# liruihui/Dis-PU

Hardware: AMD Instinct MI355X
Metric: upsampled points/sec (256->1024, 4x) (higher is better)
Workload: dtype f32; 1 GPU; BASELINE configs[1]: 32 patches x 256 points per GPU, generator forward 256->1024 (4x), fp32; patches_per_gpu=32, global_patches=32, weights=xavier-uniform seed 1234, zero bias, parallelism=patch-sharded x1

## Files before the change

### dis-pu_amd/_lib.py

```python
import collections
import ctypes as C
import os

_HERE = os.path.dirname(os.path.abspath(__file__))
LIB_PATH = os.path.join(_HERE, "lib", "libdispu_hip.so")

ABI_VERSION = 5
ARITH_PLAIN = 0
ARITH_CONTRACT = 1
ARITH_PINNED_EXP = 2
MESH_BRUTE_FORCE = 8
MESH_TILE = 64
LINEAR_PLAN_INTS = 21
POISSON_MAX_N = 49152
POISSON_MAX_ROUNDS = 256
POISSON_CELLS_NONFINITE = 4
SORT_ROWS_MAX_K = 4096
RADIX_TILE = 2048
GRID_NONFINITE, GRID_AXIS_X, GRID_AXIS_Y, GRID_AXIS_Z, GRID_TOO_MANY_POINTS = 1, 2, 3, 4, 5
LATTICE_NONFINITE, LATTICE_RANGE = 1, 2
ORIENT_HOST_ROUNDS = 1
ORIENT_PROFILE_FLOATS = 8
CLUSTER_HEAD_INTS = 16

_vp, _i, _sz, _l =C.c_void_p, C.c_int, C.c_size_t, C.c_long

SIGNATURES = {
    "dispu_version": (_i, []),
    "dispu_error_string": (C.c_char_p, [_i]),
    "dispu_event_record": (_i, [_vp, _vp]),
    "dispu_stream_wait_event": (_i, [_vp, _vp]),
    "dispu_memset_async": (_i, [_vp, _i, _sz, _vp]),
    "dispu_fps_scratch_bytes": (_sz, [_i, _i, _i]),
    "dispu_fps": (_i, [_i, _i, _i, _vp, _vp, _vp, _i, _vp]),
    "dispu_fps_ws": (_i, [_i, _i, _i, _vp, _vp, _sz, _vp, _i, _vp]),
    "dispu_fps_segments_scratch_bytes": (_sz, [_i, _vp, _vp]),
    "dispu_fps_segments": (_i, [_i, _vp, _vp, _vp, _vp, _vp, _vp, _sz, _vp, _i, _vp]),
    "dispu_fps_cells_scratch_bytes": (_sz, [_i, _vp, _vp, _i]),
    "dispu_fps_cells": (_i, [_i, _vp, _vp, _vp, _vp, _vp, _vp, _sz, _vp, _vp, _i, _i, _vp]),
    "dispu_fps_cells_wanted": (_i, [_i, _i]),
    "dispu_pca_normals_scratch_bytes": (_sz, [_i, _vp, _i]),
    "dispu_pca_normals_segments": (_i, [_i, _vp, _vp, _i, _vp, _i, _vp, _vp, _vp, _vp, _vp, _vp, _sz, _vp]),
    "dispu_orient_consistent_scratch_bytes": (_sz, [_i, _vp, _i]),
    "dispu_orient_consistent_segments": (_i, [_i, _vp, _vp, _i, _vp, _vp, _vp, _i, _i, _vp, _vp, _vp, _vp, _vp, _vp, _sz, _vp, _vp]),
    "dispu_knn_mean_dist_scratch_bytes": (_sz, [_i, _vp, _i]),
    "dispu_knn_mean_dist_segments": (_i, [_i, _vp, _vp, _i, _vp, _vp, _vp, _vp, _sz, _vp]),
    "dispu_radius_count_scratch_bytes": (_sz, [_i, _vp]),
    "dispu_radius_count_segments": (_i, [_i, _vp, _vp, C.c_float, _i, _vp, _vp, _vp, _vp, _sz, _vp]),
    "dispu_outlier_threshold_segments": (_i, [_i, _vp, _vp, _vp, _vp, C.c_double, _vp, _vp]),
    "dispu_compact_scratch_bytes": (_sz, [_i, _vp]),
    "dispu_compact_segments": (_i, [_i, _vp, _vp, _vp, _i, _vp, _vp, _i, _vp, _vp, _vp, _vp, _vp, _sz, _vp]),
    "dispu_cluster_scratch_bytes": (_sz, [_i, _vp]),
    "dispu_cluster_segments": (_i, [_i, _vp, _vp, C.c_float, _i, _vp, _vp, _vp, _vp, _vp, _vp, _vp, _sz, _vp]),
    "dispu_cluster_select_segments": (_i, [_i, _vp, _vp, _vp, _vp, _vp, _vp, _i, _i, _vp, _vp]),
    "dispu_knn_cross_scratch_bytes": (_sz, [_i, _vp, _vp]),
    "dispu_knn_cross_segments": (_i, [_i, _vp, _vp, _vp, _vp, _i, _vp, _vp, _vp, _vp, _vp, _vp, _sz, _vp]),
    "dispu_transfer_attributes_segments": (_i, [_i, _vp, _vp, _vp, _vp, _i, _i, _vp, _vp, _i, _vp, _vp, _vp, _vp, _vp, _vp, _sz, _vp]),
    "dispu_mls_project_scratch_bytes": (_sz, [_i, _vp, _vp]),
    "dispu_mls_project_segments": (_i, [_i, _vp, _vp, _vp, _vp, _i, C.c_double, _i, _vp, _vp, _vp, _vp, _vp, _vp, _sz, _vp]),
    "dispu_icp_scratch_bytes": (_sz, [_i, _vp, _vp]),
    "dispu_icp_segments": (_i, [_i, _vp, _vp, _vp, _vp, _i, _i, C.c_float, C.c_double] + [_vp] * 13 + [_sz, _vp]),
    "dispu_rigid_apply_segments": (_i, [_i, _vp, _vp, _vp, _vp, _vp, _vp]),
    "dispu_signed_distance_scratch_bytes": (_sz, [_i, _vp, _vp]),
    "dispu_signed_distance_segments": (_i, [_i, _vp, _vp, _vp, _vp, _i, C.c_double, _vp, _vp, _vp, _vp, _vp, _vp, _sz, _vp]),
    "dispu_lattice_voxels_scratch_bytes": (_sz, [C.c_longlong]),
    "dispu_lattice_voxels": (_i, [C.c_longlong, _vp, C.c_float, _i, _vp, _vp, _vp, _vp, _sz, _vp]),
    "dispu_lattice_dilate_scratch_bytes": (_sz, [C.c_longlong, _i]),
    "dispu_lattice_dilate": (_i, [C.c_longlong, _vp, _i, _vp, _vp, _vp, _sz, _vp]),
    "dispu_lattice_corners_scratch_bytes": (_sz, [C.c_longlong]),
    "dispu_lattice_corners": (_i, [C.c_longlong, _vp, _vp, _vp, _vp, _vp, _sz, _vp]),
    "dispu_lattice_positions": (_i, [C.c_longlong, _vp, C.c_float, _vp, _vp]),
    "dispu_contour_count_scratch_bytes": (_sz, [C.c_longlong, C.c_longlong]),
    "dispu_contour_count": (_i, [C.c_longlong, C.c_longlong, _vp, _vp, _vp, _vp, _vp, _vp, _vp, _sz, _vp]),
    "dispu_contour_emit": (_i, [C.c_longlong, C.c_longlong, C.c_float, _vp, _vp, _vp, _vp, _vp, C.c_longlong, C.c_longlong, _vp, _vp, _vp]),
    "dispu_fps_segments_auto_scratch_bytes": (_sz, [_i, _vp, _vp]),
    "dispu_fps_segments_auto": (_i, [_i, _vp, _vp, _vp, _vp, _vp, _vp, _sz, _vp, _vp, _i, _vp]),
    "dispu_prob_sample": (_i, [_i, _i, _i, _vp, _vp, _vp, _vp, _vp]),
    "dispu_selection_sort": (_i, [_i, _i, _i, _i, _vp, _vp, _vp, _vp]),
    "dispu_gather_point": (_i, [_i, _i, _i, _vp, _vp, _vp, _vp]),
    "dispu_gather_point_grad": (_i, [_i, _i, _i, _vp, _vp, _vp, _vp]),
    "dispu_query_ball": (_i, [_i, _i, _i, _vp, _i, _vp, _vp, _vp, _vp, _i, _vp]),
    "dispu_group_point": (_i, [_i, _i, _i, _i, _i, _vp, _vp, _vp, _vp]),
    "dispu_group_point_grad": (_i, [_i, _i, _i, _i, _i, _vp, _vp, _vp, _vp]),
    "dispu_knn_point": (_i, [_i, _i, _i, _i, _i, _vp, _vp, _vp, _vp, _vp]),
    "dispu_knn_feat": (_i, [_i, _i, _i, _i, _i, _vp, _vp, _vp, _vp, _vp]),
    "dispu_knn_feat_strided": (_i, [_i, _i, _i, _i, _i, _vp, _i, _vp, _i, _vp, _vp, _vp]),
    "dispu_knn_xyz": (_i, [_i, _i, _i, _i, _vp, _vp, _vp, _vp, _i, _vp]),
    "dispu_knn_feat_scratch_bytes": (_sz, [_i, _i, _i, _i, _i]),
    "dispu_knn_feat_strided_ws": (_i, [_i, _i, _i, _i, _i, _vp, _i, _vp, _i, _vp, _vp, _vp, _sz, _vp]),
    "dispu_knn_xyz_scratch_bytes": (_sz, [_i, _i, _i, _i]),
    "dispu_knn_xyz_ws": (_i, [_i, _i, _i, _i, _vp, _vp, _vp, _vp, _vp, _sz, _i, _vp]),
    "dispu_three_nn": (_i, [_i, _i, _i, _vp, _vp, _vp, _vp, _i, _vp]),
    "dispu_three_interpolate": (_i, [_i, _i, _i, _i, _vp, _vp, _vp, _vp, _vp]),
    "dispu_three_interpolate_grad": (_i, [_i, _i, _i, _i, _vp, _vp, _vp, _vp, _vp]),
    "dispu_nn_distance": (_i, [_i, _i, _vp, _i, _vp, _vp, _vp, _vp, _vp, _i, _vp]),
    "dispu_nn_distance_grad": (_i, [_i, _i, _vp, _i, _vp, _vp, _vp, _vp, _vp, _vp, _vp, _vp]),
    "dispu_approx_match_scratch_bytes": (_sz, [_i, _i, _i]),
    "dispu_approx_match": (_i, [_i, _i, _i, _vp, _vp, _vp, _vp, _i, _vp]),
    "dispu_approx_match_ws": (_i, [_i, _i, _i, _vp, _vp, _vp, _vp, _sz, _i, _vp]),
    "dispu_approx_match_levels_ws": (_i, [_i, _i, _i, _vp, _vp, _vp, _sz, _i, _vp]),
    "dispu_emd_loss_grad_scratch_bytes": (_sz, [_i, _i, _i]),
    "dispu_emd_loss_grad": (_i, [_i, _i, _i, _vp, _vp, _vp, _vp, C.c_float, _vp, _vp, _vp, _sz, _i, _vp]),
    "dispu_match_cost_scratch_bytes": (_sz, [_i, _i, _i]),
    "dispu_match_cost": (_i, [_i, _i, _i, _vp, _vp, _vp, _vp, _i, _vp]),
    "dispu_match_cost_ws": (_i, [_i, _i, _i, _vp, _vp, _vp, _vp, _vp, _i, _vp]),
    "dispu_match_cost_grad_scratch_bytes": (_sz, [_i, _i, _i]),
    "dispu_match_cost_grad": (_i, [_i, _i, _i, _vp, _vp, _vp, _vp, _vp, _i, _vp]),
    "dispu_match_cost_grad_ws": (_i, [_i, _i, _i, _vp, _vp, _vp, _vp, _vp, _vp, _i, _vp]),
    "dispu_linear": (_i, [_i, _i, _i, _i, _vp, _l, _l, _vp, _l, _l, _i, _vp, _i, _vp, _l, _l, _vp, _l, _l, _vp, _l, _l, _vp]),
    "dispu_linear_bn": (_i, [_i, _i, _i, _i, _vp, _l, _l, _vp, _l, _l, _i, _vp, _vp, _vp, _i, _vp, _l, _l, _vp, _l, _l, _vp, _l, _l,
                             _vp]),
    "dispu_linear_tile": (_i, [_i, _i, _i]),
    "dispu_linear_tile2": (_i, [_i, _i, _i, _i, _i]),
    "dispu_debug_linear_tile": (None, [_i]),
    "dispu_linear_plan": (_i, [_i, _i, _i, _i, _vp, _l, _l, _vp, _l, _l, _i, _vp, _vp, _vp, _i, _vp, _l, _l, _vp, _l, _l, _vp, _l, _l, _vp, _l, _i,
                               _vp]),
    "dispu_linear_bf16_plan": (_i, [_i, _i, _i, _i]),
    "dispu_sa_fused": (_i, [_i, _i, _i, _i, _i, _vp, _vp, _vp, _vp, _i, _vp, _vp, _vp, _vp, _vp, _vp, _vp]),
    "dispu_edge_conv_fused": (_i, [_i, _i, _i, _i, _vp, _l, _vp, _i, _i, _vp, _vp, _vp, _vp, _vp, _i, _vp, _vp]),
    "dispu_group_center": (_i, [_l, _i, _i, _vp, _vp, _vp]),
    "dispu_pool_nsample": (_i, [_l, _i, _i, _i, _vp, _vp, _vp, _vp]),
    "dispu_idw_weights": (_i, [_l, _vp, _vp, _vp]),
    "dispu_l2_normalize_rows": (_i, [_l, _i, _vp, _vp, _vp]),
    "dispu_scale_add": (_i, [_l, _vp, C.c_float, _vp, _vp, _vp]),
    "dispu_edge_feature": (_i, [_l, _i, _i, _i, _vp, _l, _vp, _i, _i, _vp, _l, _vp]),
    "dispu_row_mean_max": (_i, [_i, _i, _vp, _vp, _vp, _vp]),
    "dispu_repulsion": (_i, [_l, _i, _i, _i, C.c_float, _vp, _vp, _vp, _vp]),
    "dispu_linear_small_k": (_i, [_l, _i, _i, _vp, _l, _vp, _vp, _i, _vp, _l, _vp]),
    "dispu_linear_small_n": (_i, [_l, _i, _i, _vp, _l, _vp, _vp, _i, _vp, _l, _vp, _l, _vp]),
    "dispu_edge_dense_conv": (_i, [_i, _i, _i, _vp, _l, _vp, _i, _i, _vp, _vp, _vp, _vp, _vp, _vp, _vp, _l, _vp]),
    "dispu_stem_block": (_i, [_i, _i, _i, _vp, _l, _i, _i, _vp, _vp, _vp, _vp, _vp, _vp, _vp, _l, _vp, _vp, _vp, _i, _vp, _l, _vp, _vp, _vp, _vp,
                              _l, _vp]),
    "dispu_edge_dense_conv_valu": (_i, [_i, _i, _i, _vp, _l, _vp, _i, _i, _vp, _vp, _vp, _vp, _vp, _vp, _vp, _l, _vp]),
    "dispu_dup_grid": (_i, [_i, _i, _i, _i, _vp, _l, _vp, _vp, _vp, _vp, _l, _vp]),
    "dispu_ps_prep": (_i, [_l, _i, _vp, _vp, _vp, _vp, _l, _vp, _l, _vp]),
    "dispu_ps_gather_sub_relu": (_i, [_l, _i, _i, _i, _vp, _vp, _l, _vp, _l, _vp, _l, _vp]),
    "dispu_ps_skip_max": (_i, [_l, _i, _i, _i, _vp, _vp, _vp, _l, _vp, _l, _vp]),
    "dispu_ps_weight_net": (_i, [_l, _i, _i, _i, _vp, _vp, _vp, _vp, _vp, _vp, _vp, _vp]),
    "dispu_ps_point_matmul": (_i, [_l, _i, _i, _i, _vp, _l, _vp, _vp, _l, _vp]),
    "dispu_ps_local": (_i, [_l, _i, _i, _i, _vp, _vp, _vp, _l, _vp, _vp, _vp, _vp, _vp, _vp, _vp, _vp, _vp]),
    "dispu_ps_local_bf16": (_i, [_l, _i, _i, _i, _vp, _vp, _vp, _l, _vp, _vp, _vp, _vp, _vp, _vp, _vp, _vp, _vp]),
    "dispu_knn_patch": (_i, [_i, _i, _i, _i, _vp, _vp, _vp, _vp]),
    "dispu_normalize_patches": (_i, [_i, _i, _vp, _vp, _vp, _vp, _vp]),
    "dispu_denormalize_patches": (_i, [_i, _i, _vp, _vp, _vp, _vp, _vp]),
    "dispu_knn_patch_segments": (_i, [_i, _vp, _vp, _vp, _vp, _i, _vp, _vp, _vp, _vp]),
    "dispu_normalize_segments": (_i, [_i, _vp, _vp, _vp, _vp, _vp, _vp, _vp]),
    "dispu_attention": (_i, [_i, _i, _i, _i, _vp, _l, _vp, _l, _vp, _l, C.c_float, _vp, _l, _vp]),
    "dispu_attention_fwd_lse": (_i, [_i, _i, _i, _i, _vp, _l, _vp, _l, _vp, _l, C.c_float, _vp, _l, _vp, _vp]),
    "dispu_attention_bwd": (_i, [_i, _i, _i, _i, _vp, _l, _vp, _l, _vp, _l, C.c_float, _vp, _l, _vp, _vp, _l, _vp, _l, _vp, _l, _vp, _l,
                                 _vp, _vp]),
    "dispu_attention_project": (_i, [_i, _i, _i, _i, _vp, _l, _vp, _l, _vp, _l, C.c_float, _vp, _vp, _i, _vp, _l, _vp]),
    "dispu_softmax_rows": (_i, [_l, _i, C.c_float, _vp, _l, _vp]),
    "dispu_linear_tn_bf16_stream_scratch_floats": (_l, [_i, _i, _i]),
    "dispu_linear_tn_bf16_stream": (_i, [_i, _i, _i, _vp, _l, _vp, _l, _i, _vp, _l, _i, _vp, _vp, _l, _vp]),
    "dispu_bf16_pack": (_i, [_i, _i, _vp, _l, _i, _vp, _vp]),
    "dispu_linear_bf16_stream": (_i, [_i, _i, _i, _vp, _l, _i, _vp, _l, _vp, _i, _vp, _l, _i, _i, _l, _vp]),
    "dispu_linear_bf16": (_i, [_i, _i, _i, _i, _vp, _l, _l, _vp, _l, _l, _i, _vp, _i, _vp, _l, _l, _vp, _l, _l, _vp, _l, _l, _vp]),
    "dispu_linear_tn_bf16_scratch_floats": (_l, [_i, _i, _i, _i]),
    "dispu_linear_tn_bf16": (_i, [_i, _i, _i, _i, _vp, _l, _l, _vp, _l, _l, _vp, _l, _l, _i, _vp, _vp, _l, _vp]),
    "dispu_bf16x3_split_weights": (_i, [_i, _i, _vp, _l, _vp, _vp]),
    "dispu_linear_bf16x3": (_i, [_i, _i, _i, _vp, _l, _vp, _vp, _i, _vp, _l, _vp, _l, _vp, _l, _vp]),
    "dispu_debug_x3_kernel": (None, [_i]),
    "dispu_linear_tn_scratch_floats": (_l, [_i, _i, _i, _i]),
    "dispu_linear_tn": (_i, [_i, _i, _i, _i, _vp, _l, _l, _vp, _l, _l, _vp, _l, _l, _i, _vp, _vp, _l, _vp]),
    "dispu_ps_local_grad": (_i, [_l, _i] + [_vp] * 3 + [_l] + [_vp] * 14),
    "dispu_linear_tn_plan": (_i, [_i, _i, _i, _i, _vp, _l, _l, _vp, _l, _l, _vp, _l, _l, _i, _vp, _vp, _l, _vp]),
    "dispu_linear_tn_bf16_plan": (_i, [_i, _i, _i, _i, _vp, _l, _l, _vp, _l, _l, _vp, _l, _l, _i, _vp, _vp, _l, _i, _vp]),
    "dispu_linear_tn_bf16_stream_plan": (_i, [_i, _i, _i, _vp, _l, _vp, _l, _i, _vp, _l, _i, _vp, _vp, _l, _vp]),
    "dispu_tn_defer": (_i, [_vp]),
    "dispu_tn_reduce_grouped": (_i, [_i, _vp, _vp, _vp]),
    "dispu_act_bias_grad_scratch_floats": (_l, [_l, _i]),
    "dispu_act_bias_grad": (_i, [_l, _i, _vp, _l, _vp, _l, _i, _vp, _l, _vp, _i, _vp, _l, _vp]),
    "dispu_max_k": (_i, [_l, _i, _i, _vp, _l, _vp, _l, _vp]),
    "dispu_max_k_grad": (_i, [_l, _i, _i, _vp, _l, _vp, _l, _vp, _l, _vp, _l, _i, _vp]),
    "dispu_max_k_grad_tail": (_i, [_l, _i, _i, _i, _vp, _l, _vp, _l, _vp, _l, _vp, _l, _vp]),
    "dispu_edge_feature_grad": (_i, [_l, _i, _i, _i, _vp, _l, _vp, _i, _i, _vp, _l, _vp]),
    "dispu_dup_sum_grad": (_i, [_i, _i, _i, _i, _vp, _l, _vp, _l, _vp]),
    "dispu_ps_group": (_i, [_l, _i, _i, _i, _vp, _vp, _vp, _l, _vp, _l, _vp]),
    "dispu_ps_group_grad": (_i, [_l, _i, _i, _i, _vp, _vp, _l, _vp, _vp, _l, _vp]),
    "dispu_ps_point_matmul_grad": (_i, [_l, _i, _i, _i, _vp, _l, _vp, _vp, _l, _vp, _l, _vp, _vp]),
    "dispu_softmax_rows_grad": (_i, [_l, _i, C.c_float, _vp, _l, _vp, _l, _vp]),
    "dispu_bn_scratch_bytes": (_l, [_l, _i]),
    "dispu_bn_train": (_i, [_l, _i, _vp, _l, _vp, _vp, C.c_float, C.c_float, _i, _vp, _l, _vp, _vp, _vp, _vp, _l, _vp]),
    "dispu_bn_train_grad": (_i, [_l, _i, _vp, _l, _vp, _l, _vp, _l, _vp, _vp, _i, _vp, _l, _vp, _vp, _vp, _vp, _l, _vp]),
    "dispu_sigmoid_offset": (_i, [_l, _vp, _vp, _vp, _vp]),
    "dispu_sigmoid_offset_grad": (_i, [_l, _vp, _vp, _vp, _vp, _vp]),
    "dispu_repulsion_grad": (_i, [_l, _i, _i, C.c_float, C.c_float, _vp, _vp, _vp, _vp]),
    "dispu_add3": (_i, [_l, _vp, _vp, _vp, _vp, _vp]),
    "dispu_linear_splitk_finish": (_i, [_l, _i, _i, _vp, _l, _vp, _i, _vp, _l, _vp]),
    "dispu_fill_rows": (_i, [_i, _i, _vp, C.c_float, _vp, _vp]),
    "dispu_mlp_chain": (_i, [_l, _i, _i, _i, _i, _vp, _l, _vp, _vp, _vp, _vp, _vp, _vp, _vp, _vp, _vp, _l, _i, _vp, _l, _vp, _l, _vp]),
    "dispu_linear_masked": (_i, [_i, _i, _i, _i, _vp, _l, _l, _vp, _l, _l, _i, _vp, _i, _vp, _l, _l, _vp, _l, _l, _vp, _l, _i, _vp]),
    "dispu_linear_bf16_masked": (_i, [_i, _i, _i, _i, _vp, _l, _l, _vp, _l, _l, _i, _vp, _i, _vp, _l, _l, _vp, _l, _l, _vp, _l, _i, _vp]),
    "dispu_mlp_chain_sum3": (_i, [_l, _i, _i, _i, _i, _vp, _vp, _vp, _l, _vp, _vp, _vp, _vp, _vp, _vp, _vp, _vp, _vp, _l, _i, _vp, _l, _vp, _l, _vp]),
    "dispu_mlp_chain_dup": (_i, [_i, _i, _i, _i, _i, _i, _i, _vp, _l, _vp, _vp, _vp, _vp, _vp, _vp, _vp, _vp, _vp, _vp, _vp, _vp, _l, _i, _vp, _l,
                                 _vp, _l, _vp]),
    "dispu_mlp_chain_stash": (_i, [_l, _i, _i, _i, _i, _vp, _l, _vp, _vp, _vp, _vp, _vp, _vp, _vp, _vp, _vp, _l, _vp, _l, _vp, _l, _vp, _l,
                                   _i, _vp, _l, _vp, _l, _vp]),
    "dispu_mlp_chain_grad": (_i, [_l, _i, _i, _i, _vp, _l, _vp, _vp, _vp, _vp, _vp, _l, _vp, _l, _vp, _l, _vp, _l, _vp, _l, _vp, _l, _vp, _l, _vp, _l,
                                  _vp, _vp, _vp, _l, _vp, _vp, _vp, _l, _vp]),
    "dispu_mask3": (_i, [_l, _i, _vp, _l, _vp, _l, _vp, _l, _vp, _l, _vp, _vp, _vp, _l, _vp]),
    "dispu_ps_wnet_scratch_bytes": (_l, [_l]),
    "dispu_ps_wnet_bn_stats": (_i, [_l, _i, _i, _i, _vp, _vp, _vp, _vp, _vp, _vp, C.c_float, C.c_float, _vp, _vp, _vp, _vp, _vp, _vp, _l, _vp]),
    "dispu_ps_wnet_grad": (_i, [_l, _i, _i, _i, _vp, _vp, _vp, _vp, _vp, _vp, _vp, _vp, _vp, _vp, _vp, _vp, _vp, _vp, _vp, _vp, _l, _vp]),
    "dispu_knn_invert": (_i, [_i, _i, _i, _vp, _vp, _vp, _vp]),
    "dispu_ps_conv0_gather_grad": (_i, [_l, _i, _i, _i, _vp, _vp, _vp, _vp, _l, _vp, _l, _vp, _l, _vp, _l, _vp, _l, _vp]),
    "dispu_ps_prep_grad": (_i, [_l, _i, _vp, _vp, _vp, _l, _vp, _l, _vp, _vp, _vp]),
    "dispu_ps_skip_max_grad": (_i, [_l, _i, _i, _i, _vp, _vp, _vp, _l, _vp, _l, _vp, _l, _vp, _vp, _l, _i, _vp]),
    "dispu_ps_point_matmul_grad_relu": (_i, [_l, _i, _i, _i, _vp, _l, _vp, _vp, _l, _vp, _l, _vp, _vp]),
    "dispu_edge_dense_conv_grad_scratch_floats": (_l, [_i, _i]),
    "dispu_edge_dense_conv_grad_partials": (_i, [_i, _i, _i, _vp, _l, _vp, _i, _i, _vp, _vp, _vp, _vp, _vp, _vp, _vp, _l, _vp, _l, _vp, _l, _vp]),
    "dispu_edge_dense_conv_grad_reduce": (_i, [_i, _i, _vp, _l, _vp, _vp, _vp, _vp, _vp, _vp, _vp]),
    "dispu_edge_dense_conv_grad": (_i, [_i, _i, _i, _vp, _l, _vp, _i, _i, _vp, _vp, _vp, _vp, _vp, _vp, _vp, _l, _vp, _l, _vp, _vp, _vp, _vp, _vp,
                                        _vp, _vp, _l, _vp]),
    "dispu_repulsion_loss_grad": (_i, [_l, _i, _i, C.c_float, C.c_float, _vp, _vp, _vp, _vp, _vp]),
    "dispu_transpose_batched": (_i, [_i, _vp, _vp, _vp, _vp]),
    "dispu_linear_bf16s": (_i, [_i, _i, _i, _i, _vp, _l, _l, _vp, _l, _l, _i, _vp, _i, _vp, _l, _l, _vp, _l, _l, _i, _vp]),
    "dispu_linear_tn_bf16s": (_i, [_i, _i, _i, _i, _vp, _l, _l, _vp, _l, _l, _vp, _l, _l, _i, _vp, _vp, _l, _i, _vp]),
    "dispu_ps_gather_sub_relu_bf16": (_i, [_l, _i, _i, _i, _vp, _vp, _l, _vp, _l, _vp, _l, _vp]),
    "dispu_ps_point_matmul_grad_relu_s": (_i, [_l, _i, _i, _i, _vp, _l, _vp, _vp, _l, _vp, _l, _vp, _i, _vp]),
    "dispu_ps_conv0_gather_grad_s": (_i, [_l, _i, _i, _i, _vp, _vp, _vp, _vp, _l, _i, _vp, _l, _vp, _l, _vp, _l, _vp, _l, _vp]),
    "dispu_chamfer_loss_grad": (_i, [_i, _i, _vp, _i, _vp, _vp, _vp, _vp, _vp, _vp, C.c_float, _vp, _vp, _vp]),
    "dispu_pu_loss_finalize": (_i, [_vp, _vp, _l, C.c_float, C.c_float, _vp, _vp]),
    "dispu_step_meters": (_i, [_i, _i, _i, _vp, _vp, _vp, _vp, _vp, _vp, _vp, _vp]),
    "dispu_uniform_loss_grad": (_i, [_i, _i, _i, _i, _vp, _vp, _vp, _vp, _vp, _vp, _vp, _vp, _i, _vp]),
    "dispu_pu_loss_finalize_u": (_i, [_vp, _vp, _l, C.c_float, C.c_float, _vp, _i, _l, C.c_float, _vp, _vp]),
    "dispu_pu_loss_finalize_e": (_i, [_vp, _vp, _l, C.c_float, C.c_float, _vp, _i, _l, C.c_float, _vp, _vp, _i, _i, C.c_float, _vp, _vp]),
    "dispu_augment": (_i, [_i, _i, _vp, _vp, _vp, _vp, _vp, _vp, _vp]),
    "dispu_sample_batch": (_i, [_i, _i, _i, _vp, _vp, _vp, _i, _i, C.c_ulonglong, _i, C.c_float, C.c_float, _i, _vp, _vp, _vp, _vp, _vp, _vp,
                                _vp, _vp, _vp, _vp]),
    "dispu_adam": (_i, [_l, _vp, _vp, _vp, _vp, C.c_float, C.c_float, C.c_float, C.c_float, C.c_float, _vp]),
    "dispu_point_to_mesh": (_i, [_i, _vp, _i, _vp, _vp, _vp, _vp, _vp, _vp, _i, _vp]),
    "dispu_disk_count": (_i, [_i, _i, _i, _vp, _vp, _vp, _vp, _vp]),
    "dispu_disk_fill": (_i, [_i, _i, _i, _vp, _vp, _vp, _vp, _vp, _vp]),
    "dispu_disk_uniformity_scratch_bytes": (_sz, [_i, _i]),
    "dispu_disk_uniformity": (_i, [_i, _i, _i, _vp, _vp, _vp, _vp, _vp, _i, _vp, _sz, _vp, _vp]),
    "dispu_row_mean_std": (_i, [_i, _i, _vp, _vp, _vp]),
    "dispu_geodesic_scratch_bytes": (_sz, [_i, _i]),
    "dispu_geodesic_hash_slots": (_i, [_i]),
    "dispu_geodesic_distances": (_i, [_i, _vp, _vp, _vp, _vp, _vp, _vp, _vp, _vp, _vp, _i, _vp, _vp, _vp, _vp, C.c_double, _i, _vp, _sz, _vp,
                                      _vp, _vp]),
    "dispu_geodesic_disk_count": (_i, [_i, _i, _vp, _vp, _vp, _vp, _vp]),
    "dispu_geodesic_disk_fill": (_i, [_i, _i, _vp, _vp, _vp, _vp, _vp, _vp, _vp]),
    "dispu_mesh_sample": (_i, [_i, _i, _vp, _vp, _vp, _i, C.c_ulonglong, _vp, _vp, _vp, _vp]),
    "dispu_poisson_disk_scratch_bytes": (_sz, [_i, _i]),
    "dispu_poisson_disk_keep": (_i, [_i, _i, _vp, _vp, _vp, _vp, _vp, _sz, _vp, _vp]),
    "dispu_poisson_disk_select": (_i, [_i, _i, _i, _i, _vp, _vp, _vp, _vp, _vp, _vp, _sz, _vp, _vp]),
    "dispu_sort_rows_i32": (_i, [_i, _i, _vp, _vp]),
    "dispu_poisson_cells_scratch_bytes": (_sz, [_i, C.c_longlong]),
    "dispu_poisson_cells_keep": (_i, [_i, _vp, _vp, _vp, _vp, _vp, _vp, _vp, _vp, _sz, _vp, _vp]),
    "dispu_poisson_cells_select": (_i, [_i, _vp, _vp, _vp, _vp, _i, _vp, _vp, _vp, _vp, _vp, _vp, _vp, _sz, _vp, _vp]),
    "dispu_radix_sort_scratch_bytes": (_sz, [C.c_longlong]),
    "dispu_radix_sort_pairs": (_i, [C.c_longlong, _i, _vp, _vp, _vp, _vp, _vp, _sz, _vp]),
    "dispu_grid_subsample_scratch_bytes": (_sz, [C.c_longlong, _i, _i]),
    "dispu_grid_subsample_plan": (_i, [C.c_longlong, _vp, C.c_float, _vp, _sz, _vp, _vp, _vp, _vp]),
    "dispu_grid_subsample_emit": (_i, [C.c_longlong, _i, _i, _i, _vp, _vp, _vp, _vp, _sz, _vp, _vp, _vp, _vp]),
}

class TnReduceDesc(C.Structure):
    _fields_ = [("part", _vp), ("out", _vp), ("dbias", _vp), ("ldo", _l), ("stride", _l), ("K", _i), ("N", _i), ("splits", _i),
                ("rows_p", _i), ("accumulate", _i), ("bias_accumulate", _i), ("assoc", _i), ("reserved", _i)]


_LIB = None


class DispuError(RuntimeError):
    pass


def lib():
    global _LIB
    if _LIB is None:
        import torch
        if not os.path.exists(LIB_PATH):
            raise DispuError(
                "libdispu_hip.so not found at %s -- build it with `python dis-pu_amd/build.py` "
                "(there is no CPU fallback for the dis-pu_amd ops)" % LIB_PATH)
        l = C.CDLL(LIB_PATH)
        for name, (res, args) in SIGNATURES.items():
            fn = getattr(l, name)
            fn.restype = res
            fn.argtypes = args
        if l.dispu_version() < ABI_VERSION:
            raise DispuError("libdispu_hip.so at %s has ABI version %d, this package needs >= %d -- rebuild it with "
                             "`python dis-pu_amd/build.py`" % (LIB_PATH, l.dispu_version(), ABI_VERSION))
        _LIB = l
    return _LIB


class Tape(object):
    def __init__(self):
        self.calls = []
        self.keep = []

    def replay(self):
        for fn, args, what in self.calls:
            rc = fn(*args)
            if rc:
                check(rc, what + " (tape replay)")

    def __len__(self):
        return len(self.calls)


_TAPE = None
_NO_TAPE = ("dispu_version", "dispu_error_string", "dispu_linear_tile", "dispu_linear_tile2", "dispu_linear_plan", "dispu_linear_bf16_plan",
            "dispu_linear_tn_plan", "dispu_linear_tn_bf16_plan", "dispu_linear_tn_bf16_stream_plan")


class _TapeLib(object):

    def __init__(self, real):
        self._real = real
        self._cache = {}

    def __getattr__(self, name):
        fn = self._cache.get(name)
        if fn is None:
            real = getattr(self._real, name)
            if name in _NO_TAPE or real.restype is not _i or "scratch" in name:
                fn = real
            else:
                argtypes = real.argtypes

                def fn(*args, _real=real, _types=argtypes, _name=name):
                    if _TAPE is None:
                        return _real(*args)
                    cargs = tuple(a if isinstance(a, C._SimpleCData) else t(a) for a, t in zip(args, _types))
                    rc = _real(*cargs)
                    _TAPE.calls.append((_real, cargs, _name))
                    return rc
            self._cache[name] = fn
        return fn


_TAPELIB = None


def tape_lib():
    global _TAPELIB
    if _TAPELIB is None:
        _TAPELIB = _TapeLib(lib())
    return _TAPELIB


def tape_begin():
    global _TAPE
    _TAPE = Tape()
    return _TAPE


def tape_end():
    global _TAPE
    t, _TAPE = _TAPE, None
    return t


def taping():
    return _TAPE


def check(code, what):
    if code != 0:
        msg = lib().dispu_error_string(code)
        raise DispuError("%s failed: hip error %d (%s)" % (what, code, msg.decode() if msg else "?"))


def linear_plan(batch, M, K, N, X, ldx, sx, W, ldw, sw, transb, bias, scale, shift, act, Y, ldy, sy, R1, ldr1, sr1, R2, ldr2, sr2, Mk, ldm,
                mcols):
    buf = (_i * LINEAR_PLAN_INTS)()
    check(lib().dispu_linear_plan(batch, M, K, N, X, ldx, sx, W, ldw, sw, transb, bias, scale, shift, act, Y, ldy, sy, R1, ldr1, sr1, R2, ldr2,
                                  sr2, Mk, ldm, mcols, buf), "dispu_linear_plan")
    out = []
    for i in range(buf[0]):
        kind, n0, n1, bm, bn, bk, tb, edge, epi, ng = buf[1 + 10 * i:11 + 10 * i]
        out.append(("tiled", n0, n1, bm, bn, bk, tb, edge, epi) if kind else ("skinny", n0, n1, ng, tb))
    return out


TnPlan = collections.namedtuple("TnPlan", "rc kind TK TNN edge splits rows direct reduce reduce_grid capped wpb grid_y")
TnBf16Plan = collections.namedtuple("TnBf16Plan", "rc kind tile splits rows reduce rows_p")
TnStreamPlan = collections.namedtuple("TnStreamPlan", "rc BN storage splits rows")
TN_KINDS = ("none", "narrow", "tiled", "clear")
TN_REDUCE = ("none", "scalar", "vec4")


def linear_tn_plan(batch, M, K, N, X, ldx, sx, Z, ldz, sz, out, ldo, so, accumulate, dbias, scratch, scratch_floats):
    buf = (_i * 12)()
    rc = lib().dispu_linear_tn_plan(batch, M, K, N, X, ldx, sx, Z, ldz, sz, out, ldo, so, accumulate, dbias, scratch, scratch_floats, buf)
    v = list(buf)
    return TnPlan(rc, TN_KINDS[v[0]], v[1], v[2], v[3], v[4], v[5], v[6], TN_REDUCE[v[7]], v[8], v[9], v[10], v[11])


def linear_tn_bf16_plan(batch, M, K, N, X, ldx, sx, Z, ldz, sz, out, ldo, so, accumulate, dbias, scratch, scratch_floats, storage=0):
    buf = (_i * 6)()
    rc = lib().dispu_linear_tn_bf16_plan(batch, M, K, N, X, ldx, sx, Z, ldz, sz, out, ldo, so, accumulate, dbias, scratch, scratch_floats,
                                         storage, buf)
    v = list(buf)
    return TnBf16Plan(rc, TN_KINDS[v[0]], v[1], v[2], v[3], v[4], v[5])


def linear_tn_bf16_stream_plan(M, K, N, X, ldx, Z, ldz, storage, out, ldo, accumulate, dbias, scratch, scratch_floats):
    buf = (_i * 4)()
    rc = lib().dispu_linear_tn_bf16_stream_plan(M, K, N, X, ldx, Z, ldz, storage, out, ldo, accumulate, dbias, scratch, scratch_floats, buf)
    return TnStreamPlan(rc, *list(buf))


def stream_ptr(device=None):
    import torch
    return C.c_void_p(torch.cuda.current_stream(device).cuda_stream)


def ptr(t):
    return C.c_void_p(t.data_ptr()) if t is not None else C.c_void_p(0)
```

### dis-pu_amd/csrc/linear.hip

```cpp
#include "common.h"
#include "internal.h"

#include <type_traits>

#include <cstdio>
#include <cstdlib>

namespace dispu {

typedef float f32x16 __attribute__((ext_vector_type(16)));

struct LinearArgs {
    int M, K, N;
    const float* X; long ldx; long sx;
    const float* W; long ldw; long sw;
    const float* bias;
    float* Y; long ldy; long sy;
    const float* R1; long ldr1; long sr1;
    const float* R2; long ldr2; long sr2;
    int act;
    const float* scale;
    const float* shift;
    const float* Mk; long ldm; int mcols;
};

template <int BM, int BN, int BK, bool TRANSB, bool EDGE>
struct LinearLds {
    static constexpr bool DMA = !EDGE && !TRANSB && BK == 16 && (BM == 64 || BM == 128) && (BN == 64 || BN == 128 || BN == 256);
    static constexpr int NST = DMA ? 4 : 2;
    static constexpr int LDA = DMA ? BM : BM + 1;
    static constexpr int LDB = TRANSB ? BN + 1 : (DMA && BN < 256) ? BN : BN + 4;
    static constexpr int STAGE = ((BK * (LDA + LDB) + 3) / 4) * 4;
    static constexpr size_t BYTES = (size_t)NST * STAGE * sizeof(float);
};

#ifdef LIN_CLOCK
__device__ unsigned long long lin_clock_ticks[4];
#endif
template <int BM, int BN, int WM, int WN, int BK, bool TRANSB, bool EDGE, int EPI_T>
__global__ __launch_bounds__(64 * (WM * WN + (LinearLds<BM, BN, BK, TRANSB, EDGE>::DMA ? 4 : WM * WN))) void linear_mfma_kernel(LinearArgs a) {
#ifdef LIN_CLOCK
    const unsigned long long lc0 = __builtin_readcyclecounter();
    unsigned long long lc_wait = 0;
#endif
    using L = LinearLds<BM, BN, BK, TRANSB, EDGE>;
    constexpr bool DMA = L::DMA;
    constexpr int NT = 64 * WM * WN;
    constexpr int LDA = L::LDA, LDB = L::LDB;
    constexpr int TM = BM / (32 * WM), TN = BN / (32 * WN);
    constexpr int A_F4 = BM * BK / 4 / NT;
    constexpr int B_F4 = BN * BK / 4 / NT;
    static_assert(A_F4 >= 1 && B_F4 >= 1 && TM >= 1 && TN >= 1, "tile too small for the workgroup");
    static_assert((BM * BK / 4) % NT == 0 && (BN * BK / 4) % NT == 0, "tile must split evenly over the threads");
    extern __shared__ __attribute__((aligned(16))) float lds[];

    const int lane = threadIdx.x & 63, wave = threadIdx.x >> 6;
    const int z = blockIdx.z;
    const int m0 = blockIdx.y * BM, n0 = blockIdx.x * BN;
    const int M = a.M, K = a.K, N = a.N;
    const int ntile = (K + BK - 1) / BK;

    if (wave >= WM * WN) {
        if constexpr (DMA) {
            const int lw = __builtin_amdgcn_readfirstlane(wave - WM * WN);
            const float* __restrict__ X = a.X + (size_t)z * a.sx;
            const float* __restrict__ W = a.W + (size_t)z * a.sw;
            constexpr int NA = 4 * BM / 64, NB = 16 * BN / 256, PER = (NA + NB) / 4;
            static_assert((NA + NB) % 4 == 0, "DMA instructions must split evenly over the four loader waves");
            constexpr int RPI = 256 / BN;
            const long ldw = a.ldw, ldx = a.ldx;
            const float* gsrc[PER];
            int ldst[PER];
#pragma unroll
            for (int u = 0; u < PER; ++u) {
                const int q = lw + 4 * u;
                if (q < NA) {
                    const int kg = q / (BM / 64), rb = q % (BM / 64);
                    gsrc[u] = X + (size_t)(m0 + rb * 64 + lane) * ldx + 4 * kg;
                    ldst[u] = (kg * BM + rb * 64) * 4;
                } else {
                    const int pb = q - NA, kr = pb * RPI + lane / (BN / 4);
                    gsrc[u] = W + (size_t)kr * ldw + n0 + 4 * (lane % (BN / 4));
                    ldst[u] = BK * LDA + (pb * RPI) * LDB;
                }
            }
            auto issue = [&](int t) {
                float* st = lds + (t & 3) * L::STAGE;
                const size_t ko = (size_t)t * BK;
#pragma unroll
                for (int u = 0; u < PER; ++u) {
                    const int q = lw + 4 * u;
                    const float* src = (q < NA) ? gsrc[u] + ko : gsrc[u] + ko * ldw;
                    __builtin_amdgcn_global_load_lds(src, (__attribute__((address_space(3))) void*)(st + ldst[u]), 16, 0, 0);
                }
            };
            auto wait_newer = [&](int newer) {
                if (newer >= 2) __builtin_amdgcn_s_waitcnt(0x0F70 | (((2 * PER) & 0xF)) | ((((2 * PER) >> 4) & 0x3) << 14));
                else if (newer == 1) __builtin_amdgcn_s_waitcnt(0x0F70 | ((PER & 0xF)) | (((PER >> 4) & 0x3) << 14));
                else __builtin_amdgcn_s_waitcnt(0x0F70);
            };
            issue(0);
            if (ntile > 1) issue(1);
            if (ntile > 2) issue(2);
            wait_newer(min(2, ntile - 1));
            asm volatile("s_barrier" ::: "memory");
            for (int t = 0; t < ntile; ++t) {
                if (t + 3 < ntile) issue(t + 3);
                wait_newer(max(0, min(2, ntile - 2 - t)));
                asm volatile("s_barrier" ::: "memory");
            }
            return;
        }
        const int tid = threadIdx.x - NT;
        const float* __restrict__ X = a.X + (size_t)z * a.sx;
        const float* __restrict__ W = a.W + (size_t)z * a.sw;
        const long ldx = a.ldx, ldw = a.ldw;
        float4 pa[A_F4], pb[B_F4];
        const bool x_vec = ((ldx & 3) == 0) && ((((uintptr_t)X) & 15) == 0);
        const bool w_vec = ((ldw & 3) == 0) && ((((uintptr_t)W) & 15) == 0);

        auto load_rowsk = [&](const float* __restrict__ P, long ld, bool vec, int row_base, int rows, int k0, int it) -> float4 {
            const int idx = tid + it * NT;
            const int r = idx / (BK / 4), kq = idx % (BK / 4);
            const int row = row_base + r, k = k0 + kq * 4;
            if constexpr (!EDGE) return *reinterpret_cast<const float4*>(P + (size_t)row * ld + k);
            float4 v = make_float4(0.f, 0.f, 0.f, 0.f);
            if (row < rows && k < K) {
                const float* p = P + (size_t)row * ld + k;
                if (vec && k + 3 < K) {
                    v = *reinterpret_cast<const float4*>(p);
                } else {
                    v.x = p[0];
                    if (k + 1 < K) v.y = p[1];
                    if (k + 2 < K) v.z = p[2];
                    if (k + 3 < K) v.w = p[3];
                }
            }
            return v;
        };
        auto store_rowsk = [&](float* S, int LD, float4 v, int it) {
            const int idx = tid + it * NT;
            const int r = idx / (BK / 4), kq = idx % (BK / 4);
            S[(kq * 4 + 0) * LD + r] = v.x;
            S[(kq * 4 + 1) * LD + r] = v.y;
            S[(kq * 4 + 2) * LD + r] = v.z;
            S[(kq * 4 + 3) * LD + r] = v.w;
        };
        auto load_b = [&](int k0, int it) -> float4 {
            const int idx = tid + it * NT;
            const int kr = idx / (BN / 4), nq = idx % (BN / 4);
            const int k = k0 + kr, n = n0 + nq * 4;
            if constexpr (!EDGE) return *reinterpret_cast<const float4*>(W + (size_t)k * ldw + n);
            float4 v = make_float4(0.f, 0.f, 0.f, 0.f);
            if (k < K && n < N) {
                const float* p = W + (size_t)k * ldw + n;
                if (w_vec && n + 3 < N) {
                    v = *reinterpret_cast<const float4*>(p);
                } else {
                    v.x = p[0];
                    if (n + 1 < N) v.y = p[1];
                    if (n + 2 < N) v.z = p[2];
                    if (n + 3 < N) v.w = p[3];
                }
            }
            return v;
        };
        auto store_b = [&](float* S, float4 v, int it) {
            const int idx = tid + it * NT;
            const int kr = idx / (BN / 4), nq = idx % (BN / 4);
            *reinterpret_cast<float4*>(&S[kr * LDB + nq * 4]) = v;
        };
        float4 pa1[A_F4], pb1[B_F4];
        auto load_tile = [&](int k0, float4 (&qa)[A_F4], float4 (&qb)[B_F4]) {
#pragma unroll
            for (int it = 0; it < A_F4; ++it) qa[it] = load_rowsk(X, ldx, x_vec, m0, M, k0, it);
#pragma unroll
            for (int it = 0; it < B_F4; ++it) qb[it] = TRANSB ? load_rowsk(W, ldw, w_vec, n0, N, k0, it) : load_b(k0, it);
        };
        auto store_tile = [&](int stage, const float4 (&qa)[A_F4], const float4 (&qb)[B_F4]) {
            float* As = lds + stage * L::STAGE;
            float* Bs = As + BK * LDA;
#pragma unroll
            for (int it = 0; it < A_F4; ++it) store_rowsk(As, LDA, qa[it], it);
#pragma unroll
            for (int it = 0; it < B_F4; ++it) {
                if constexpr (TRANSB) store_rowsk(Bs, LDB, qb[it], it);
                else store_b(Bs, qb[it], it);
            }
        };
        load_tile(0, pa, pb);
        store_tile(0, pa, pb);
        if (ntile > 1) load_tile(BK, pa1, pb1);
        if (ntile > 2) load_tile(2 * BK, pa, pb);
        __syncthreads();
        for (int t = 0; t < ntile; t += 2) {
            if (t + 1 < ntile) {
                store_tile(1, pa1, pb1);
                if (t + 3 < ntile) load_tile((t + 3) * BK, pa1, pb1);
            }
            __syncthreads();
            if (t + 1 < ntile) {
                if (t + 2 < ntile) {
                    store_tile(0, pa, pb);
                    if (t + 4 < ntile) load_tile((t + 4) * BK, pa, pb);
                }
                __syncthreads();
            }
        }
        return;
    }

    const int wm = wave / WN, wn = wave % WN;
    f32x16 acc[TM][TN];
#pragma unroll
    for (int i = 0; i < TM; ++i)
#pragma unroll
        for (int j = 0; j < TN; ++j)
#pragma unroll
            for (int r = 0; r < 16; ++r) acc[i][j][r] = 0.f;

    const int fi = lane & 31, fk = lane >> 5;
    constexpr bool CI = !EDGE && !TRANSB && (TN == 4 || TN == 2);
    auto rdB = [&](const float* Bs, int krow, float (&b)[TN]) {
        if constexpr (CI && TN == 4) {
            const float4 t4 = *reinterpret_cast<const float4*>(&Bs[krow * LDB + wn * (TN * 32) + 4 * fi]);
            b[0] = t4.x; b[1] = t4.y; b[2] = t4.z; b[3] = t4.w;
        } else if constexpr (CI && TN == 2) {
            const float2 t2 = *reinterpret_cast<const float2*>(&Bs[krow * LDB + wn * (TN * 32) + 2 * fi]);
            b[0] = t2.x; b[1] = t2.y;
        } else {
#pragma unroll
            for (int j = 0; j < TN; ++j) b[j] = Bs[krow * LDB + wn * (TN * 32) + j * 32 + fi];
        }
    };
    __syncthreads();
    if constexpr (DMA) {
        auto slab = [&](auto stage_c) {
            constexpr int SG = decltype(stage_c)::value;
            const float* st = lds + SG * L::STAGE;
            const float* Bs = st + BK * LDA;
            const float* Asf = st + fk;
            float a2[2][TM][2];
            float bf[2][TN];
#pragma unroll
            for (int i = 0; i < TM; ++i) {
                const float* pr = Asf + (wm * (TM * 32) + i * 32 + fi) * 4;
                a2[0][i][0] = pr[0]; a2[0][i][1] = pr[2];
            }
            rdB(Bs, fk, bf[0]);
#pragma unroll
            for (int s2 = 0; s2 < BK / 2; ++s2) {
                const int kg = s2 >> 1, u = s2 & 1, cur = s2 & 1, nxt = cur ^ 1;
                if (s2 + 1 < BK / 2) {
                    const int kk = 2 * (s2 + 1);
                    if (u == 1) {
#pragma unroll
                        for (int i = 0; i < TM; ++i) {
                            const float* pr = Asf + ((kg + 1) * BM + wm * (TM * 32) + i * 32 + fi) * 4;
                            a2[(kg + 1) & 1][i][0] = pr[0]; a2[(kg + 1) & 1][i][1] = pr[2];
                        }
                    }
                    rdB(Bs, kk + fk, bf[nxt]);
                }
#pragma unroll
                for (int i = 0; i < TM; ++i)
#pragma unroll
                    for (int j = 0; j < TN; ++j)
                        acc[i][j] = __builtin_amdgcn_mfma_f32_32x32x2f32(a2[kg & 1][i][u], bf[cur][j], acc[i][j], 0, 0, 0);
                constexpr int NB = CI ? 1 : TN / 2;
                if (u == 1) __builtin_amdgcn_sched_group_barrier(0x100, TM + NB, 0);
                else __builtin_amdgcn_sched_group_barrier(0x100, NB, 0);
                __builtin_amdgcn_sched_group_barrier(0x008, TM * TN, 0);
            }
#ifdef LIN_CLOCK
            const unsigned long long lb0 = __builtin_readcyclecounter();
            __syncthreads();
            lc_wait += __builtin_readcyclecounter() - lb0;
#else
            __syncthreads();
#endif
        };
        for (int t = 0; t < ntile; t += 4) {
            slab(std::integral_constant<int, 0>{});
            if (t + 1 < ntile) slab(std::integral_constant<int, 1>{});
            if (t + 2 < ntile) slab(std::integral_constant<int, 2>{});
            if (t + 3 < ntile) slab(std::integral_constant<int, 3>{});
        }
    } else
    for (int t = 0; t < ntile; ++t) {
        const float* As = lds + (t & 1) * L::STAGE;
        const float* Bs = As + BK * LDA;
        float af[2][TM], bf[2][TN];
#pragma unroll
        for (int i = 0; i < TM; ++i) af[0][i] = As[fk * LDA + wm * (TM * 32) + i * 32 + fi];
        rdB(Bs, fk, bf[0]);
#pragma unroll
        for (int s2 = 0; s2 < BK / 2; ++s2) {
            const int cur = s2 & 1, nxt = cur ^ 1;
            if (s2 + 1 < BK / 2) {
                const int kk = 2 * (s2 + 1);
#pragma unroll
                for (int i = 0; i < TM; ++i) af[nxt][i] = As[(kk + fk) * LDA + wm * (TM * 32) + i * 32 + fi];
                rdB(Bs, kk + fk, bf[nxt]);
            }
#pragma unroll
            for (int i = 0; i < TM; ++i)
#pragma unroll
                for (int j = 0; j < TN; ++j)
                    acc[i][j] = __builtin_amdgcn_mfma_f32_32x32x2f32(af[cur][i], bf[cur][j], acc[i][j], 0, 0, 0);
            __builtin_amdgcn_sched_group_barrier(0x100, TM + (CI ? 1 : TN), 0);
            __builtin_amdgcn_sched_group_barrier(0x008, TM * TN, 0);
        }
#ifdef LIN_CLOCK
        const unsigned long long lb0 = __builtin_readcyclecounter();
        __syncthreads();
        lc_wait += __builtin_readcyclecounter() - lb0;
#else
        __syncthreads();
#endif
    }

#ifdef LIN_CLOCK
    if (blockIdx.x == 0 && blockIdx.y == 5 && threadIdx.x == 0) { lin_clock_ticks[0] = __builtin_readcyclecounter() - lc0; lin_clock_ticks[1] = ntile; lin_clock_ticks[2] = lc_wait; }
#endif
    constexpr int EPI = (EPI_T == 6) ? 0 : EPI_T;
    constexpr bool E_SCALE = (EPI == 1 || EPI == 4), E_R1 = (EPI >= 2), E_R2 = (EPI >= 3);
    float* __restrict__ Y = a.Y + (size_t)z * a.sy;
    const float lo = (a.act == 1) ? 0.f : -__builtin_inff();
    const bool has_bias = a.bias != nullptr;
    const float* __restrict__ R1 = (E_R1 && a.R1) ? a.R1 + (size_t)z * a.sr1 : nullptr;
    const float* __restrict__ R2 = (E_R2 && a.R2) ? a.R2 + (size_t)z * a.sr2 : nullptr;
    const int wm_u = __builtin_amdgcn_readfirstlane(wm), wn_u = __builtin_amdgcn_readfirstlane(wn);
    const int rbase = m0 + wm_u * (TM * 32), cbase = n0 + wn_u * (TN * 32);
    const long ldy = a.ldy, ldr1 = a.ldr1, ldr2 = a.ldr2, ldm = a.ldm;
    const unsigned offy = (unsigned)(4 * fk * ldy + fi), off1 = (unsigned)(4 * fk * ldr1 + fi), off2 = (unsigned)(4 * fk * ldr2 + fi);
    const unsigned offm = (unsigned)(4 * fk * ldm + fi);
    if constexpr (CI) {
        typedef float vecT __attribute__((ext_vector_type(TN)));
        const int col0 = cbase + TN * fi;
        const unsigned voy = (unsigned)(4 * fk * ldy + TN * fi), vo1 = (unsigned)(4 * fk * ldr1 + TN * fi), vo2 = (unsigned)(4 * fk * ldr2 + TN * fi);
        const unsigned vom = (unsigned)(4 * fk * ldm + TN * fi);
        vecT bv, sc, sh;
#pragma unroll
        for (int j = 0; j < TN; ++j) { bv[j] = 0.f; sc[j] = 1.f; sh[j] = 0.f; }
        if (has_bias) bv = *reinterpret_cast<const vecT*>(a.bias + col0);
        if constexpr (E_SCALE) {
            if (a.scale) { sc = *reinterpret_cast<const vecT*>(a.scale + col0); sh = *reinterpret_cast<const vecT*>(a.shift + col0); }
        }
#pragma unroll
        for (int i = 0; i < TM; ++i) {
#pragma unroll
            for (int rb = 0; rb < 16; rb += 8) {
                vecT r1v[8], r2v[8], mkv[8];
                if constexpr (EPI == 5) {
#pragma unroll
                    for (int r = 0; r < 8; ++r) {
                        const int rowu = rbase + i * 32 + ((rb + r) & 3) + 8 * ((rb + r) >> 2);
#pragma unroll
                        for (int j = 0; j < TN; ++j) mkv[r][j] = 1.f;
                        if (a.Mk != nullptr) {
                            const vecT m = *reinterpret_cast<const vecT*>(a.Mk + (size_t)rowu * ldm + cbase + vom);
#pragma unroll
                            for (int j = 0; j < TN; ++j) mkv[r][j] = (col0 + j < a.mcols) ? m[j] : 1.f;
                        }
                    }
                }
                if constexpr (EPI >= 4) {
#pragma unroll
                    for (int r = 0; r < 8; ++r) {
                        const int rowu = rbase + i * 32 + ((rb + r) & 3) + 8 * ((rb + r) >> 2);
#pragma unroll
                        for (int j = 0; j < TN; ++j) { r1v[r][j] = 0.f; r2v[r][j] = 0.f; }
                        if (R1) r1v[r] = *reinterpret_cast<const vecT*>(R1 + (size_t)rowu * ldr1 + cbase + vo1);
                    }
#pragma unroll
                    for (int r = 0; r < 8; ++r) {
                        const int rowu = rbase + i * 32 + ((rb + r) & 3) + 8 * ((rb + r) >> 2);
                        if (R2) r2v[r] = *reinterpret_cast<const vecT*>(R2 + (size_t)rowu * ldr2 + cbase + vo2);
                    }
                }
#pragma unroll
                for (int r = 0; r < 8; ++r) {
                    const int rowu = rbase + i * 32 + ((rb + r) & 3) + 8 * ((rb + r) >> 2);
                    vecT v;
#pragma unroll
                    for (int j = 0; j < TN; ++j) {
                        float e = acc[i][j][rb + r];
                        if (has_bias) e = e + bv[j];
                        if constexpr (E_SCALE) {
                            if (a.scale) e = e * sc[j] + sh[j];
                        }
                        e = fmaxf(e, lo);
                        if constexpr (EPI >= 4) {
                            if (R1) e = e + r1v[r][j];
                            if (R2) e = e + r2v[r][j];
                        }
                        if constexpr (EPI == 5) e = (mkv[r][j] > 0.f) ? e : 0.f;
                        v[j] = e;
                    }
                    *reinterpret_cast<vecT*>(Y + (size_t)rowu * ldy + cbase + voy) = v;
                }
                if constexpr (EPI >= 4) __builtin_amdgcn_sched_barrier(0);
            }
        }
        return;
    }
#pragma unroll
    for (int j = 0; j < TN; ++j) {
        const int colu = cbase + j * 32;
        const int col = colu + fi;
        const bool col_ok = !EDGE || col < N;
        const int colc = col_ok ? col : 0;
        const float bv = has_bias ? a.bias[colc] : 0.f;
        float sc = 1.f, sh = 0.f;
        if constexpr (E_SCALE) {
            if (a.scale) { sc = a.scale[colc]; sh = a.shift[colc]; }
        }
#pragma unroll
        for (int i = 0; i < TM; ++i) {
            float r1v[16], r2v[16], mkv[16];
            if constexpr (EPI == 5) {
                const bool msk = a.Mk != nullptr && col < a.mcols && col_ok;
#pragma unroll
                for (int r = 0; r < 16; ++r) {
                    const int rowu = rbase + i * 32 + (r & 3) + 8 * (r >> 2);
                    const bool ok = msk && (!EDGE || rowu + 4 * fk < M);
                    mkv[r] = ok ? (a.Mk + (size_t)rowu * ldm + colu)[offm] : 1.f;
                }
            }
            if constexpr (EPI >= 4) {
#pragma unroll
                for (int r = 0; r < 16; ++r) {
                    const int rowu = rbase + i * 32 + (r & 3) + 8 * (r >> 2);
                    const bool ok = col_ok && (!EDGE || rowu + 4 * fk < M);
                    r1v[r] = (R1 && ok) ? (R1 + (size_t)rowu * ldr1 + colu)[off1] : 0.f;
                }
#pragma unroll
                for (int r = 0; r < 16; ++r) {
                    const int rowu = rbase + i * 32 + (r & 3) + 8 * (r >> 2);
                    const bool ok = col_ok && (!EDGE || rowu + 4 * fk < M);
                    r2v[r] = (R2 && ok) ? (R2 + (size_t)rowu * ldr2 + colu)[off2] : 0.f;
                }
            }
#pragma unroll
            for (int r = 0; r < 16; ++r) {
                const int rowu = rbase + i * 32 + (r & 3) + 8 * (r >> 2);
                if (col_ok && (!EDGE || rowu + 4 * fk < M)) {
                    float v = acc[i][j][r];
                    if (has_bias) v = v + bv;
                    if constexpr (E_SCALE) {
                        if (a.scale) v = v * sc + sh;
                    }
                    v = fmaxf(v, lo);
                    if constexpr (EPI >= 4) {
                        if (R1) v = v + r1v[r];
                        if (R2) v = v + r2v[r];
                    }
                    if constexpr (EPI == 5) v = (mkv[r] > 0.f) ? v : 0.f;
                    (Y + (size_t)rowu * ldy + colu)[offy] = v;
                }
            }
            if constexpr (EPI >= 4) __builtin_amdgcn_sched_barrier(0);
        }
    }
}

template <int BM, int BN, int WM, int WN, int BK, bool TRANSB, bool EDGE, int EPI>
static int launch_epi(const LinearArgs& a, dim3 grid, hipStream_t s) {
    constexpr size_t bytes = LinearLds<BM, BN, BK, TRANSB, EDGE>::BYTES;
    auto kern = linear_mfma_kernel<BM, BN, WM, WN, BK, TRANSB, EDGE, EPI>;
    if (bytes > 64 * 1024) {
        static DevOnce done;
        if (done.needed()) {
            hipError_t e = hipFuncSetAttribute(reinterpret_cast<const void*>(kern), hipFuncAttributeMaxDynamicSharedMemorySize, (int)bytes);
            if (e != hipSuccess) return (int)e;
            done.done();
        }
    }
    hipLaunchKernelGGL(kern, grid, dim3(64 * (WM * WN + (LinearLds<BM, BN, BK, TRANSB, EDGE>::DMA ? 4 : WM * WN))), bytes, s, a);
    return (int)hipGetLastError();
}

struct LinearLaunch {
    int skinny;
    int n0, n1;
    int bm, bn, bk;
    int transb;
    int edge;
    int epi;
    int ng;
};
struct LinearPlan {
    int n;
    LinearLaunch l[2];
};

}

using namespace dispu;

static int g_tile_override = 0;
DISPU_EXPORT void dispu_debug_linear_tile(int code) { g_tile_override = code; }

static int linear_tile_rule(int batch, int M, int N, bool dma) {
    if (g_tile_override > 0) return g_tile_override;
    const long mb128 = (long)((M + 127) / 128) * batch;
    if (N >= 256 && N % 256 == 0 && mb128 * (N / 256) >= 256) return 128257;
    if (N > 64 && N % 128 != 0 && N % 64 == 0 && mb128 >= 64) return 64064;
    const long mb64 = (long)((M + 63) / 64) * batch;
    if (N > 64) {
        if (mb128 * ((N + 127) / 128) >= 256) return 128128;
        const long wg = mb64 * ((N + 127) / 128);
        return (wg >= 512 || (dma && N % 128 == 0 && wg >= 256)) ? 64128 : 64064;
    }
    return mb128 >= 256 ? 128064 : 64064;
}

DISPU_EXPORT int dispu_linear_tile(int batch, int M, int N) { return linear_tile_rule(batch, M, N, true); }
DISPU_EXPORT int dispu_linear_tile2(int batch, int M, int K, int N, int transb) { return linear_tile_rule(batch, M, N, !transb && (K % 16) == 0); }

static LinearLaunch linear_decide_tiled(const LinearArgs& a, int batch, bool transb) {
    LinearLaunch l{};
    l.n0 = 0; l.n1 = a.N; l.transb = transb ? 1 : 0;
    constexpr int BK = 16;
    int bkr = 32;
    switch (linear_tile_rule(batch, a.M, a.N, !transb && (a.K % 16) == 0)) {
        case 128257: l.bm = 128; l.bn = 256; bkr = 16; break;
        case 128128: l.bm = 128; l.bn = 128; break;
        case 64128: l.bm = 64; l.bn = 128; break;
        case 128064: l.bm = 128; l.bn = 64; break;
        default: l.bm = 64; l.bn = 64; break;
    }
    const bool aligned = ((a.ldx & 3) == 0) && ((a.ldw & 3) == 0) && ((a.sx & 3) == 0) && ((a.sw & 3) == 0) &&
                         ((((uintptr_t)a.X) & 15) == 0) && ((((uintptr_t)a.W) & 15) == 0);
    const auto al16 = [](const void* p) { return (((uintptr_t)p) & 15) == 0; };
    const bool out_aligned = ((a.ldy & 3) == 0) && ((a.sy & 3) == 0) && al16(a.Y) && (!a.bias || al16(a.bias)) &&
                             (!a.scale || (al16(a.scale) && al16(a.shift))) &&
                             (!a.R1 || (((a.ldr1 & 3) == 0) && ((a.sr1 & 3) == 0) && al16(a.R1))) &&
                             (!a.R2 || (((a.ldr2 & 3) == 0) && ((a.sr2 & 3) == 0) && al16(a.R2))) &&
                             (!a.Mk || (((a.ldm & 3) == 0) && al16(a.Mk) && a.mcols >= a.N));
    const bool tiles_ok = aligned && out_aligned && (a.M % l.bm == 0) && (a.N % l.bn == 0);
    if (tiles_ok && !transb && (a.K % BK == 0)) { l.bk = BK; l.edge = 0; }
    else if (tiles_ok && transb && (a.K % bkr == 0)) { l.bk = bkr; l.edge = 0; }
    else { l.bk = bkr; l.edge = 1; }
    if (!a.scale && !a.R1 && !a.R2 && !a.Mk)
        l.epi = (l.bm == 128 && l.bn == 256 && l.bk == 16 && !transb && !l.edge && a.K >= 1024) ? 6 : 0;
    else if (a.scale && !a.R1 && !a.R2 && !a.Mk) l.epi = 1;
    else l.epi = a.Mk ? 5 : 4;
    return l;
}

static int linear_decide(int batch, int M, int K, int N, const float* X, long ldx, long sx, const float* W, long ldw, long sw, int transb,
                         const float* bias, const float* scale, const float* shift, int act, const float* Y, long ldy, long sy,
                         const float* R1, long ldr1, long sr1, const float* R2, long ldr2, long sr2, const float* Mk, long ldm, int mcols,
                         LinearPlan& plan) {
    plan = LinearPlan{};
    if (batch < 0 || M < 0 || K <= 0 || N <= 0 || !X || !W || !Y || act < 0 || act > 1 || ((scale == nullptr) != (shift == nullptr)))
        return (int)hipErrorInvalidValue;
    if (Mk && batch != 1) return (int)hipErrorInvalidValue;
    if (batch == 0 || M == 0) return 0;
    int nh = N;
    if (batch == 1 && !scale && !R2) {
        int ng = linear_skinny_rule(M, K, N, X, ldx, W, ldw, transb);
        if (ng == 0) {
            const int tail = N % 128, n0 = N - tail;
            if (n0 > 0 && tail > 0 && tail <= 32) {
                const float* Wt = transb ? W + (size_t)n0 * ldw : W + n0;
                const int ngt = linear_skinny_rule(M, K, tail, X, ldx, Wt, ldw, transb);
                if (ngt) {
                    LinearLaunch& t = plan.l[plan.n++];
                    t.skinny = 1; t.n0 = n0; t.n1 = N; t.transb = transb ? 1 : 0; t.ng = ngt;
                    nh = n0;
                    ng = linear_skinny_rule(M, K, nh, X, ldx, W, ldw, transb);
                }
            }
        }
        if (ng) {
            LinearLaunch& t = plan.l[plan.n++];
            t.skinny = 1; t.n0 = 0; t.n1 = nh; t.transb = transb ? 1 : 0; t.ng = ng;
            return 0;
        }
    }
    LinearArgs a{M, K, nh, X, ldx, sx, W, ldw, sw, bias, const_cast<float*>(Y), ldy, sy, R1, ldr1, sr1, R2, ldr2, sr2, act, scale, shift,
                 (Mk && mcols > 0) ? Mk : nullptr, ldm, mcols};
    plan.l[plan.n++] = linear_decide_tiled(a, batch, transb != 0);
    return 0;
}

template <int BM, int BN, int WM, int WN, int BK, bool TRANSB, bool EDGE>
static int launch_one(const LinearArgs& a, dim3 grid, int epi, hipStream_t s) {
    switch (epi) {
        case 0: return launch_epi<BM, BN, WM, WN, BK, TRANSB, EDGE, 0>(a, grid, s);
        case 1: return launch_epi<BM, BN, WM, WN, BK, TRANSB, EDGE, 1>(a, grid, s);
        case 4: return launch_epi<BM, BN, WM, WN, BK, TRANSB, EDGE, 4>(a, grid, s);
        case 5: return launch_epi<BM, BN, WM, WN, BK, TRANSB, EDGE, 5>(a, grid, s);
        case 6:
            if constexpr (BM == 128 && BN == 256 && BK == 16 && !TRANSB && !EDGE) return launch_epi<BM, BN, WM, WN, BK, TRANSB, EDGE, 6>(a, grid, s);
            break;
    }
    return (int)hipErrorInvalidValue;
}

template <int BM, int BN, int WM, int WN, int BK, int BKR = BK>
static int launch_linear(const LinearArgs& a, int batch, const LinearLaunch& l, hipStream_t s) {
    dim3 grid((a.N + BN - 1) / BN, (a.M + BM - 1) / BM, batch);
    if (!l.edge && !l.transb) return launch_one<BM, BN, WM, WN, BK, false, false>(a, grid, l.epi, s);
    if (!l.edge) return launch_one<BM, BN, WM, WN, BKR, true, false>(a, grid, l.epi, s);
    if (l.transb) return launch_one<BM, BN, WM, WN, BKR, true, true>(a, grid, l.epi, s);
    return launch_one<BM, BN, WM, WN, BKR, false, true>(a, grid, l.epi, s);
}

static int linear_impl(int batch, int M, int K, int N, const float* X, long ldx, long sx, const float* W, long ldw, long sw, int transb,
                       const float* bias, const float* scale, const float* shift, int act, float* Y, long ldy, long sy, const float* R1,
                       long ldr1, long sr1, const float* R2, long ldr2, long sr2, const float* Mk, long ldm, int mcols, void* stream);

DISPU_EXPORT int dispu_linear(int batch, int M, int K, int N, const float* X, long ldx, long sx, const float* W,
                              long ldw, long sw, int transb, const float* bias, int act, float* Y, long ldy, long sy,
                              const float* R1, long ldr1, long sr1, const float* R2, long ldr2, long sr2, void* stream) {
    return linear_impl(batch, M, K, N, X, ldx, sx, W, ldw, sw, transb, bias, nullptr, nullptr, act, Y, ldy, sy, R1, ldr1,
                       sr1, R2, ldr2, sr2, nullptr, 0, 0, stream);
}

DISPU_EXPORT int dispu_linear_masked(int batch, int M, int K, int N, const float* X, long ldx, long sx, const float* W,
                                     long ldw, long sw, int transb, const float* bias, int act, float* Y, long ldy, long sy,
                                     const float* R1, long ldr1, long sr1, const float* Mk, long ldm, int mcols, void* stream) {
    if (Mk && batch != 1) return (int)hipErrorInvalidValue;
    return linear_impl(batch, M, K, N, X, ldx, sx, W, ldw, sw, transb, bias, nullptr, nullptr, act, Y, ldy, sy, R1, ldr1,
                       sr1, nullptr, 0, 0, Mk, ldm, Mk ? mcols : 0, stream);
}

DISPU_EXPORT int dispu_linear_bn(int batch, int M, int K, int N, const float* X, long ldx, long sx, const float* W,
                                 long ldw, long sw, int transb, const float* bias, const float* scale, const float* shift,
                                 int act, float* Y, long ldy, long sy, const float* R1, long ldr1, long sr1,
                                 const float* R2, long ldr2, long sr2, void* stream) {
    return linear_impl(batch, M, K, N, X, ldx, sx, W, ldw, sw, transb, bias, scale, shift, act, Y, ldy, sy, R1, ldr1, sr1, R2, ldr2, sr2,
                       nullptr, 0, 0, stream);
}

DISPU_EXPORT int dispu_linear_plan(int batch, int M, int K, int N, const float* X, long ldx, long sx, const float* W, long ldw, long sw,
                                   int transb, const float* bias, const float* scale, const float* shift, int act, const float* Y, long ldy,
                                   long sy, const float* R1, long ldr1, long sr1, const float* R2, long ldr2, long sr2, const float* Mk,
                                   long ldm, int mcols, int* plan) {
    if (!plan) return (int)hipErrorInvalidValue;
    LinearPlan p;
    const int rc = linear_decide(batch, M, K, N, X, ldx, sx, W, ldw, sw, transb, bias, scale, shift, act, Y, ldy, sy, R1, ldr1, sr1, R2,
                                 ldr2, sr2, Mk, ldm, Mk ? mcols : 0, p);
    for (int i = 0; i < DISPU_LINEAR_PLAN_INTS; ++i) plan[i] = 0;
    if (rc) return rc;
    plan[0] = p.n;
    for (int i = 0; i < p.n; ++i) {
        const LinearLaunch& l = p.l[i];
        int* o = plan + 1 + 10 * i;
        o[0] = l.skinny ? 0 : 1; o[1] = l.n0; o[2] = l.n1; o[3] = l.bm; o[4] = l.bn; o[5] = l.bk; o[6] = l.transb; o[7] = l.edge;
        o[8] = l.epi; o[9] = l.ng;
    }
    return 0;
}

static int linear_impl(int batch, int M, int K, int N, const float* X, long ldx, long sx, const float* W, long ldw, long sw, int transb,
                       const float* bias, const float* scale, const float* shift, int act, float* Y, long ldy, long sy, const float* R1,
                       long ldr1, long sr1, const float* R2, long ldr2, long sr2, const float* Mk, long ldm, int mcols, void* stream) {
    LinearPlan plan;
    int rc = linear_decide(batch, M, K, N, X, ldx, sx, W, ldw, sw, transb, bias, scale, shift, act, Y, ldy, sy, R1, ldr1, sr1, R2, ldr2, sr2,
                           Mk, ldm, mcols, plan);
    if (rc) return rc;
    hipStream_t s = (hipStream_t)stream;
    for (int i = 0; i < plan.n; ++i) {
        const LinearLaunch& l = plan.l[i];
        const int n0 = l.n0, nn = l.n1 - l.n0;
        if (l.skinny) {
            const float* Wt = transb ? W + (size_t)n0 * ldw : W + n0;
            rc = linear_skinny_launch(l.ng, M, K, nn, X, ldx, Wt, ldw, transb, bias ? bias + n0 : nullptr, act, Y + n0, ldy,
                                      R1 ? R1 + n0 : nullptr, ldr1, Mk ? Mk + n0 : nullptr, ldm, mcols - n0, s);
        } else {
            LinearArgs a{M, K, nn, X, ldx, sx, W, ldw, sw, bias, Y, ldy, sy, R1, ldr1, sr1, R2, ldr2, sr2, act, scale, shift,
                         (Mk && mcols > 0) ? Mk : nullptr, ldm, mcols};
            switch (l.bm * 1000 + l.bn) {
                case 128256: rc = launch_linear<128, 256, 2, 2, 16>(a, batch, l, s); break;
                case 128128: rc = launch_linear<128, 128, 2, 2, 16, 32>(a, batch, l, s); break;
                case 64128: rc = launch_linear<64, 128, 2, 2, 16, 32>(a, batch, l, s); break;
                case 128064: rc = launch_linear<128, 64, 2, 2, 16, 32>(a, batch, l, s); break;
                default: rc = launch_linear<64, 64, 2, 2, 16, 32>(a, batch, l, s); break;
            }
        }
        if (rc) return rc;
    }
    return 0;
}
```

### dis-pu_amd/csrc/ps_local.hip

```cpp
#include "common.h"

#include <cstdlib>
#include <type_traits>

namespace dispu {

typedef float f32x16 __attribute__((ext_vector_type(16)));
typedef float f32x2 __attribute__((ext_vector_type(2)));
typedef float f32x4 __attribute__((ext_vector_type(4)));
typedef unsigned u32x4 __attribute__((ext_vector_type(4)));
typedef unsigned u32x2 __attribute__((ext_vector_type(2)));
typedef __bf16 bf16x4 __attribute__((ext_vector_type(4)));

constexpr int PL_BM = 128, PL_BN = 128, PL_BK = 32, PL_K = 128, PL_NT = 256;
constexpr int PL_LDA = PL_BM + 1, PL_LDB = PL_BN + 4;
constexpr int PL_STAGE = PL_BK * (PL_LDA + PL_LDB);
constexpr size_t PL_LDS_BYTES = (size_t)(2 * PL_STAGE + 8 * 256) * sizeof(float);

__global__ __launch_bounds__(PL_NT) void ps_local_kernel(long npoints, int n_per_cloud, const int* __restrict__ idx,
                                                          const float* __restrict__ xyz, const float* __restrict__ Gm, long ldg,
                                                          const float* __restrict__ Am, const float* __restrict__ W1,
                                                          const float* __restrict__ b1, const float* __restrict__ Ww,
                                                          const float* __restrict__ bw, const float* __restrict__ scale,
                                                          const float* __restrict__ shift, float* __restrict__ out) {
    extern __shared__ __attribute__((aligned(16))) float lds[];
    float* wv = lds + 2 * PL_STAGE;
    const int tid = threadIdx.x, lane = tid & 63, wave = tid >> 6;
    const int wm = wave >> 1, wn = wave & 1;
    const long p0 = (long)blockIdx.x * 8;

#pragma unroll
    for (int e = tid; e < 8 * 256; e += PL_NT) {
        const int t = e & 15, s = (e >> 4) & 15, pl = e >> 8;
        const long i = p0 + pl;
        float v = 0.f;
        if (i < npoints) {
            const long j = (i / n_per_cloud) * n_per_cloud + idx[i * 16 + s];
            float acc = 0.f;
#pragma unroll
            for (int c = 0; c < 3; ++c) acc = __builtin_fmaf(xyz[j * 3 + c] - xyz[i * 3 + c], Ww[c * 16 + t], acc);
            acc = acc + bw[t];
            acc = acc * scale[t] + shift[t];
            v = fmaxf(acc, 0.f);
        }
        wv[e] = v;
    }

    const int kq = tid & 7;
    long gi[4], gj[4];
#pragma unroll
    for (int it = 0; it < 4; ++it) {
        const int r = (tid >> 3) + 32 * it;
        long i = p0 + (r >> 4);
        if (i >= npoints) i = npoints - 1;
        gi[it] = i;
        gj[it] = (i / n_per_cloud) * n_per_cloud + idx[i * 16 + (r & 15)];
    }
    float4 pg[4], pa[4], pb[4];
    auto load_tile = [&](int k0) {
#pragma unroll
        for (int it = 0; it < 4; ++it) {
            pg[it] = *reinterpret_cast<const float4*>(Gm + gj[it] * ldg + k0 + kq * 4);
            pa[it] = *reinterpret_cast<const float4*>(Am + gi[it] * PL_K + k0 + kq * 4);
        }
#pragma unroll
        for (int it = 0; it < 4; ++it) {
            const int e = tid + it * PL_NT;
            const int kr = e / (PL_BN / 4), nq = e % (PL_BN / 4);
            pb[it] = *reinterpret_cast<const float4*>(W1 + (size_t)(k0 + kr) * PL_BN + nq * 4);
        }
    };
    auto store_tile = [&](int stage) {
        float* As = lds + stage * PL_STAGE;
        float* Bs = As + PL_BK * PL_LDA;
#pragma unroll
        for (int it = 0; it < 4; ++it) {
            const int r = (tid >> 3) + 32 * it;
            As[(kq * 4 + 0) * PL_LDA + r] = fmaxf(pg[it].x - pa[it].x, 0.f);
            As[(kq * 4 + 1) * PL_LDA + r] = fmaxf(pg[it].y - pa[it].y, 0.f);
            As[(kq * 4 + 2) * PL_LDA + r] = fmaxf(pg[it].z - pa[it].z, 0.f);
            As[(kq * 4 + 3) * PL_LDA + r] = fmaxf(pg[it].w - pa[it].w, 0.f);
        }
#pragma unroll
        for (int it = 0; it < 4; ++it) {
            const int e = tid + it * PL_NT;
            const int kr = e / (PL_BN / 4), nq = e % (PL_BN / 4);
            *reinterpret_cast<float4*>(&Bs[kr * PL_LDB + nq * 4]) = pb[it];
        }
    };

    f32x16 acc[2][2];
#pragma unroll
    for (int i = 0; i < 2; ++i)
#pragma unroll
        for (int j = 0; j < 2; ++j)
#pragma unroll
            for (int r = 0; r < 16; ++r) acc[i][j][r] = 0.f;

    constexpr int NTILE = PL_K / PL_BK;
    load_tile(0);
    store_tile(0);
    load_tile(PL_BK);
    __syncthreads();
    const int fi = lane & 31, fk = lane >> 5;
#pragma unroll
    for (int t = 0; t < NTILE; ++t) {
        const float* As = lds + (t & 1) * PL_STAGE;
        const float* Bs = As + PL_BK * PL_LDA;
        if (t + 1 < NTILE) {
            store_tile((t + 1) & 1);
            if (t + 2 < NTILE) load_tile((t + 2) * PL_BK);
        }
#pragma unroll
        for (int kk = 0; kk < PL_BK; kk += 2) {
            float af[2], bf[2];
#pragma unroll
            for (int i = 0; i < 2; ++i) af[i] = As[(kk + fk) * PL_LDA + wm * 64 + i * 32 + fi];
#pragma unroll
            for (int j = 0; j < 2; ++j) bf[j] = Bs[(kk + fk) * PL_LDB + wn * 64 + j * 32 + fi];
#pragma unroll
            for (int i = 0; i < 2; ++i)
#pragma unroll
                for (int j = 0; j < 2; ++j)
                    acc[i][j] = __builtin_amdgcn_mfma_f32_32x32x2f32(af[i], bf[j], acc[i][j], 0, 0, 0);
        }
        __syncthreads();
    }

#pragma unroll
    for (int j = 0; j < 2; ++j) {
        const int c = wn * 64 + j * 32 + fi;
        const float bias = b1[c];
#pragma unroll
        for (int i = 0; i < 2; ++i) {
#pragma unroll
            for (int q = 0; q < 2; ++q) {
                const int pl = wm * 4 + i * 2 + q;
                float own[8], oth[8];
#pragma unroll
                for (int u = 0; u < 8; ++u) {
                    own[u] = fmaxf(acc[i][j][q * 8 + u] + bias, 0.f);
                    oth[u] = __shfl_xor(own[u], 32, 64);
                }
                float o[8];
#pragma unroll
                for (int t = 0; t < 8; ++t) o[t] = 0.f;
                const float* wp = wv + pl * 256 + fk * 8;
#pragma unroll
                for (int s = 0; s < 16; ++s) {
                    const int u = (s & 3) + 4 * (s >> 3);
                    const bool hi = (s >> 2) & 1;
                    const float xv = (hi == (fk != 0)) ? own[u] : oth[u];
                    const float4 w0 = *reinterpret_cast<const float4*>(wp + s * 16);
                    const float4 w1 = *reinterpret_cast<const float4*>(wp + s * 16 + 4);
                    o[0] = __builtin_fmaf(xv, w0.x, o[0]); o[1] = __builtin_fmaf(xv, w0.y, o[1]);
                    o[2] = __builtin_fmaf(xv, w0.z, o[2]); o[3] = __builtin_fmaf(xv, w0.w, o[3]);
                    o[4] = __builtin_fmaf(xv, w1.x, o[4]); o[5] = __builtin_fmaf(xv, w1.y, o[5]);
                    o[6] = __builtin_fmaf(xv, w1.z, o[6]); o[7] = __builtin_fmaf(xv, w1.w, o[7]);
                }
                const long pi = p0 + pl;
                if (pi < npoints) {
                    float* dst = out + pi * 2048 + c * 16 + fk * 8;
                    *reinterpret_cast<float4*>(dst) = make_float4(o[0], o[1], o[2], o[3]);
                    *reinterpret_cast<float4*>(dst + 4) = make_float4(o[4], o[5], o[6], o[7]);
                }
            }
        }
    }
}


template <int CTRL>
__device__ __forceinline__ float pl_quad(float v) {
    return __int_as_float(__builtin_amdgcn_update_dpp(0, __float_as_int(v), CTRL, 0xF, 0xF, true));
}

__device__ __forceinline__ void pl_lds_barrier() { asm volatile("s_waitcnt lgkmcnt(0)\n\ts_barrier" ::: "memory"); }

constexpr int PW_LDAR = PL_BK + 4;
constexpr int PW_ASTG = PL_BM * PW_LDAR;
constexpr int PW_LDB = PL_BN + 16;
constexpr int PW_WRES = PL_K * PW_LDB;
constexpr int PW_FLOATS = PW_WRES + 2 * PW_ASTG + 2 * 2048 + 2 * 1024 + 512;
constexpr size_t PW_LDS_BYTES = (size_t)PW_FLOATS * sizeof(float);

template <bool UNI, bool OUT16 = false>
__global__ __launch_bounds__(512) void ps_local_ws_kernel(long npoints, int n_per_cloud, const int* __restrict__ idx,
                                                           const float* __restrict__ xyz, const float* __restrict__ Gm, int ldg,
                                                           const float* __restrict__ Am, const float* __restrict__ W1,
                                                           const float* __restrict__ b1, const float* __restrict__ Ww,
                                                           const float* __restrict__ bw, const float* __restrict__ scale,
                                                           const float* __restrict__ shift,
                                                           std::conditional_t<OUT16, unsigned short, float>* __restrict__ out) {
    extern __shared__ __attribute__((aligned(16))) float lds[];
    float* wres = lds;
    float* astg = wres + PW_WRES;
    float* wvbuf = astg + 2 * PW_ASTG;
    float* abuf = wvbuf + 2 * 2048;
    float* cxbuf = abuf + 2 * 1024;
    const int lane = threadIdx.x & 63, wave = threadIdx.x >> 6;
    const int np = (int)npoints;
    const int ng_all = (np + 7) / 8;
    const bool xcd_map = ((gridDim.x & 7u) == 0) && (ng_all % 8 == 0) && ((int)gridDim.x <= ng_all);
    const int gstep = xcd_map ? (int)(gridDim.x >> 3) : (int)gridDim.x;
    const int g_first = xcd_map ? (int)(blockIdx.x & 7u) * (ng_all / 8) + (int)(blockIdx.x >> 3) : (int)blockIdx.x;
    const int ng = xcd_map ? ((int)(blockIdx.x & 7u) + 1) * (ng_all / 8) : ng_all;
    if (g_first >= ng) return;
    constexpr int NTILE = PL_K / PL_BK;

    if (wave >= 4) {
        const int ht = threadIdx.x - 256;
        const int kq = ht & 7;
        const int rho = ht >> 3;
        const int rq = rho >> 4, rs = 4 * (rho & 3) + ((rho >> 2) & 3);
        auto clampi = [&](int i) { return (UNI || i < np) ? i : np - 1; };
        auto cloud_base = [&](int i) { return (int)((unsigned)i / (unsigned)n_per_cloud) * n_per_cloud; };
        auto cloud_base_g = [&](int g) { return __builtin_amdgcn_readfirstlane((int)((unsigned)(g * 8) / (unsigned)n_per_cloud) * n_per_cloud); };
        const __amdgpu_buffer_rsrc_t r_idx = __builtin_amdgcn_make_buffer_rsrc(const_cast<int*>(idx), 0, (int)((unsigned)np * 64u), 0x00020000);
        const __amdgpu_buffer_rsrc_t r_g = __builtin_amdgcn_make_buffer_rsrc(const_cast<float*>(Gm), 0, (int)((unsigned)np * (unsigned)ldg * 4u), 0x00020000);
        const __amdgpu_buffer_rsrc_t r_a = __builtin_amdgcn_make_buffer_rsrc(const_cast<float*>(Am), 0, (int)((unsigned)np * 512u), 0x00020000);
        const __amdgpu_buffer_rsrc_t r_x = __builtin_amdgcn_make_buffer_rsrc(const_cast<float*>(xyz), 0, (int)((unsigned)np * 12u), 0x00020000);
        auto bload4 = [](__amdgpu_buffer_rsrc_t rs, int voff, int soff) -> float4 {
            const u32x4 r = __builtin_amdgcn_raw_buffer_load_b128(rs, voff, soff, 0);
            return make_float4(__uint_as_float(r[0]), __uint_as_float(r[1]), __uint_as_float(r[2]), __uint_as_float(r[3]));
        };
        int goff[4], goff_n[4];
        int ioff[4];
#pragma unroll
        for (int it = 0; it < 4; ++it) ioff[it] = ((2 * it + rq) * 16 + rs) * 4;
        auto rows_of = [&](int g, int (&go)[4]) {
            if constexpr (UNI) {
                const int cb = cloud_base_g(g);
#pragma unroll
                for (int it = 0; it < 4; ++it)
                    go[it] = ((cb + (int)__builtin_amdgcn_raw_buffer_load_b32(r_idx, ioff[it], g * 512, 0)) * ldg + kq * 4) * 4;
            } else {
#pragma unroll
                for (int it = 0; it < 4; ++it) {
                    const int i = clampi(g * 8 + 2 * it + rq);
                    go[it] = (cloud_base(i) + idx[i * 16 + rs]) * ldg + kq * 4;
                }
            }
        };
        int ri[4];
        auto rows_load = [&](int g) {
#pragma unroll
            for (int it = 0; it < 4; ++it) {
                if constexpr (UNI) ri[it] = (int)__builtin_amdgcn_raw_buffer_load_b32(r_idx, ioff[it], g * 512, 0);
                else ri[it] = idx[clampi(g * 8 + 2 * it + rq) * 16 + rs];
            }
        };
        auto rows_finish = [&](int g, int (&go)[4]) {
            if constexpr (UNI) {
                const int cb = cloud_base_g(g);
#pragma unroll
                for (int it = 0; it < 4; ++it) go[it] = ((cb + ri[it]) * ldg + kq * 4) * 4;
            } else {
#pragma unroll
                for (int it = 0; it < 4; ++it) go[it] = (cloud_base(clampi(g * 8 + 2 * it + rq)) + ri[it]) * ldg + kq * 4;
            }
        };
        float4 pg0[4], pg1[4];
        auto load_g = [&](float4 (&pg)[4], int k0, const int (&go)[4]) {
#pragma unroll
            for (int it = 0; it < 4; ++it) {
                if constexpr (UNI) pg[it] = bload4(r_g, go[it], k0 * 4);
                else pg[it] = *reinterpret_cast<const float4*>(Gm + go[it] + k0);
            }
        };
        auto store_a = [&](const float4 (&pg)[4], int stage, int k0, const float* ab) {
            float* As = astg + stage * PW_ASTG;
            float4 avs[4];
#pragma unroll
            for (int it = 0; it < 4; ++it) avs[it] = *reinterpret_cast<const float4*>(ab + (2 * it + rq) * PL_K + k0 + kq * 4);
            __builtin_amdgcn_sched_barrier(0);
#pragma unroll
            for (int it = 0; it < 4; ++it) {
                const float4 av = avs[it];
                const int r = rho + 32 * it;
                const f32x2 dlo = f32x2{pg[it].x, pg[it].y} - f32x2{av.x, av.y};
                const f32x2 dhi = f32x2{pg[it].z, pg[it].w} - f32x2{av.z, av.w};
                *reinterpret_cast<float4*>(&As[r * PW_LDAR + kq * 4]) =
                    make_float4(fmaxf(dlo.x, 0.f), fmaxf(dlo.y, 0.f), fmaxf(dhi.x, 0.f), fmaxf(dhi.y, 0.f));
            }
        };
        float4 arow;
        auto load_arow = [&](int g) {
            if constexpr (UNI) {
                arow = bload4(r_a, ht * 16, g * (8 * PL_K * 4));
            } else {
                const int i = clampi(g * 8 + (ht >> 5));
                arow = *reinterpret_cast<const float4*>(Am + (size_t)i * PL_K + (ht & 31) * 4);
            }
        };
        auto store_arow = [&](float* ab) { *reinterpret_cast<float4*>(ab + (ht >> 5) * PL_K + (ht & 31) * 4) = arow; };
        const int wt = ht & 15, wsn = (ht >> 4) & 15;
        const float ww0 = Ww[wt], ww1 = Ww[16 + wt], ww2 = Ww[32 + wt], wbw = bw[wt], wsc = scale[wt], wsh = shift[wt];
        int pj = 0, pi_ = 0;
        float px[6];
        auto wn_a = [&](int g) {
            if (ht < 128) {
                if constexpr (UNI) {
                    pi_ = g * 8 + (ht >> 4);
                    pj = cloud_base_g(g) + (int)__builtin_amdgcn_raw_buffer_load_b32(r_idx, ht * 4, g * 512, 0);
                } else {
                    pi_ = clampi(g * 8 + (ht >> 4));
                    pj = cloud_base(pi_) + idx[pi_ * 16 + (ht & 15)];
                }
            }
        };
        auto wn_b = [&]() {
            if (ht < 128) {
                if constexpr (UNI) {
                    const int oj = pj * 12, oi = pi_ * 12;
#pragma unroll
                    for (int c = 0; c < 3; ++c) {
                        px[c] = __uint_as_float(__builtin_amdgcn_raw_buffer_load_b32(r_x, oj, c * 4, 0));
                        px[3 + c] = __uint_as_float(__builtin_amdgcn_raw_buffer_load_b32(r_x, oi, c * 4, 0));
                    }
                } else {
#pragma unroll
                    for (int c = 0; c < 3; ++c) { px[c] = xyz[pj * 3 + c]; px[3 + c] = xyz[pi_ * 3 + c]; }
                }
            }
        };
        auto wn_c = [&]() {
            if (ht < 128) {
#pragma unroll
                for (int c = 0; c < 3; ++c) cxbuf[ht * 4 + c] = px[c] - px[3 + c];
                cxbuf[ht * 4 + 3] = 0.f;
            }
        };
        auto wn_d = [&](int g, float* wv, int U0, int U1) {
#pragma unroll
            for (int u = U0; u < U1; ++u) {
                float v = 0.f;
                if (UNI || g * 8 + u < np) {
                    const float4 cx = *reinterpret_cast<const float4*>(cxbuf + (u * 16 + wsn) * 4);
                    float acc = 0.f;
                    acc = __builtin_fmaf(cx.x, ww0, acc);
                    acc = __builtin_fmaf(cx.y, ww1, acc);
                    acc = __builtin_fmaf(cx.z, ww2, acc);
                    acc = acc + wbw;
                    acc = acc * wsc + wsh;
                    v = fmaxf(acc, 0.f);
                }
                wv[ht + u * PL_NT] = v;
            }
        };

#pragma unroll
        for (int it = 0; it < 16; ++it) {
            const int e = ht + it * PL_NT;
            const int kr = e >> 5, nq = e & 31;
            *reinterpret_cast<float4*>(&wres[kr * PW_LDB + nq * 4]) = *reinterpret_cast<const float4*>(W1 + (size_t)kr * PL_BN + nq * 4);
        }
        int g = g_first;
        rows_of(g, goff);
        load_arow(g);
        store_arow(abuf);
        wn_a(g);
        wn_b();
        wn_c();
        load_g(pg0, 0, goff);
        load_g(pg1, PL_BK, goff);
        __syncthreads();
        wn_d(g, wvbuf, 0, 8);
        store_a(pg0, 0, 0, abuf);
        load_g(pg0, 2 * PL_BK, goff);
        __syncthreads();
        int n = 0;
#ifdef PL_STAMPS
        unsigned long long h_sa = 0, h_rest = 0, h_bar = 0;
#define PL_H(v) const unsigned long long v = __builtin_readcyclecounter()
#else
#define PL_H(v)
#endif
        for (; g < ng; g += gstep, ++n) {
            const int gn = g + gstep;
            const bool has_next = gn < ng;
            const float* ab = abuf + (n & 1) * 1024;
            float* ab_n = abuf + ((n + 1) & 1) * 1024;
            PL_H(a0);
            store_a(pg1, 1, PL_BK, ab);
            PL_H(a1);
            load_g(pg1, 3 * PL_BK, goff);
            if (n > 0) wn_d(g, wvbuf + (n & 1) * 2048, 3, 6);
            if (has_next) { rows_load(gn); load_arow(gn); wn_a(gn); }
            PL_H(a2);
            pl_lds_barrier();
            PL_H(b0);
            store_a(pg0, 0, 2 * PL_BK, ab);
            PL_H(b1);
            if (n > 0) wn_d(g, wvbuf + (n & 1) * 2048, 6, 8);
            if (has_next) { rows_finish(gn, goff_n); load_g(pg0, 0, goff_n); store_arow(ab_n); wn_b(); }
            PL_H(b2);
            pl_lds_barrier();
            PL_H(c0);
            store_a(pg1, 1, 3 * PL_BK, ab);
            PL_H(c1);
            if (has_next) { load_g(pg1, PL_BK, goff_n); wn_c(); }
            PL_H(c2);
            pl_lds_barrier();
            PL_H(d0);
            if (has_next) {
                store_a(pg0, 0, 0, ab_n);
            }
            PL_H(d1);
            if (has_next) {
                load_g(pg0, 2 * PL_BK, goff_n);
                wn_d(gn, wvbuf + ((n + 1) & 1) * 2048, 0, 3);
            }
            PL_H(d2);
            pl_lds_barrier();
#ifdef PL_STAMPS
            { PL_H(e0); h_sa += (a1 - a0) + (b1 - b0) + (c1 - c0) + (d1 - d0); h_rest += (a2 - a1) + (b2 - b1) + (c2 - c1) + (d2 - d1);
              h_bar += (b0 - a2) + (c0 - b2) + (d0 - c2) + (e0 - d2); }
#endif
#pragma unroll
            for (int it = 0; it < 4; ++it) goff[it] = goff_n[it];
        }
#ifdef PL_STAMPS
        if (blockIdx.x == 5 && (threadIdx.x & 63) == 0) {
            unsigned long long* st = reinterpret_cast<unsigned long long*>(out + (size_t)npoints * 2048) + 20 + (wave - 4) * 4;
            st[0] = h_sa; st[1] = h_rest; st[2] = h_bar; st[3] = n;
        }
#endif
        return;
    }

    const int wm = wave >> 1, wn = wave & 1;
    const int lc = lane & 15, la = lane >> 4;
    float bias[4];
#pragma unroll
    for (int cb = 0; cb < 4; ++cb) bias[cb] = b1[wn * 64 + cb * 16 + lc];
    __syncthreads();
    __syncthreads();
    int n = 0;
#ifdef PL_STAMPS
    unsigned long long c_mma = 0, c_bar = 0, c_con = 0, c_bt[4] = {0, 0, 0, 0};
#define PL_T(v) const unsigned long long v = __builtin_readcyclecounter()
#else
#define PL_T(v)
#endif
    f32x4 o[4][4];
#pragma unroll
    for (int pt = 0; pt < 4; ++pt)
#pragma unroll
        for (int cb = 0; cb < 4; ++cb) o[pt][cb] = f32x4{0.f, 0.f, 0.f, 0.f};
    const __amdgpu_buffer_rsrc_t out_rsrc = __builtin_amdgcn_make_buffer_rsrc(out, 0, (int)((unsigned)np * (OUT16 ? 4096u : 8192u)), 0x00020000);
    int g_prev = 0;
    auto flush_tile = [&](int gp, int pt, int cb, bool live) {
        const int pi = gp * 8 + 4 * wm + pt;
        const int ch = wn * 64 + cb * 16 + lc;
        const unsigned off = (live && pi < np) ? ((unsigned)pi * 2048u + (unsigned)(ch * 16 + 4 * la)) * (OUT16 ? 2u : 4u) : 0xFFFFFFF0u;
        if constexpr (OUT16) {
            const bf16x4 h = {(__bf16)o[pt][cb][0], (__bf16)o[pt][cb][1], (__bf16)o[pt][cb][2], (__bf16)o[pt][cb][3]};
            __builtin_amdgcn_raw_buffer_store_b64(__builtin_bit_cast(u32x2, h), out_rsrc, (int)off, 0, 0);
        } else {
            __builtin_amdgcn_raw_buffer_store_b128(__builtin_bit_cast(u32x4, o[pt][cb]), out_rsrc, (int)off, 0, 0);
        }
    };
    for (int g = g_first; g < ng; g += gstep, ++n) {
        const bool have_prev = n > 0;
        f32x4 acc[4][4];
#pragma unroll
        for (int pt = 0; pt < 4; ++pt)
#pragma unroll
            for (int cb = 0; cb < 4; ++cb) acc[pt][cb] = f32x4{0.f, 0.f, 0.f, 0.f};
#pragma unroll
        for (int t = 0; t < NTILE; ++t) {
            const float* As = astg + (t & 1) * PW_ASTG;
            const float* Bs = wres + (t * PL_BK) * PW_LDB;
            PL_T(s0);
            float af[2][4], bf[2][4];
            auto load_frags = [&](int k0, float (&a)[4], float (&b)[4]) {
#ifdef PL_X_NOA
#pragma unroll
                for (int pt = 0; pt < 4; ++pt) a[pt] = 1.0f + lc;
#else
#pragma unroll
                for (int pt = 0; pt < 4; ++pt) a[pt] = As[(wm * 64 + pt * 16 + lc) * PW_LDAR + k0 + la];
#endif
#ifdef PL_X_NOB
#pragma unroll
                for (int cb = 0; cb < 4; ++cb) b[cb] = 0.5f + la;
#else
#pragma unroll
                for (int cb = 0; cb < 4; ++cb) b[cb] = Bs[(k0 + la) * PW_LDB + wn * 64 + cb * 16 + lc];
#endif
            };
            load_frags(0, af[0], bf[0]);
#pragma unroll
            for (int ks = 0; ks < PL_BK / 4; ++ks) {
                const int cur = ks & 1;
                if (ks + 1 < PL_BK / 4) load_frags(4 * (ks + 1), af[cur ^ 1], bf[cur ^ 1]);
#pragma unroll
                for (int pt = 0; pt < 4; ++pt)
#pragma unroll
                    for (int cb = 0; cb < 4; ++cb)
                        acc[pt][cb] = __builtin_amdgcn_mfma_f32_16x16x4f32(af[cur][pt], bf[cur][cb], acc[pt][cb], 0, 0, 0);
#ifndef PL_NOFLUSH
                if ((ks & 1) == 0) {
                    const int u = t * 4 + (ks >> 1);
                    flush_tile(g_prev, u >> 2, u & 3, have_prev);
                }
#endif
            }
            PL_T(s1);
            pl_lds_barrier();
            PL_T(s2);
#ifdef PL_STAMPS
            c_mma += s1 - s0; c_bar += s2 - s1; c_bt[t] += s2 - s1;
#endif
        }
        PL_T(p0s);
        const float* wv = wvbuf + (n & 1) * 2048;
#pragma unroll
        for (int pt = 0; pt < 4; ++pt) {
            float bw[4];
#pragma unroll
            for (int b = 0; b < 4; ++b) bw[b] = wv[(4 * wm + pt) * 256 + (4 * b + la) * 16 + lc];
#pragma unroll
            for (int cb = 0; cb < 4; ++cb) o[pt][cb] = f32x4{0.f, 0.f, 0.f, 0.f};
#pragma unroll
            for (int b = 0; b < 4; ++b)
#pragma unroll
                for (int cb = 0; cb < 4; ++cb)
                    o[pt][cb] = __builtin_amdgcn_mfma_f32_16x16x4f32(bw[b], fmaxf(acc[pt][cb][b] + bias[cb], 0.f), o[pt][cb], 0, 0, 0);
        }
        g_prev = g;
#ifdef PL_STAMPS
        { PL_T(p2s); c_con += p2s - p0s; }
#endif
    }
#pragma unroll
    for (int u = 0; u < 16; ++u) flush_tile(g_prev, u >> 2, u & 3, n > 0);
#ifdef PL_STAMPS
    if (blockIdx.x == 5 && lane == 0) {
        unsigned long long* st = reinterpret_cast<unsigned long long*>(out + (size_t)npoints * 2048) + wave * 5;
        st[0] = c_mma; st[1] = c_bar; st[2] = 0; st[3] = c_con; st[4] = n;
        unsigned long long* sb = reinterpret_cast<unsigned long long*>(out + (size_t)npoints * 2048) + 40 + wave * 4;
        sb[0] = c_bt[0]; sb[1] = c_bt[1]; sb[2] = c_bt[2]; sb[3] = c_bt[3];
    }
#endif
}

}

using namespace dispu;

template <bool OUT16>
static int pw_launch(long npoints, int n_per_cloud, const int* idx, const float* xyz, const float* G, long ldg, const float* A, const float* W1,
                     const float* b1, const float* Ww, const float* bw, const float* scale, const float* shift,
                     std::conditional_t<OUT16, unsigned short, float>* out, hipStream_t stream) {
    const long max_pts = 262144;
    if (n_per_cloud > max_pts) return (int)hipErrorInvalidValue;
    const long per = npoints <= max_pts ? npoints : (max_pts / n_per_cloud) * (long)n_per_cloud;
    for (long p0 = 0; p0 < npoints; p0 += per) {
        const long np = (npoints - p0 < per) ? npoints - p0 : per;
        const long ngroups = (np + 7) / 8;
        const unsigned grid = (unsigned)(ngroups < 256 ? ngroups : 256);
        const bool uni = (n_per_cloud % 8) == 0 && (np % 8) == 0 && np * ldg * 4 < 0x7fffffffL;
        if (uni)
            hipLaunchKernelGGL((ps_local_ws_kernel<true, OUT16>), dim3(grid), dim3(512), PW_LDS_BYTES, stream, np, n_per_cloud, idx + p0 * 16,
                               xyz + p0 * 3, G + p0 * ldg, (int)ldg, A + p0 * PL_K, W1, b1, Ww, bw, scale, shift, out + p0 * 2048);
        else
            hipLaunchKernelGGL((ps_local_ws_kernel<false, OUT16>), dim3(grid), dim3(512), PW_LDS_BYTES, stream, np, n_per_cloud, idx + p0 * 16,
                               xyz + p0 * 3, G + p0 * ldg, (int)ldg, A + p0 * PL_K, W1, b1, Ww, bw, scale, shift, out + p0 * 2048);
    }
    return 0;
}

DISPU_EXPORT int dispu_ps_local(long npoints, int n_per_cloud, int k, int c, const int* idx, const float* xyz, const float* G,
                                long ldg, const float* A, const float* W1, const float* b1, const float* Ww, const float* bw,
                                const float* scale, const float* shift, float* out, void* stream) {
    if (npoints < 0 || n_per_cloud <= 0 || k != 16 || c != 128 || ldg < 128 || (ldg & 3) || npoints * ldg > 0x7fffffffL) return (int)hipErrorInvalidValue;
    if ((((uintptr_t)G) | ((uintptr_t)A) | ((uintptr_t)W1) | ((uintptr_t)out)) & 15) return (int)hipErrorInvalidValue;
    if (npoints == 0) return 0;
    const int mode = 1;
    static DevOnce attr;      
    if (attr.needed()) {
        hipError_t e = hipFuncSetAttribute(reinterpret_cast<const void*>(ps_local_kernel), hipFuncAttributeMaxDynamicSharedMemorySize,
                                           (int)PL_LDS_BYTES);
        if (e != hipSuccess) return (int)e;
        e = hipFuncSetAttribute(reinterpret_cast<const void*>(ps_local_ws_kernel<false>), hipFuncAttributeMaxDynamicSharedMemorySize,
                                (int)PW_LDS_BYTES);
        if (e != hipSuccess) return (int)e;
        e = hipFuncSetAttribute(reinterpret_cast<const void*>(ps_local_ws_kernel<true>), hipFuncAttributeMaxDynamicSharedMemorySize,
                                (int)PW_LDS_BYTES);
        if (e != hipSuccess) return (int)e;
        attr.done();
    }
    if (mode == 0) {
        hipLaunchKernelGGL(ps_local_kernel, dim3((unsigned)((npoints + 7) / 8)), dim3(PL_NT), PL_LDS_BYTES, (hipStream_t)stream, npoints,
                           n_per_cloud, idx, xyz, G, ldg, A, W1, b1, Ww, bw, scale, shift, out);
    } else {
        const int rc = pw_launch<false>(npoints, n_per_cloud, idx, xyz, G, ldg, A, W1, b1, Ww, bw, scale, shift, out, (hipStream_t)stream);
        if (rc) return rc;
    }
    return (int)hipGetLastError();
}

DISPU_EXPORT int dispu_ps_local_bf16(long npoints, int n_per_cloud, int k, int c, const int* idx, const float* xyz, const float* G,
                                     long ldg, const float* A, const float* W1, const float* b1, const float* Ww, const float* bw,
                                     const float* scale, const float* shift, void* out, void* stream) {
    if (npoints < 0 || n_per_cloud <= 0 || k != 16 || c != 128 || ldg < 128 || (ldg & 3) || npoints * ldg > 0x7fffffffL) return (int)hipErrorInvalidValue;
    if ((((uintptr_t)G) | ((uintptr_t)A) | ((uintptr_t)W1) | ((uintptr_t)out)) & 15) return (int)hipErrorInvalidValue;
    if (npoints == 0) return 0;
    static DevOnce attr;
    if (attr.needed()) {
        DISPU_TRY(hipFuncSetAttribute(reinterpret_cast<const void*>(ps_local_ws_kernel<false, true>), hipFuncAttributeMaxDynamicSharedMemorySize,
                                      (int)PW_LDS_BYTES));
        DISPU_TRY(hipFuncSetAttribute(reinterpret_cast<const void*>(ps_local_ws_kernel<true, true>), hipFuncAttributeMaxDynamicSharedMemorySize,
                                      (int)PW_LDS_BYTES));
        attr.done();
    }
    const int rc = pw_launch<true>(npoints, n_per_cloud, idx, xyz, G, ldg, A, W1, b1, Ww, bw, scale, shift, reinterpret_cast<unsigned short*>(out),
                                   (hipStream_t)stream);
    if (rc) return rc;
    return (int)hipGetLastError();
}
```

### dis-pu_amd/generator.py

```python
import collections
import contextlib
import math

import numpy as np
import torch

from . import _lib

K_NEIGH = 16
GROWTH = 24
DENSE_BLOCKS = 4
BN_EPS = 1e-3


def gen_grid(up_ratio):
    sq = int(math.sqrt(up_ratio)) + 1
    for i in range(sq, 0, -1):
        if up_ratio % i == 0:
            num_x, num_y = i, up_ratio // i
            break
    gx = np.linspace(-0.2, 0.2, num_x, dtype=np.float32)
    gy = np.linspace(-0.2, 0.2, num_y, dtype=np.float32)
    x, y = np.meshgrid(gx, gy)
    return np.stack([x, y], -1).reshape(-1, 2).astype(np.float32)


def _off(t, o):
    return _lib.C.c_void_p(t.data_ptr() + 4 * o)


Path = collections.namedtuple("Path", "stem heads in_chain attention local after add3 nl_late")


class _Opts(object):
    patch_num_point = 256
    up_ratio = 4


def linear_profile_name(plan, batch, M, K, N):
    tf = lambda v: "true" if v else "false"
    tiled = [l for l in plan if l[0] == "tiled"]
    if tiled:
        _, _, _, bm, bn, bk, tb, edge, epi = tiled[0]
        return "linear<%d, %d, 2, 2, %d, %s, %s, %d>[%dx%dx%d]" % (bm, bn, bk, tf(tb), tf(edge), epi, M * batch, K, N)
    if plan:
        return "linear_skinny<%d, %s>[%dx%dx%d]" % (plan[-1][3], tf(plan[-1][4]), M, K, N)
    return "linear"


class Generator(object):

    MAX_POINTS = 2048 * 256

    def __init__(self, opts=None, is_training=False, name="Generator", params=None, device=None, dtype="f32"):
        if dtype not in ("f32", "bf16"):
            raise ValueError("Generator dtype must be 'f32' or 'bf16', got %r" % (dtype,))
        if dtype == "bf16" and is_training:
            raise ValueError("Generator(dtype='bf16') is the inference mode; mixed-precision training is Trainer(dtype='bf16')")
        self.dtype = dtype
        self.opts = opts if opts is not None else _Opts()
        self.is_training = is_training
        self.name = name
        self.num_point = int(self.opts.patch_num_point)
        self.up_ratio = int(self.opts.up_ratio)
        if self.up_ratio != 4:
            raise NotImplementedError("the shipped generator graph is built for up_ratio 4 (DisPU/configs.py)")
        self.out_num_point = self.num_point * self.up_ratio
        self.device = torch.device(device if device is not None else "cuda:0")
        if self.device.type == "cuda" and self.device.index is None:
            self.device = torch.device("cuda", torch.cuda.current_device())
        self.P = {}
        self._ws = {}
        self.profile = None
        self.fused_local = True
        self.fused_attention = True
        self.fused_project = True
        self.split_bf16 = False
        self._planes = {}
        self._aft_bt = None
        self.branches = True
        self._aux = None
        self.fused_heads = True
        self.keep_intermediates = False
        self.chain_inputs = True
        self.return_views = False
        self.fine_out = None
        self._trainer = None
        if params is not None:
            self.load_params(params)

    def load_params(self, params):
        dev = self.device
        if self.is_training:
            from .train import Trainer, TrainOpts
            topts = TrainOpts()
            for k in dir(self.opts):
                if not k.startswith("_"):
                    setattr(topts, k, getattr(self.opts, k))
            self._trainer = Trainer(opts=topts, params=params, device=dev)
            self.P = self._trainer.P
            return
        self.P = {k: torch.from_numpy(np.ascontiguousarray(v, np.float32)).to(dev) for k, v in params.items()}
        self._planes = {}
        bn = "refine/PointShuffle/weight_net/wconv0/bn/"
        g, b = params[bn + "gamma"].astype(np.float64), params[bn + "beta"].astype(np.float64)
        mu, var = params[bn + "moving_mean"].astype(np.float64), params[bn + "moving_variance"].astype(np.float64)
        scale = g / np.sqrt(var + BN_EPS)
        self.bn_scale = torch.from_numpy(scale.astype(np.float32)).to(dev)
        self.bn_shift = torch.from_numpy((b - mu * scale).astype(np.float32)).to(dev)
        self.grid = torch.from_numpy(gen_grid(self.up_ratio)).to(dev)
        w1 = self.P["generator/upshuffle_0/conv1/weights"]
        self.w_up_feat = w1[:480].contiguous()
        self.w_up_grid = w1[480:482].contiguous()
        w0 = self.P["refine/PointShuffle/conv0/weights"]
        self.w_c0_feat = w0[6:134].contiguous()
        nlp = "refine/PointShuffle/PointShuffle/"
        self.w_up3 = torch.cat([self.P[nlp + "conv_kv/weights"], self.P[nlp + "conv_query/weights"], self.w_c0_feat], dim=1).contiguous()
        self.b_up3 = torch.cat([self.P[nlp + "conv_kv/biases"], self.P[nlp + "conv_query/biases"],
                                torch.zeros(128, dtype=torch.float32, device=dev)]).contiguous()
        wsk = self.P["refine/PointShuffle/skip/weights"]
        self.w_skip_pad = torch.cat([wsk, torch.zeros((10, wsk.shape[1]), dtype=torch.float32, device=dev)], dim=0).contiguous()
        if self.dtype == "bf16":
            w = self.P["refine/PointShuffle/after_conv/weights"]
            bt = torch.empty((256, 2048), dtype=torch.bfloat16, device=dev)
            _lib.check(_lib.lib().dispu_bf16_pack(2048, 256, _lib.ptr(w), 256, 1, _lib.ptr(bt), _lib.stream_ptr(dev)), "dispu_bf16_pack")
            self._aft_bt = bt

    def _w(self, scope):
        return self.P[scope + "/weights"], self.P[scope + "/biases"]

    def _workspace(self, B, N):
        key = (B, N)
        ws = self._ws.get(key)
        if ws is not None:
            return ws
        dev, f32, i32 = self.device, torch.float32, torch.int32
        M = N * self.up_ratio
        rn, rm, k = B * N, B * M, K_NEIGH

        def E(*shape, dtype=f32):
            return torch.empty(shape, dtype=dtype, device=dev)

        ws = dict(
            feat=E(rn, 480), prep=E(rn, 48), prep_b=E(rn, 48), kidx=E(rn, k + 1, dtype=i32), h256=E(rn, 256),
            up256=E(rm, 256), up128=E(rm, 128), c256=E(rm, 256), c64=E(rm, 64), coarse=E(B, M, 3),
            psidx=E(rm, k, dtype=i32), up3=E(rm, 320), att=E(rm, 64), nl=E(rm, 256),
            skipin=torch.zeros((rm, 144), dtype=f32, device=dev), skip=E(rm, 256), am=E(rm, 128),
            fp=E(rm, 2048, dtype=torch.bfloat16 if self.dtype == "bf16" else f32), aft=E(rm, 256), agg=E(rm, 256),
            f256=E(rm, 256), f64=E(rm, 64), fine=E(B, M, 3))
        ws["kv"], ws["q"], ws["gm"] = ws["up3"][:, 0:128], ws["up3"][:, 128:192], ws["up3"][:, 192:320]
        self._ws[key] = ws
        return ws

    def _extra(self, store, key, shape, dtype=torch.float32):
        t = store.get(key)
        if t is None or t.numel() < math.prod(shape):
            t = store[key] = torch.empty(shape, dtype=dtype, device=self.device)
        return t

    def _call(self, name, fn, *args):
        if self.profile is None:
            _lib.check(fn(*args), name)
            return
        e0, e1 = torch.cuda.Event(enable_timing=True), torch.cuda.Event(enable_timing=True)
        e0.record()
        _lib.check(fn(*args), name)
        e1.record()
        self.profile.append((name, e0, e1))

    def _linear(self, st, X, K, W, bias, act, Y, N, M=None, ldx=None, ldw=None, ldy=None, batch=1, sx=0, sw=0, sy=0,
                transb=0, R1=None, R2=None, xoff=0, woff=0, yoff=0):
        M = X.shape[0] if M is None else M
        ldx = X.stride(0) if ldx is None else ldx
        ldw = W.stride(0) if ldw is None else ldw
        ldy = Y.stride(0) if ldy is None else ldy
        x, w, b, y, r1, r2 = _off(X, xoff), _off(W, woff), _lib.ptr(bias), _off(Y, yoff), _lib.ptr(R1), _lib.ptr(R2)
        ldr1 = R1.stride(0) if R1 is not None else 0
        ldr2 = R2.stride(0) if R2 is not None else 0
        name = "linear"
        if self.profile is not None:
            plan = _lib.linear_plan(batch, M, K, N, x, ldx, sx, w, ldw, sw, transb, b, None, None, act, y, ldy, sy, r1, ldr1, 0, r2, ldr2, 0,
                                    None, 0, 0)
            name = linear_profile_name(plan, batch, M, K, N)
        self._call(name, _lib.lib().dispu_linear, batch, M, K, N, x, ldx, sx, w, ldw, sw, transb, b, act, y, ldy, sy, r1, ldr1, 0, r2, ldr2, 0, st)

    def __call__(self, inputs):
        return self.forward(inputs)

    @property
    def trainer(self):
        return self._trainer

    def path(self, B, N):
        bf16 = self.dtype == "bf16"
        if bf16 and (self.split_bf16 or not self.fused_local):
            raise ValueError("Generator(dtype='bf16') stores F' as bf16 in the fused local cell: it excludes split_bf16 and fused_local = False")
        M = N * self.up_ratio
        tiles = B * M % 128 == 0
        heads = bool(self.fused_heads and tiles)
        in_chain = bool(heads and self.chain_inputs)
        on_chip = self.fused_attention and M % 32 == 0
        if bf16:
            after = "bf16_stream" if tiles else "bf16s"
        elif self.split_bf16 and tiles:
            after = "x3"
        else:
            after = "plain" if in_chain else "residual"
        return Path(stem=N <= 256 and N % 2 == 0, heads=heads, in_chain=in_chain,
                    attention="project" if on_chip and self.fused_project else "flash" if on_chip else "gemm",
                    local="bf16" if bf16 else "fused" if self.fused_local else "pair", after=after,
                    add3=bf16 and not in_chain, nl_late=bool(self.branches and in_chain))

    def forward(self, inputs):
        if not self.P:
            raise RuntimeError("Generator has no parameters: call load_params() first")
        if self.is_training:
            coarse, fine = self._trainer.forward(inputs)
            return (coarse, fine) if self.return_views else (coarse.clone(), fine.clone())
        if not (isinstance(inputs, torch.Tensor) and inputs.is_cuda and inputs.dtype == torch.float32 and inputs.dim() == 3
                and inputs.shape[2] == 3):
            raise ValueError("Generator expects a float32 [B,N,3] tensor on a ROCm device")
        inputs = inputs.contiguous()
        B, N, _ = inputs.shape
        if N <= K_NEIGH:
            raise ValueError("Generator needs patches of at least %d points (the dense blocks take the k + 1 = %d nearest "
                             "neighbours of every point), got N = %d" % (K_NEIGH + 1, K_NEIGH + 1, N))
        chunk = max(1, self.MAX_POINTS // N)
        if B > chunk:
            if self.return_views:
                raise ValueError("return_views needs B <= %d at N = %d (one workspace)" % (chunk, N))
            outs = [self.forward(inputs[lo:lo + chunk]) for lo in range(0, B, chunk)]
            return torch.cat([o[0] for o in outs]), torch.cat([o[1] for o in outs])
        path = self.path(B, N)
        M = N * self.up_ratio
        fine = self.fine_out
        if fine is not None and not (isinstance(fine, torch.Tensor) and fine.device == inputs.device and fine.dtype == torch.float32
                                     and tuple(fine.shape) == (B, M, 3) and fine.is_contiguous()):
            raise ValueError("fine_out must be a contiguous float32 [%d, %d, 3] tensor on %s" % (B, M, inputs.device))
        ws = self._workspace(B, N)
        coarse, fine = ws["coarse"], ws["fine"] if fine is None else fine
        st = _lib.stream_ptr(inputs.device)
        self._features(ws, path, inputs, st)
        self._coarse_head(ws, path, B, N, st)
        ev_up3, ev_nl = self._non_local(ws, path, B, N, st)
        self._knn_skip(ws, B, M, st)
        self._join(ev_up3)
        self._local(ws, path, B, N, st)
        self._join(None if path.nl_late else ev_nl)
        self._after_conv(ws, path, B * M, st)
        self._join(ev_nl if path.nl_late else None)
        self._fine_head(ws, path, B * M, fine, st)
        return (coarse, fine) if self.return_views else (coarse.clone(), fine.clone())

    def _join(self, event):
        if event is not None:
            torch.cuda.current_stream(self.device).wait_event(event)

    def _chain(self, first, head):
        return [_lib.ptr(t) for scope in (first, head + "fc_layer0", head + "fc_layer1", head + "fc_layer2") for t in self._w(scope)]

    def _features(self, ws, path, inputs, st):
        L, ptr = _lib.lib(), _lib.ptr
        B, N, _ = inputs.shape
        rn, k1, feat = B * N, K_NEIGH + 1, ws["feat"]
        fe = "generator/feature_extraction_coarse/"
        wl0, bl0 = self._w(fe + "layer0")
        if not path.stem:
            self._call("layer0", L.dispu_linear_small_k, rn, 3, 24, ptr(inputs), 3, ptr(wl0), ptr(bl0), 0, _off(feat, 456), 480, st)
        col = 456
        for d in range(1, DENSE_BLOCKS + 1):
            pbuf, nxt = (ws["prep"], ws["prep_b"]) if d % 2 == 0 else (ws["prep_b"], ws["prep"])
            if d == 1:
                F, ldf, foff, C = feat, 480, 456, 24
            else:
                if not path.stem:
                    w, b = self._w(fe + "layer%d_prep" % d)
                    self._linear(st, feat, 480 - col, w, b, 1, pbuf, 48, xoff=col)
                F, ldf, foff, C = pbuf, 48, 0, 48
            convs = [ptr(t) for l in range(3) for t in self._w(fe + "layer%d/l%d" % (d, l))]
            width = 3 * GROWTH + C
            col -= width
            if path.stem:
                last = d == DENSE_BLOCKS
                wp, bp = (None, None) if last else self._w(fe + "layer%d_prep" % (d + 1))
                layer0 = (ptr(inputs), ptr(wl0), ptr(bl0), _off(feat, 456)) if d == 1 else (None, None, None, None)
                self._call("stem_block", L.dispu_stem_block, rn, N, C, _off(F, foff), ldf, k1, 1, *convs, _off(feat, col), 480,
                           ptr(ws["kidx"]) if self.keep_intermediates else None, ptr(wp), ptr(bp), 480 - col - width,
                           None if last else ptr(nxt), 48, *layer0, 480, st)
                continue
            nbf = L.dispu_knn_feat_scratch_bytes(B, N, N, C, k1)
            scratch = ptr(self._extra(ws, "knnf_scratch", (nbf,), torch.uint8)) if nbf else None
            self._call("knn_feat", L.dispu_knn_feat_strided_ws, B, N, N, C, k1, _off(F, foff), ldf, _off(F, foff), ldf, None, ptr(ws["kidx"]),
                       scratch, nbf, st)
            self._call("edge_dense_conv", L.dispu_edge_dense_conv, rn, N, C, _off(F, foff), ldf, ptr(ws["kidx"]), k1, 1, *convs,
                       _off(feat, col), 480, st)
        assert col == 0

    def _coarse_head(self, ws, path, B, N, st):
        L, ptr = _lib.lib(), _lib.ptr
        rm = B * N * self.up_ratio
        _, b1 = self._w("generator/upshuffle_0/conv1")
        conv2, cs = "generator/upshuffle_0/conv2", "generator/coarse_coordinate_regressor/"
        self._linear(st, ws["feat"], 480, self.w_up_feat, None, 0, ws["h256"], 256)
        if path.in_chain:
            self._call("mlp_chain[coarse]", L.dispu_mlp_chain_dup, B, N, self.up_ratio, 256, 128, 256, 64, ptr(ws["h256"]), 256, ptr(self.w_up_grid),
                       ptr(b1), ptr(self.grid), *self._chain(conv2, cs), ptr(ws["up128"]), 128, 0, None, 0, ptr(ws["coarse"]), 3, st)
            return
        self._call("dup_grid", L.dispu_dup_grid, B, N, 256, self.up_ratio, ptr(ws["h256"]), 256, ptr(self.w_up_grid), ptr(b1), ptr(self.grid),
                   ptr(ws["up256"]), 256, st)
        if path.heads:
            self._call("mlp_chain[coarse]", L.dispu_mlp_chain, rm, 256, 128, 256, 64, ptr(ws["up256"]), 256, *self._chain(conv2, cs),
                       ptr(ws["up128"]), 128, 0, None, 0, ptr(ws["coarse"]), 3, st)
        else:
            w, b = self._w(conv2)
            self._linear(st, ws["up256"], 256, w, b, 1, ws["up128"], 128)
            w, b = self._w(cs + "fc_layer0")
            self._linear(st, ws["up128"], 128, w, b, 1, ws["c256"], 256)
            w, b = self._w(cs + "fc_layer1")
            self._linear(st, ws["c256"], 256, w, b, 1, ws["c64"], 64)
            w, b = self._w(cs + "fc_layer2")
            self._call("coarse", L.dispu_linear_small_n, rm, 64, 3, ptr(ws["c64"]), 64, ptr(w), ptr(b), 0, None, 0, ptr(ws["coarse"]), 3, st)

    def _non_local(self, ws, path, B, N, st):
        L, ptr = _lib.lib(), _lib.ptr
        M, q, kv, sb = N * self.up_ratio, ws["q"], ws["kv"], st
        br, aux, ev_up3, ev_nl = self.branches, None, None, None
        if br:
            if self._aux is None:
                self._aux = (torch.cuda.Stream(device=self.device), torch.cuda.Event(), torch.cuda.Event(), torch.cuda.Event())
            aux, ev_fork, ev_up3, ev_nl = self._aux
            ev_fork.record(torch.cuda.current_stream(self.device))
            aux.wait_event(ev_fork)
            sb = _lib.C.c_void_p(aux.cuda_stream)
        with (torch.cuda.stream(aux) if br else contextlib.nullcontext()):
            self._linear(sb, ws["up128"], 128, self.w_up3, self.b_up3, 0, ws["up3"], 256)
            self._linear(sb, ws["up128"], 128, self.w_up3, self.b_up3[256:], 0, ws["up3"], 64, woff=256, yoff=256)
            if br:
                ev_up3.record(aux)
            w_bp, b_bp = self._w("refine/PointShuffle/PointShuffle/conv_back_project")
            if path.attention == "project":
                self._call("attention_project", L.dispu_attention_project, B, M, M, 64, ptr(q), 320, ptr(kv), 320, _off(kv, 64), 320, 0.125,
                           ptr(w_bp), ptr(b_bp), 256, ptr(ws["nl"]), 256, sb)
            elif path.attention == "flash":
                self._call("attention", L.dispu_attention, B, M, M, 64, ptr(q), 320, ptr(kv), 320, _off(kv, 64), 320, 0.125, ptr(ws["att"]), 64, sb)
            else:
                s = self._extra(self._ws, ("scores", B, N), (B, M, M))
                self._linear(sb, q, 64, kv, None, 0, s, M, M=M, ldx=320, ldw=320, ldy=M, batch=B, sx=M * 320, sw=M * 320, sy=M * M, transb=1)
                self._call("softmax", L.dispu_softmax_rows, B * M, M, 0.125, ptr(s), M, sb)
                self._linear(sb, s, M, kv, None, 0, ws["att"], 64, M=M, ldx=M, ldw=320, ldy=64, batch=B, sx=M * M, sw=M * 320, sy=M * 64, woff=64)
            if path.attention != "project":
                self._linear(sb, ws["att"], 64, w_bp, b_bp, 1, ws["nl"], 256)
            if br:
                ev_nl.record(aux)
        return ev_up3, ev_nl

    def _knn_skip(self, ws, B, M, st):
        L, ptr = _lib.lib(), _lib.ptr
        rm, k, coarse = B * M, K_NEIGH, ws["coarse"]
        nb = L.dispu_knn_xyz_scratch_bytes(B, M, M, k)
        scratch = ptr(self._extra(ws, "knn_scratch", (nb,), torch.uint8)) if nb else None
        self._call("knn_xyz", L.dispu_knn_xyz_ws, B, M, M, k, ptr(coarse), ptr(coarse), ptr(ws["psidx"]), None, scratch, nb, _lib.ARITH_PLAIN, st)
        self._call("skip_max", L.dispu_ps_skip_max, rm, M, k, 128, ptr(ws["psidx"]), ptr(coarse), ptr(ws["up128"]), 128, ptr(ws["skipin"]), 144, st)
        _, b = self._w("refine/PointShuffle/skip")
        self._linear(st, ws["skipin"], 144, self.w_skip_pad, b, 1, ws["skip"], 256)

    def _local(self, ws, path, B, N, st):
        L, ptr = _lib.lib(), _lib.ptr
        M, k, ps = N * self.up_ratio, K_NEIGH, "refine/PointShuffle/"
        rm, coarse, psidx, gm, am = B * M, ws["coarse"], ws["psidx"], ws["gm"], ws["am"]
        w0, b0 = self._w(ps + "conv0")
        self._call("ps_prep", L.dispu_ps_prep, rm, 128, ptr(coarse), ptr(w0), ptr(b0), ptr(gm), 320, ptr(am), 128, st)
        w1, b1 = self._w(ps + "conv1")
        wnet = [ptr(t) for t in self._w(ps + "weight_net/wconv0") + (self.bn_scale, self.bn_shift)]
        if path.local != "pair":
            name, fn = ("ps_local_bf16", L.dispu_ps_local_bf16) if path.local == "bf16" else ("ps_local", L.dispu_ps_local)
            self._call(name, fn, rm, M, k, 128, ptr(psidx), ptr(coarse), ptr(gm), 320, ptr(am), ptr(w1), ptr(b1), *wnet, ptr(ws["fp"]), st)
            return
        rows = rm * k
        flat = self._extra(self._ws, ("pair", B, N), (rows * 272,))
        x1, x2, wv = (t.view(rows, -1) for t in flat.split([rows * 128, rows * 128, rows * 16]))
        self._call("gather_sub_relu", L.dispu_ps_gather_sub_relu, rm, M, k, 128, ptr(psidx), ptr(gm), 320, ptr(am), 128, ptr(x1), 128, st)
        self._linear(st, x1, 128, w1, b1, 1, x2, 128)
        self._call("weight_net", L.dispu_ps_weight_net, rm, M, k, 16, ptr(psidx), ptr(coarse), *wnet, ptr(wv), st)
        self._call("point_matmul", L.dispu_ps_point_matmul, rm, k, 128, 16, ptr(x2), 128, ptr(wv), ptr(ws["fp"]), 2048, st)

    def _after_conv(self, ws, path, rm, st):
        L, ptr = _lib.lib(), _lib.ptr
        w, b = self._w("refine/PointShuffle/after_conv")
        fp, aft = ws["fp"], ws["aft"]
        if path.after == "bf16_stream":
            self._call("linear_bf16_stream[%dx2048x256]" % rm, L.dispu_linear_bf16_stream, rm, 2048, 256, ptr(fp), 2048, 1,
                       ptr(self._aft_bt), 2048, ptr(b), 1, ptr(aft), 256, 0, 1, 0, st)
        elif path.after == "bf16s":
            self._call("linear_bf16s[%dx2048x256]" % rm, L.dispu_linear_bf16s, 1, rm, 2048, 256, ptr(fp), 2048, 0, ptr(w), 256, 0, 0,
                       ptr(b), 1, ptr(aft), 256, 0, None, 0, 0, 1, st)
        elif path.after == "x3":
            pl = self._planes.get("after_conv")
            if pl is None:
                pl = torch.empty((3 * 2048 * 256,), dtype=torch.bfloat16, device=self.device)
                _lib.check(L.dispu_bf16x3_split_weights(2048, 256, ptr(w), 256, ptr(pl), st), "dispu_bf16x3_split_weights")
                self._planes["after_conv"] = pl
            skip, nl = (None, None) if path.in_chain else (ptr(ws["skip"]), ptr(ws["nl"]))
            self._call("linear_bf16x3[%dx2048x256]" % rm, L.dispu_linear_bf16x3, rm, 2048, 256, ptr(fp), 2048, ptr(pl), ptr(b), 1,
                       ptr(aft), 256, skip, 256, nl, 256, st)
        else:
            r1, r2 = (None, None) if path.after == "plain" else (ws["skip"], ws["nl"])
            self._linear(st, fp, 2048, w, b, 1, aft, 256, R1=r1, R2=r2)
        if path.add3:
            total = self._extra(ws, "sum", (rm, 256))
            self._call("add3", L.dispu_add3, rm * 256, ptr(aft), ptr(ws["skip"]), ptr(ws["nl"]), ptr(total), st)

    def _fine_head(self, ws, path, rm, fine, st):
        L, ptr = _lib.lib(), _lib.ptr
        agg, fs = "refine/PointShuffle/aggregation", "refine/fine_coordinate_regressor/"
        x, coarse = ws["sum"] if path.add3 else ws["aft"], ws["coarse"]
        if path.heads:
            tail = (ptr(ws["agg"]) if self.keep_intermediates else None, 256, 1, ptr(coarse), 3, ptr(fine), 3, st)
            if path.in_chain:
                self._call("mlp_chain[fine]", L.dispu_mlp_chain_sum3, rm, 256, 256, 256, 64, ptr(x), ptr(ws["skip"]), ptr(ws["nl"]), 256,
                           *self._chain(agg, fs), *tail)
            else:
                self._call("mlp_chain[fine]", L.dispu_mlp_chain, rm, 256, 256, 256, 64, ptr(x), 256, *self._chain(agg, fs), *tail)
            return
        w, b = self._w(agg)
        self._linear(st, x, 256, w, b, 1, ws["agg"], 256)
        w, b = self._w(fs + "fc_layer0")
        self._linear(st, ws["agg"], 256, w, b, 1, ws["f256"], 256)
        w, b = self._w(fs + "fc_layer1")
        self._linear(st, ws["f256"], 256, w, b, 1, ws["f64"], 64)
        w, b = self._w(fs + "fc_layer2")
        self._call("fine", L.dispu_linear_small_n, rm, 64, 3, ptr(ws["f64"]), 64, ptr(w), ptr(b), 1, ptr(coarse), 3, ptr(fine), 3, st)
```

### include/dispu_hip.h

```cpp
#ifndef DISPU_HIP_H
#define DISPU_HIP_H

#include <stddef.h>

#ifdef __cplusplus
extern "C" {
#endif

#define DISPU_ARITH_PLAIN 0
#define DISPU_ARITH_CONTRACT 1
#define DISPU_ARITH_PINNED_EXP 2
#define DISPU_KNN_LANE_PER_QUERY 4
#define DISPU_MESH_BRUTE_FORCE 8
#define DISPU_MESH_TILE 64

int dispu_version(void);
int dispu_event_record(void* event, void* stream);
int dispu_stream_wait_event(void* stream, void* event);
int dispu_memset_async(void* dst, int value, size_t bytes, void* stream);
const char* dispu_error_string(int code);


size_t dispu_fps_scratch_bytes(int b, int n, int m);
int dispu_fps(int b, int n, int m, const float* inp, float* temp, int* out, int arith, void* stream);
int dispu_fps_ws(int b, int n, int m, const float* inp, float* temp, size_t temp_bytes, int* out, int arith, void* stream);
size_t dispu_fps_segments_scratch_bytes(int C, const int* off_host, const int* moff_host);
int dispu_fps_segments(int C, const int* off, const int* moff, const int* off_host, const int* moff_host, const float* inp, void* temp,
                       size_t temp_bytes, int* out, int arith, void* stream);
size_t dispu_fps_cells_scratch_bytes(int C, const int* off_host, const int* moff_host, int cell);
int dispu_fps_cells(int C, const int* off, const int* moff, const int* off_host, const int* moff_host, const float* inp, void* scratch,
                    size_t scratch_bytes, int* out, int* status, int arith, int cell, void* stream);
int dispu_fps_cells_wanted(int n, int m);
size_t dispu_fps_segments_auto_scratch_bytes(int C, const int* off_host, const int* moff_host);
int dispu_fps_segments_auto(int C, const int* off, const int* moff, const int* off_host, const int* moff_host, const float* inp, void* temp,
                            size_t temp_bytes, int* out, int* status, int arith, void* stream);

int dispu_prob_sample(int b, int n, int m, const float* inp_p, const float* inp_r, float* temp, int* out, void* stream);

int dispu_gather_point(int b, int n, int m, const float* inp, const int* idx, float* out, void* stream);

int dispu_gather_point_grad(int b, int n, int m, const float* out_g, const int* idx, float* inp_g, void* stream);


int dispu_query_ball(int b, int n, int m, const float* radius, int nsample, const float* xyz1, const float* xyz2,
                     int* idx, int* pts_cnt, int arith, void* stream);

int dispu_group_point(int b, int n, int c, int m, int nsample, const float* points, const int* idx, float* out,
                      void* stream);

int dispu_group_point_grad(int b, int n, int c, int m, int nsample, const float* grad_out, const int* idx,
                           float* grad_points, void* stream);

int dispu_selection_sort(int b, int n, int m, int k, const float* dist, int* outi, float* out, void* stream);

int dispu_knn_point(int b, int n, int m, int c, int k, const float* xyz1, const float* xyz2, float* val, int* idx,
                    void* stream);

int dispu_knn_feat(int b, int n, int m, int c, int k, const float* points, const float* queries, float* dist,
                   int* idx, void* stream);

int dispu_knn_feat_strided(int b, int n, int m, int c, int k, const float* points, int ldp, const float* queries,
                           int ldq, float* dist, int* idx, void* stream);
size_t dispu_knn_feat_scratch_bytes(int b, int n, int m, int c, int k);
int dispu_knn_feat_strided_ws(int b, int n, int m, int c, int k, const float* points, int ldp, const float* queries, int ldq,
                              float* dist, int* idx, void* scratch, size_t scratch_bytes, void* stream);


int dispu_knn_xyz(int b, int n, int m, int k, const float* support, const float* query, int* idx, float* dist,
                  int arith, void* stream);
size_t dispu_knn_xyz_scratch_bytes(int b, int n, int m, int k);
int dispu_knn_xyz_ws(int b, int n, int m, int k, const float* support, const float* query, int* idx, float* dist, void* scratch,
                     size_t scratch_bytes, int arith, void* stream);


int dispu_three_nn(int b, int n, int m, const float* xyz1, const float* xyz2, float* dist, int* idx, int arith,
                   void* stream);
int dispu_three_interpolate(int b, int m, int c, int n, const float* points, const int* idx, const float* weight,
                            float* out, void* stream);
int dispu_three_interpolate_grad(int b, int n, int c, int m, const float* grad_out, const int* idx,
                                 const float* weight, float* grad_points, void* stream);


int dispu_nn_distance(int b, int n, const float* xyz1, int m, const float* xyz2, float* dist1, int* idx1, float* dist2,
                      int* idx2, int arith, void* stream);
int dispu_nn_distance_grad(int b, int n, const float* xyz1, int m, const float* xyz2, const float* grad_dist1,
                           const int* idx1, const float* grad_dist2, const int* idx2, float* grad_xyz1,
                           float* grad_xyz2, void* stream);


size_t dispu_approx_match_scratch_bytes(int b, int n, int m);
int dispu_approx_match(int b, int n, int m, const float* xyz1, const float* xyz2, float* match, float* temp, int arith,
                       void* stream);
int dispu_approx_match_ws(int b, int n, int m, const float* xyz1, const float* xyz2, float* match, float* temp,
                          size_t temp_bytes, int arith, void* stream);
int dispu_approx_match_levels_ws(int b, int n, int m, const float* xyz1, const float* xyz2, float* temp, size_t temp_bytes, int arith,
                                 void* stream);
size_t dispu_emd_loss_grad_scratch_bytes(int b, int n, int m);
int dispu_emd_loss_grad(int b, int n, int m, const float* xyz1, const float* xyz2, float* temp, const float* radius, float coef,
                        float* cost, float* dpred, float* scratch, size_t scratch_bytes, int arith, void* stream);
int dispu_match_cost(int b, int n, int m, const float* xyz1, const float* xyz2, const float* match, float* cost, int arith,
                     void* stream);
size_t dispu_match_cost_scratch_bytes(int b, int n, int m);
int dispu_match_cost_ws(int b, int n, int m, const float* xyz1, const float* xyz2, const float* match, float* cost,
                        float* scratch, int arith, void* stream);
int dispu_match_cost_grad(int b, int n, int m, const float* xyz1, const float* xyz2, const float* match, float* grad1,
                          float* grad2, int arith, void* stream);
size_t dispu_match_cost_grad_scratch_bytes(int b, int n, int m);
int dispu_match_cost_grad_ws(int b, int n, int m, const float* xyz1, const float* xyz2, const float* match, float* grad1,
                             float* grad2, float* scratch, int arith, void* stream);


int dispu_linear(int batch, int M, int K, int N, const float* X, long ldx, long sx, const float* W, long ldw, long sw,
                 int transb, const float* bias, int act, float* Y, long ldy, long sy, const float* R1, long ldr1,
                 long sr1, const float* R2, long ldr2, long sr2, void* stream);
int dispu_linear_bn(int batch, int M, int K, int N, const float* X, long ldx, long sx, const float* W, long ldw, long sw,
                    int transb, const float* bias, const float* scale, const float* shift, int act, float* Y, long ldy,
                    long sy, const float* R1, long ldr1, long sr1, const float* R2, long ldr2, long sr2, void* stream);
int dispu_linear_tile(int batch, int M, int N);
int dispu_linear_tile2(int batch, int M, int K, int N, int transb);
void dispu_debug_linear_tile(int code);
#define DISPU_LINEAR_PLAN_INTS 21
int dispu_linear_plan(int batch, int M, int K, int N, const float* X, long ldx, long sx, const float* W, long ldw, long sw,
                      int transb, const float* bias, const float* scale, const float* shift, int act, const float* Y, long ldy,
                      long sy, const float* R1, long ldr1, long sr1, const float* R2, long ldr2, long sr2, const float* Mk,
                      long ldm, int mcols, int* plan);
int dispu_linear_small_k(long rows, int K, int N, const float* X, long ldx, const float* W, const float* bias, int act,
                         float* Y, long ldy, void* stream);
int dispu_linear_small_n(long rows, int K, int N, const float* X, long ldx, const float* W, const float* bias, int mode,
                         const float* R, long ldr, float* Y, long ldy, void* stream);
int dispu_edge_dense_conv(int npoints, int n_per_cloud, int C, const float* F, long ldf, const int* idx, int ldi, int ioff,
                          const float* W0, const float* b0, const float* W1, const float* b1, const float* W2,
                          const float* b2, float* Y, long ldy, void* stream);
int dispu_stem_block(int npoints, int n_per_cloud, int C, const float* F, long ldf, int ksel, int ioff, const float* W0, const float* b0,
                     const float* W1, const float* b1, const float* W2, const float* b2, float* Y, long ldy, int* idx_out, const float* Wp,
                     const float* bp, int k_old, float* P, long ldp, const float* xyz, const float* Wl, const float* bl, float* Lout,
                     long ldl, void* stream);
int dispu_edge_dense_conv_valu(int npoints, int n_per_cloud, int C, const float* F, long ldf, const int* idx, int ldi,
                               int ioff, const float* W0, const float* b0, const float* W1, const float* b1,
                               const float* W2, const float* b2, float* Y, long ldy, void* stream);
int dispu_dup_grid(int nclouds, int n, int co, int up, const float* H, long ldh, const float* Wg, const float* bias,
                   const float* grid, float* Y, long ldy, void* stream);
int dispu_ps_prep(long rows, int co, const float* xyz, const float* W0, const float* bias, float* G, long ldg, float* A,
                  long lda, void* stream);
int dispu_ps_gather_sub_relu(long rows, int n_per_cloud, int k, int c, const int* idx, const float* G, long ldg,
                             const float* A, long lda, float* X1, long ldx1, void* stream);
int dispu_ps_skip_max(long rows, int n_per_cloud, int k, int cf, const int* idx, const float* xyz, const float* feat,
                      long ldf, float* out, long ldo, void* stream);
int dispu_ps_weight_net(long rows, int n_per_cloud, int k, int t_n, const int* idx, const float* xyz, const float* Ww,
                        const float* bw, const float* scale, const float* shift, float* wv, void* stream);
int dispu_ps_point_matmul(long rows, int k, int c, int t_n, const float* X2, long ldx2, const float* wv, float* out,
                          long ldo, void* stream);
int dispu_ps_local(long npoints, int n_per_cloud, int k, int c, const int* idx, const float* xyz, const float* G, long ldg,
                   const float* A, const float* W1, const float* b1, const float* Ww, const float* bw, const float* scale,
                   const float* shift, float* out, void* stream);
int dispu_ps_local_bf16(long npoints, int n_per_cloud, int k, int c, const int* idx, const float* xyz, const float* G, long ldg,
                        const float* A, const float* W1, const float* b1, const float* Ww, const float* bw, const float* scale,
                        const float* shift, void* out, void* stream);
int dispu_attention(int b, int m, int nk, int d, const float* Q, long ldq, const float* K, long ldk, const float* V,
                    long ldv, float scale, float* O, long ldo, void* stream);
int dispu_attention_project(int b, int m, int nk, int d, const float* Q, long ldq, const float* K, long ldk, const float* V,
                            long ldv, float scale, const float* W, const float* bias, int n_out, float* Y, long ldy,
                            void* stream);
int dispu_attention_fwd_lse(int b, int m, int nk, int d, const float* Q, long ldq, const float* K, long ldk, const float* V,
                            long ldv, float scale, float* O, long ldo, float* lse2, void* stream);
int dispu_attention_bwd(int b, int m, int nk, int d, const float* Q, long ldq, const float* K, long ldk, const float* V, long ldv,
                        float scale, const float* O, long ldo, const float* lse2, const float* dO, long lddo, float* dQ, long lddq,
                        float* dK, long lddk, float* dV, long lddv, float* dvec, void* stream);
int dispu_softmax_rows(long rows, int n, float mul, float* S, long lds, void* stream);

int dispu_mlp_chain(long rows, int K0, int N1, int N2, int N3, const float* X, long ldx, const float* W1, const float* b1,
                    const float* W2, const float* b2, const float* W3, const float* b3, const float* W4, const float* b4,
                    float* Y1, long ldy1, int mode, const float* R, long ldr, float* out, long ldo, void* stream);
int dispu_mlp_chain_sum3(long rows, int K0, int N1, int N2, int N3, const float* X, const float* X2, const float* X3, long ldx,
                         const float* W1, const float* b1, const float* W2, const float* b2, const float* W3, const float* b3,
                         const float* W4, const float* b4, float* Y1, long ldy1, int mode, const float* R, long ldr, float* out, long ldo,
                         void* stream);
int dispu_mlp_chain_dup(int nclouds, int n, int up, int K0, int N1, int N2, int N3, const float* H, long ldh, const float* Wg,
                        const float* bg, const float* grid, const float* W1, const float* b1, const float* W2, const float* b2,
                        const float* W3, const float* b3, const float* W4, const float* b4, float* Y1, long ldy1, int mode, const float* R,
                        long ldr, float* out, long ldo, void* stream);

int dispu_group_center(long rows, int ns, int c, float* grouped, const float* center, void* stream);
int dispu_sa_fused(int b, int n, int m, int ns, int c, const float* xyz, const float* new_xyz, const float* points, const int* idx,
                   int nl, const float* const* W, const float* const* bias, const float* const* scale, const float* const* shift,
                   const int* cout, float* out, void* stream);
int dispu_edge_conv_fused(int b, int n, int k, int c, const float* feat, long ldf, const int* idx, int ldi, int nl,
                          const float* const* W, const float* const* bias, const float* const* scale, const float* const* shift,
                          const int* cout, int act_last, float* out, void* stream);
int dispu_pool_nsample(long rows, int ns, int c, int mode, const float* X, const float* gxyz, float* out, void* stream);
int dispu_l2_normalize_rows(long rows, int c, const float* X, float* out, void* stream);
int dispu_scale_add(long n, const float* x, float alpha, const float* y, float* out, void* stream);
int dispu_idw_weights(long rows, const float* dist, float* weight, void* stream);
int dispu_edge_feature(long rows, int n_per_cloud, int k, int c, const float* F, long ldf, const int* idx, int ldi, int ioff,
                       float* out, long ldo, void* stream);
int dispu_row_mean_max(int b, int n, const float* x, float* mean, float* mx, void* stream);
int dispu_repulsion(long rows, int n_per_cloud, int ns, int use_l1, float h, const float* pred, const int* idx, float* out,
                    void* stream);

int dispu_linear_bf16(int batch, int M, int K, int N, const float* X, long ldx, long sx, const float* W, long ldw, long sw,
                      int transb, const float* bias, int act, float* Y, long ldy, long sy, const float* R1, long ldr1, long sr1,
                      const float* R2, long ldr2, long sr2, void* stream);
long dispu_linear_tn_bf16_scratch_floats(int batch, int M, int K, int N);
int dispu_linear_tn_bf16(int batch, int M, int K, int N, const float* X, long ldx, long sx, const float* Z, long ldz, long sz,
                         float* out, long ldo, long so, int accumulate, float* dbias, float* scratch, long scratch_floats,
                         void* stream);
int dispu_bf16x3_split_weights(int K, int N, const float* W, long ldw, void* planes, void* stream);
int dispu_linear_bf16x3(int M, int K, int N, const float* X, long ldx, const void* planes, const float* bias, int act, float* Y,
                        long ldy, const float* R1, long ldr1, const float* R2, long ldr2, void* stream);
void dispu_debug_x3_kernel(int which);
long dispu_linear_tn_scratch_floats(int batch, int M, int K, int N);
int dispu_linear_tn(int batch, int M, int K, int N, const float* X, long ldx, long sx, const float* Z, long ldz, long sz,
                    float* out, long ldo, long so, int accumulate, float* dbias, float* scratch, long scratch_floats,
                    void* stream);
#define DISPU_LINEAR_TN_PLAN_INTS 12
int dispu_linear_tn_plan(int batch, int M, int K, int N, const float* X, long ldx, long sx, const float* Z, long ldz, long sz,
                         const float* out, long ldo, long so, int accumulate, const float* dbias, const float* scratch,
                         long scratch_floats, int* plan);
#define DISPU_LINEAR_TN_BF16_PLAN_INTS 6
int dispu_linear_tn_bf16_plan(int batch, int M, int K, int N, const void* X, long ldx, long sx, const void* Z, long ldz, long sz,
                              const float* out, long ldo, long so, int accumulate, const float* dbias, const float* scratch,
                              long scratch_floats, int storage, int* plan);
#define DISPU_LINEAR_TN_BF16_STREAM_PLAN_INTS 4
int dispu_linear_tn_bf16_stream_plan(int M, int K, int N, const void* X, long ldx, const void* Z, long ldz, int storage, const float* out,
                                     long ldo, int accumulate, const float* dbias, const float* scratch, long scratch_floats, int* plan);
typedef struct dispu_tn_reduce_desc {
    const float* part; float* out; float* dbias;
    long ldo, stride;
    int K, N, splits, rows_p;
    int accumulate, bias_accumulate, assoc, reserved;
} dispu_tn_reduce_desc;
int dispu_tn_defer(dispu_tn_reduce_desc* desc);
int dispu_tn_reduce_grouped(int count, const dispu_tn_reduce_desc* table_host, const dispu_tn_reduce_desc* table_device, void* stream);
long dispu_act_bias_grad_scratch_floats(long rows, int n);
int dispu_act_bias_grad(long rows, int n, const float* dY, long lddy, const float* Y, long ldy, int act, float* dZ, long lddz,
                        float* dbias, int accumulate, float* scratch, long scratch_floats, void* stream);
int dispu_max_k(long rows, int ns, int c, const float* X, long ldx, float* out, long ldo, void* stream);
int dispu_max_k_grad(long rows, int ns, int c, const float* X, long ldx, const float* Y, long ldy, const float* dY, long lddy,
                     float* dX, long lddx, int accumulate, void* stream);
int dispu_max_k_grad_tail(long rows, int ns, int c, int tail, const float* X, long ldx, const float* Y, long ldy, const float* dY,
                          long lddy, float* dX, long lddx, void* stream);
int dispu_edge_feature_grad(long rows, int n_per_cloud, int k, int c, const float* dE, long lde, const int* idx, int ldi,
                            int ioff, float* dF, long lddf, void* stream);
int dispu_dup_sum_grad(int nclouds, int n, int co, int up, const float* dZ, long lddz, float* dH, long lddh, void* stream);
int dispu_ps_group(long rows, int n_per_cloud, int k, int cf, const int* idx, const float* xyz, const float* feat, long ldf,
                   float* gf, long ldg, void* stream);
int dispu_ps_group_grad(long rows, int n_per_cloud, int k, int cf, const int* idx, const float* dgf, long ldg, float* dxyz,
                        float* dfeat, long lddf, void* stream);
int dispu_ps_point_matmul_grad(long rows, int k, int c, int t_n, const float* X2, long ldx2, const float* wv, const float* dout,
                               long ldo, float* dX2, long lddx2, float* dwv, void* stream);
int dispu_softmax_rows_grad(long rows, int n, float mul, const float* P, long ldp, float* dP, long lddp, void* stream);
long dispu_bn_scratch_bytes(long rows, int c);
int dispu_bn_train(long rows, int c, const float* X, long ldx, const float* gamma, const float* beta, float eps, float decay,
                   int act, float* Y, long ldy, float* stats, float* moving_mean, float* moving_var, void* scratch,
                   long scratch_bytes, void* stream);
int dispu_bn_train_grad(long rows, int c, const float* X, long ldx, const float* Y, long ldy, const float* dY, long lddy,
                        const float* stats, const float* gamma, int act, float* dX, long lddx, float* dgamma, float* dbeta,
                        float* sums, void* scratch, long scratch_bytes, void* stream);
int dispu_sigmoid_offset(long total, const float* z, const float* base, float* out, void* stream);
int dispu_sigmoid_offset_grad(long total, const float* z, const float* dout, float* dz, float* dbase, void* stream);
int dispu_repulsion_grad(long rows, int n_per_cloud, int ns, float h, float scale, const float* pred, const int* idx,
                         float* dpred, void* stream);
int dispu_add3(long total, const float* a, const float* b, const float* c, float* out, void* stream);
int dispu_linear_splitk_finish(long rows, int n, int nparts, const float* part, long part_stride, const float* bias, int act, float* Y,
                               long ldy, void* stream);
int dispu_fill_rows(int b, int n, const float* val, float mul, float* out, void* stream);
int dispu_adam(long total, float* p, const float* g, float* m, float* v, float lr_t, float beta1, float beta2, float eps,
               float gscale, void* stream);

int dispu_linear_masked(int batch, int M, int K, int N, const float* X, long ldx, long sx, const float* W, long ldw, long sw,
                        int transb, const float* bias, int act, float* Y, long ldy, long sy, const float* R1, long ldr1, long sr1,
                        const float* Mk, long ldm, int mcols, void* stream);
int dispu_linear_bf16_masked(int batch, int M, int K, int N, const float* X, long ldx, long sx, const float* W, long ldw, long sw,
                             int transb, const float* bias, int act, float* Y, long ldy, long sy, const float* R1, long ldr1, long sr1,
                             const float* Mk, long ldm, int mcols, void* stream);
int dispu_linear_bf16_plan(int batch, int M, int N, int splits);
int dispu_bf16_pack(int rows, int cols, const float* W, long ldw, int transpose, void* out, void* stream);
long dispu_linear_tn_bf16_stream_scratch_floats(int M, int K, int N);
int dispu_linear_tn_bf16_stream(int M, int K, int N, const void* X, long ldx, const void* Z, long ldz, int storage, float* out, long ldo,
                                int accumulate, float* dbias, float* scratch, long scratch_floats, void* stream);
int dispu_linear_bf16_stream(int M, int K, int N, const void* X, long ldx, int x_bf16, const void* Bt, long ldb, const float* bias, int act,
                             void* Y, long ldy, int y_bf16, int splits, long y_split, void* stream);
int dispu_mlp_chain_stash(long rows, int K0, int N1, int N2, int N3, const float* X, long ldx, const float* W1, const float* b1,
                          const float* W2, const float* b2, const float* W3, const float* b3, const float* W4, const float* b4,
                          float* Y1, long ldy1, float* Y2, long ldy2, float* Y3, long ldy3, float* Z, long ldz, int mode,
                          const float* R, long ldr, float* out, long ldo, void* stream);
int dispu_mlp_chain_grad(long rows, int K0, int N1, int N2, const float* dZ, long lddz, const float* W4, const float* Wt3,
                         const float* Wt2, const float* Wt1, const float* Y3, long ldy3, const float* Y2, long ldy2,
                         const float* Y1, long ldy1, const float* R, long ldr, const float* R2, long ldr2, float* D3, long ldd3,
                         float* D2, long ldd2, float* D1, long ldd1, const float* Ma, const float* Mb, const float* Mc, long ldm, float* Da, float* Db,
                         float* Dc, long ldd0, void* stream);
int dispu_ps_local_grad(long npoints, int n_per_cloud, const int* idx, const float* xyz, const float* Gm, long ldg, const float* Am,
                        const float* W1, const float* b1, const float* W1t, const float* Ww, const float* bw, const float* scale,
                        const float* shift, const float* dF, float* dz1, float* dwv, float* dG, float* dAneg, void* stream);
int dispu_mask3(long rows, int n, const float* dY, long lddy, const float* Y1, long ld1, const float* Y2, long ld2, const float* Y3,
                long ld3, float* o1, float* o2, float* o3, long ldo, void* stream);
long dispu_ps_wnet_scratch_bytes(long rows);
int dispu_ps_wnet_bn_stats(long rows, int n_per_cloud, int k, int t_n, const int* idx, const float* xyz, const float* Ww, const float* bw,
                           const float* gamma, const float* beta, float eps, float decay, float* stats, float* scale, float* shift,
                           float* moving_mean, float* moving_var, void* scratch, long scratch_bytes, void* stream);
int dispu_ps_wnet_grad(long rows, int n_per_cloud, int k, int t_n, const int* idx, const float* xyz, const float* Ww, const float* bw,
                       const float* stats, const float* scale, const float* shift, const float* gamma, const float* dwv, float* dWw,
                       float* dbw, float* dgamma, float* dbeta, float* dxyz, float* sums, void* scratch, long scratch_bytes, void* stream);
int dispu_knn_invert(int b, int n, int k, const int* idx, int* off, int* inv, void* stream);
int dispu_ps_conv0_gather_grad(long rows, int n_per_cloud, int k, int c, const int* idx, const int* off, const int* inv, const float* dh0,
                               long ldz, const float* Gm, long ldgm, const float* Am, long ldam, float* dG, long ldg, float* dAneg, long lda,
                               void* stream);
int dispu_ps_prep_grad(long rows, int co, const float* xyz, const float* W0, const float* dG, long ldg, const float* dAneg, long lda,
                       float* dxyz, float* dW0, void* stream);
int dispu_ps_skip_max_grad(long rows, int n_per_cloud, int k, int cf, const int* idx, const float* xyz, const float* feat, long ldf,
                           const float* gmax, long ldm, const float* dgmax, long ldd, float* dxyz, float* dfeat, long lddf,
                           int feat_is_relu, void* stream);
long dispu_edge_dense_conv_grad_scratch_floats(int npoints, int C);
int dispu_edge_dense_conv_grad(int npoints, int n_per_cloud, int C, const float* F, long ldf, const int* idx, int ldi, int ioff,
                               const float* W0, const float* b0, const float* W1, const float* b1, const float* W2, const float* b2,
                               const float* dOut, long lddo, float* dF, long lddf, float* dW0, float* db0, float* dW1, float* db1,
                               float* dW2, float* db2, float* scratch, long scratch_floats, void* stream);
int dispu_edge_dense_conv_grad_partials(int npoints, int n_per_cloud, int C, const float* F, long ldf, const int* idx, int ldi, int ioff,
                                        const float* W0, const float* b0, const float* W1, const float* b1, const float* W2,
                                        const float* b2, const float* dOut, long lddo, float* dF, long lddf, float* scratch,
                                        long scratch_floats, void* stream);
int dispu_edge_dense_conv_grad_reduce(int npoints, int C, const float* scratch, long scratch_floats, float* dW0, float* db0, float* dW1,
                                      float* db1, float* dW2, float* db2, void* stream);
int dispu_chamfer_loss_grad(int b, int n_gt, const float* gt, int n_pred, const float* pred, const float* d_gt, const int* i_gt,
                            const float* d_pred, const int* i_pred, const float* radius, float coef, float* value, float* dpred,
                            void* stream);
int dispu_pu_loss_finalize(const float* cd, const float* rep, long nrep, float wf, float rep_w, float* out, void* stream);
int dispu_step_meters(int b, int n_gt, int n_pred, const float* d_gt_c, const float* d_pred_c, const float* d_gt_f,
                      const float* d_pred_f, const float* radius, const float* loss_out, float* row, void* stream);
int dispu_repulsion_loss_grad(long rows, int n_per_cloud, int ns, float h, float scale, const float* pred, const int* idx, float* out,
                              float* dpred, void* stream);
int dispu_uniform_loss_grad(int b, int n, int npoint, int nlevels, const int* ns, const float* levels, const float* pcd,
                            const int* seeds, float* partial, float* dpcd, int* idx_out, int* cnt_out, int arith, void* stream);
int dispu_pu_loss_finalize_u(const float* cd, const float* rep, long nrep, float wf, float rep_w, const float* upart, int nlevels,
                             long nu, float uniform_w, float* out, void* stream);
int dispu_pu_loss_finalize_e(const float* cd, const float* rep, long nrep, float wf, float rep_w, const float* upart, int nlevels,
                             long nu, float uniform_w, const float* emd_cost, const float* radius, int b, int m, float emd_w,
                             float* out, void* stream);
int dispu_transpose_batched(int count, const int* desc, const float* src, float* dst, void* stream);
int dispu_linear_bf16s(int batch, int M, int K, int N, const void* X, long ldx, long sx, const float* W, long ldw, long sw, int transb,
                       const float* bias, int act, void* Y, long ldy, long sy, const float* R1, long ldr1, long sr1, int storage,
                       void* stream);
int dispu_linear_tn_bf16s(int batch, int M, int K, int N, const void* X, long ldx, long sx, const void* Z, long ldz, long sz, float* out,
                          long ldo, long so, int accumulate, float* dbias, float* scratch, long scratch_floats, int storage, void* stream);
int dispu_ps_gather_sub_relu_bf16(long rows, int n_per_cloud, int k, int c, const int* idx, const float* G, long ldg, const float* A,
                                  long lda, void* X1, long ldx1, void* stream);
int dispu_ps_point_matmul_grad_relu_s(long rows, int k, int c, int t_n, const void* X2, long ldx2, const float* wv, const void* dout,
                                      long ldo, void* dX2, long lddx2, float* dwv, int bf16_storage, void* stream);
int dispu_ps_conv0_gather_grad_s(long rows, int n_per_cloud, int k, int c, const int* idx, const int* off, const int* inv, const void* dh0,
                                 long ldz, int dh0_bf16, const float* Gm, long ldgm, const float* Am, long ldam, float* dG, long ldg,
                                 float* dAneg, long lda, void* stream);
int dispu_ps_point_matmul_grad_relu(long rows, int k, int c, int t_n, const float* X2, long ldx2, const float* wv, const float* dout,
                                    long ldo, float* dX2, long lddx2, float* dwv, void* stream);

int dispu_augment(int b, int n, const float* in, const float* noise, const float* rot, const float* scale,
                  const float* shift, float* out, void* stream);

#define DISPU_SAMPLER_MAX_ROUNDS 4096
#define DISPU_SAMPLER_MAX_G 8192
int dispu_sample_batch(int L, int G, int P, const float* gt_data, const float* input_data, const int* perm, int start, int B,
                       unsigned long long seed, int epoch, float jitter_sigma, float jitter_clip, int augment, float* input, float* gt,
                       float* radius, int* status, int* idx_out, float* rot_out, float* scale_out, float* noise_out,
                       unsigned int* raw_out, void* stream);

int dispu_knn_patch(int b, int n, int m, int k, const float* cloud, const float* queries, int* idx, void* stream);
int dispu_normalize_patches(int b, int n, const float* in, float* out, float* centroid, float* furthest, void* stream);
int dispu_denormalize_patches(int b, int m, const float* in, const float* centroid, const float* furthest, float* out,
                              void* stream);
int dispu_knn_patch_segments(int C, const int* off, const int* qoff, const int* off_host, const int* qoff_host, int k, const float* cloud,
                             const float* queries, int* idx, void* stream);
int dispu_normalize_segments(int C, const int* off, const int* off_host, const float* in, float* out, float* centroid, float* furthest,
                             void* stream);

int dispu_point_to_mesh(int n, const float* points, int F, const float* tris, const int* face_ids, const float* tile_box, float* dist,
                        float* proj, int* face, int flags, void* stream);
int dispu_disk_count(int S, int n, int R, const float* seeds, const float* points, const float* radii, long long* offsets,
                     void* stream);
int dispu_disk_fill(int S, int n, int R, const float* seeds, const float* points, const float* radii, const long long* offsets,
                    int* members, void* stream);
size_t dispu_disk_uniformity_scratch_bytes(int S, int R);
int dispu_disk_uniformity(int S, int R, int n, const float* points, const long long* offsets, const int* members, const double* radii,
                          const double* pct, int N, void* scratch, size_t scratch_bytes, double* out, void* stream);
size_t dispu_geodesic_scratch_bytes(int S, int window_cap);
int dispu_geodesic_hash_slots(int window_cap);
int dispu_geodesic_distances(int S, const int* seed_face, const double* seed_bary, const double* verts, const int* faces, const int* twin,
                             const double* edge_geo, const int* pseudo, const long long* fan_off, const int* fan, int n, const float* points,
                             const int* point_face, const long long* cand_off, const int* cand, double max_dist, int window_cap,
                             void* scratch, size_t scratch_bytes, double* dist, int* status, void* stream);
int dispu_geodesic_disk_count(int S, int R, const long long* cand_off, const double* dist, const float* radii, long long* offsets,
                              void* stream);
int dispu_geodesic_disk_fill(int S, int R, const long long* cand_off, const int* cand, const double* dist, const float* radii,
                             const long long* offsets, int* members, void* stream);
int dispu_row_mean_std(int b, int n, const float* x, double* out, void* stream);

int dispu_mesh_sample(int V, int F, const float* verts, const int* faces, const double* cum, int count, unsigned long long seed,
                      float* points, int* face, double* bary, void* stream);
#define DISPU_POISSON_MAX_N 49152
#define DISPU_POISSON_MAX_ROUNDS 256
size_t dispu_poisson_disk_scratch_bytes(int b, int n);
int dispu_poisson_disk_keep(int b, int n, const float* points, const float* radius, unsigned char* keep, int* count, void* scratch,
                            size_t scratch_bytes, int* status, void* stream);
int dispu_poisson_disk_select(int b, int n, int m, int steps, const float* points, const float* r_hi, int* idx, float* r_out,
                              int* count_out, void* scratch, size_t scratch_bytes, int* status, void* stream);
int dispu_sort_rows_i32(int b, int k, int* idx, void* stream);
#define DISPU_POISSON_CELLS_NONFINITE 4
size_t dispu_poisson_cells_scratch_bytes(int C, long long total_n);
int dispu_poisson_cells_keep(int C, const int* off, const int* off_host, const float* points, const float* radius, unsigned char* keep,
                             int* count, int* rounds, void* scratch, size_t scratch_bytes, int* status, void* stream);
int dispu_poisson_cells_select(int C, const int* off, const int* moff, const int* off_host, const int* moff_host, int steps,
                               const float* points, const float* r_hi, int* idx, float* r_out, int* count_out, int* rounds,
                               void* scratch, size_t scratch_bytes, int* status, void* stream);

#define DISPU_RADIX_TILE 2048
size_t dispu_radix_sort_scratch_bytes(long long n);
int dispu_radix_sort_pairs(long long n, int bits, const unsigned long long* keys_in, const unsigned int* vals_in,
                           unsigned long long* keys_out, unsigned int* vals_out, void* scratch, size_t scratch_bytes, void* stream);
#define DISPU_GRID_NONFINITE 1
#define DISPU_GRID_AXIS_X 2
#define DISPU_GRID_AXIS_Y 3
#define DISPU_GRID_AXIS_Z 4
#define DISPU_GRID_TOO_MANY_POINTS 5
size_t dispu_grid_subsample_scratch_bytes(long long n, int fdim, int ldim);
int dispu_grid_subsample_plan(long long n, const float* points, float dl, void* scratch, size_t scratch_bytes, int* m_out, int* status_out,
                              double* grid_out, void* stream);
int dispu_grid_subsample_emit(long long n, int m, int fdim, int ldim, const float* points, const float* features, const int* classes,
                              void* scratch, size_t scratch_bytes, float* out_points, float* out_features, int* out_classes, void* stream);

size_t dispu_pca_normals_scratch_bytes(int C, const int* off_host, int k);
int dispu_pca_normals_segments(int C, const int* off, const int* off_host, int k, const float* cloud, int orient_mode, const float* orient,
                               float* normal, float* variation, int* idx_out, int* status, void* scratch, size_t scratch_bytes,
                               void* stream);

size_t dispu_knn_mean_dist_scratch_bytes(int C, const int* off_host, int k);
int dispu_knn_mean_dist_segments(int C, const int* off, const int* off_host, int k, const float* cloud, float* mean_dist, int* status,
                                 void* scratch, size_t scratch_bytes, void* stream);
size_t dispu_radius_count_scratch_bytes(int C, const int* off_host);
int dispu_radius_count_segments(int C, const int* off, const int* off_host, float radius, int cap, const float* cloud, int* count,
                                int* status, void* scratch, size_t scratch_bytes, void* stream);
int dispu_outlier_threshold_segments(int C, const int* off, const int* off_host, const float* mean_dist, const int* status, double ratio,
                                     double* stats, void* stream);
size_t dispu_compact_scratch_bytes(int C, const int* off_host);
int dispu_compact_segments(int C, const int* off, const int* off_host, const float* cloud, int rule, const void* src, const double* stats,
                           int min_neighbors, const int* status, float* out_points, int* out_index, int* new_off, void* scratch,
                           size_t scratch_bytes, void* stream);

#define DISPU_CLUSTER_HEAD_INTS 16
size_t dispu_cluster_scratch_bytes(int C, const int* off_host);
int dispu_cluster_segments(int C, const int* off, const int* off_host, float eps, int min_points, const float* cloud, int* labels,
                           unsigned char* core_or_null, int* sizes_or_null, int* nclusters, int* status, void* scratch,
                           size_t scratch_bytes, void* stream);
int dispu_cluster_select_segments(int C, const int* off, const int* off_host, const int* labels, const int* sizes, const int* nclusters,
                                  const int* status, int keep, int min_size, int* flags, void* stream);

size_t dispu_knn_cross_scratch_bytes(int C, const int* qoff_host, const int* roff_host);
int dispu_knn_cross_segments(int C, const int* qoff, const int* qoff_host, const int* roff, const int* roff_host, int k,
                             const float* queries, const float* refs, int* idx_out, float* d2_out, int* status, void* scratch,
                             size_t scratch_bytes, void* stream);
int dispu_transfer_attributes_segments(int C, const int* qoff, const int* qoff_host, const int* roff, const int* roff_host, int k, int mode,
                                       const float* queries, const float* refs, int F, const float* feat, float* out_feat,
                                       const int* labels, int* out_labels, int* status, void* scratch, size_t scratch_bytes, void* stream);

#define DISPU_ORIENT_HOST_ROUNDS 1
#define DISPU_ORIENT_PROFILE_FLOATS 8
size_t dispu_orient_consistent_scratch_bytes(int C, const int* off_host, int k);
int dispu_orient_consistent_segments(int C, const int* off, const int* off_host, int k, const float* points, const float* normal_in,
                                     const int* neighbors, int vote, int flags, float* normal_out, unsigned char* flip, int* component,
                                     int* n_components, int* status, void* scratch, size_t scratch_bytes, float* profile_host,
                                     void* stream);

size_t dispu_mls_project_scratch_bytes(int C, const int* qoff_host, const int* roff_host);
int dispu_mls_project_segments(int C, const int* qoff, const int* qoff_host, const int* roff, const int* roff_host, int k, double support,
                               int iterations, const float* queries, const float* refs, float* out, int* idx_out, int* status,
                               void* scratch, size_t scratch_bytes, void* stream);

size_t dispu_signed_distance_scratch_bytes(int C, const int* qoff_host, const int* roff_host);
int dispu_signed_distance_segments(int C, const int* qoff, const int* qoff_host, const int* roff, const int* roff_host, int k, double support,
                                   const float* queries, const float* refs, const float* normals, float* out, int* status, void* scratch,
                                   size_t scratch_bytes, void* stream);

size_t dispu_icp_scratch_bytes(int C, const int* qoff_host, const int* roff_host);
int dispu_icp_segments(int C, const int* qoff, const int* qoff_host, const int* roff, const int* roff_host, int mode, int iterations,
                       float max_d2, double tolerance, const float* source, const float* target, const float* target_normals,
                       const double* init, double* transform, float* aligned, int* corr, int* inliers, double* rmse, int* iters,
                       int* flag, int* status, void* scratch, size_t scratch_bytes, void* stream);
int dispu_rigid_apply_segments(int C, const int* off, const int* off_host, const float* points, const double* transform, float* out,
                               void* stream);

#define DISPU_LATTICE_NONFINITE 1
#define DISPU_LATTICE_RANGE 2
size_t dispu_lattice_voxels_scratch_bytes(long long n);
int dispu_lattice_voxels(long long n, const float* points, float voxel, int band, unsigned long long* occ_out, int* count_host,
                         int* status_host, void* scratch, size_t scratch_bytes, void* stream);
size_t dispu_lattice_dilate_scratch_bytes(long long nocc, int band);
int dispu_lattice_dilate(long long nocc, const unsigned long long* occ, int band, unsigned long long* act_out, long long* count_host,
                         void* scratch, size_t scratch_bytes, void* stream);
size_t dispu_lattice_corners_scratch_bytes(long long nvox);
int dispu_lattice_corners(long long nvox, const unsigned long long* act, unsigned long long* lat_out, int* corner_out,
                          long long* count_host, void* scratch, size_t scratch_bytes, void* stream);
int dispu_lattice_positions(long long nlat, const unsigned long long* lat, float voxel, float* pos_out, void* stream);
size_t dispu_contour_count_scratch_bytes(long long nvox, long long nlat);
int dispu_contour_count(long long nvox, long long nlat, const int* corner, const float* values, unsigned* slot_number, unsigned* tri_start,
                        long long* nverts_host, long long* nfaces_host, void* scratch, size_t scratch_bytes, void* stream);
int dispu_contour_emit(long long nvox, long long nlat, float voxel, const unsigned long long* lat, const int* corner, const float* values,
                       const unsigned* slot_number, const unsigned* tri_start, long long nverts, long long nfaces, float* verts_out,
                       int* faces_out, void* stream);

#ifdef __cplusplus
}
#endif
#endif
```

Measured before the change: 36.05 million points/s.

## Fuse PointShuffle ps_prep into up3 linear epilogue and xyz-forming local kernel

```diff
diff --git a/dis-pu_amd/_lib.py b/dis-pu_amd/_lib.py
--- a/dis-pu_amd/_lib.py
+++ b/dis-pu_amd/_lib.py
@@ -115,6 +115,8 @@
     "dispu_debug_linear_tile": (None, [_i]),
     "dispu_linear_plan": (_i, [_i, _i, _i, _i, _vp, _l, _l, _vp, _l, _l, _i, _vp, _vp, _vp, _i, _vp, _l, _l, _vp, _l, _l, _vp, _l, _l, _vp, _l, _i,
                                _vp]),
+    "dispu_linear_xyz3": (_i, [_i, _i, _i, _vp, _l, _vp, _l, _vp, _vp, _l, _vp, _vp, _l, _i, _i, _vp]),
+    "dispu_linear_xyz3_plan": (_i, [_i, _i, _i, _vp, _l, _vp, _l, _vp, _vp, _l, _vp, _vp, _l, _i, _i, _vp]),
     "dispu_linear_bf16_plan": (_i, [_i, _i, _i, _i]),
     "dispu_sa_fused": (_i, [_i, _i, _i, _i, _i, _vp, _vp, _vp, _vp, _i, _vp, _vp, _vp, _vp, _vp, _vp, _vp]),
     "dispu_edge_conv_fused": (_i, [_i, _i, _i, _i, _vp, _l, _vp, _i, _i, _vp, _vp, _vp, _vp, _vp, _i, _vp, _vp]),
@@ -140,6 +142,8 @@
     "dispu_ps_point_matmul": (_i, [_l, _i, _i, _i, _vp, _l, _vp, _vp, _l, _vp]),
     "dispu_ps_local": (_i, [_l, _i, _i, _i, _vp, _vp, _vp, _l, _vp, _vp, _vp, _vp, _vp, _vp, _vp, _vp, _vp]),
     "dispu_ps_local_bf16": (_i, [_l, _i, _i, _i, _vp, _vp, _vp, _l, _vp, _vp, _vp, _vp, _vp, _vp, _vp, _vp, _vp]),
+    "dispu_ps_local_xyz": (_i, [_l, _i, _i, _i, _vp, _vp, _vp, _l, _vp, _vp, _vp, _vp, _vp, _vp, _vp, _vp, _vp]),
+    "dispu_ps_local_xyz_bf16": (_i, [_l, _i, _i, _i, _vp, _vp, _vp, _l, _vp, _vp, _vp, _vp, _vp, _vp, _vp, _vp, _vp]),
     "dispu_knn_patch": (_i, [_i, _i, _i, _i, _vp, _vp, _vp, _vp]),
     "dispu_normalize_patches": (_i, [_i, _i, _vp, _vp, _vp, _vp, _vp]),
     "dispu_denormalize_patches": (_i, [_i, _i, _vp, _vp, _vp, _vp, _vp]),
@@ -305,7 +309,8 @@
 
 
 _TAPE = None
-_NO_TAPE = ("dispu_version", "dispu_error_string", "dispu_linear_tile", "dispu_linear_tile2", "dispu_linear_plan", "dispu_linear_bf16_plan",
+_NO_TAPE = ("dispu_version", "dispu_error_string", "dispu_linear_tile", "dispu_linear_tile2", "dispu_linear_plan", "dispu_linear_xyz3_plan",
+            "dispu_linear_bf16_plan",
             "dispu_linear_tn_plan", "dispu_linear_tn_bf16_plan", "dispu_linear_tn_bf16_stream_plan")
 
 
@@ -372,6 +377,16 @@
     buf = (_i * LINEAR_PLAN_INTS)()
     check(lib().dispu_linear_plan(batch, M, K, N, X, ldx, sx, W, ldw, sw, transb, bias, scale, shift, act, Y, ldy, sy, R1, ldr1, sr1, R2, ldr2,
                                   sr2, Mk, ldm, mcols, buf), "dispu_linear_plan")
+    return _plan_launches(buf)
+
+
+def linear_xyz3_plan(M, K, N, X, ldx, W, ldw, bias, Y, ldy, xyz, W3, ldw3, c_lo, c_hi):
+    buf = (_i * LINEAR_PLAN_INTS)()
+    check(lib().dispu_linear_xyz3_plan(M, K, N, X, ldx, W, ldw, bias, Y, ldy, xyz, W3, ldw3, c_lo, c_hi, buf), "dispu_linear_xyz3_plan")
+    return _plan_launches(buf)
+
+
+def _plan_launches(buf):
     out = []
     for i in range(buf[0]):
         kind, n0, n1, bm, bn, bk, tb, edge, epi, ng = buf[1 + 10 * i:11 + 10 * i]
diff --git a/dis-pu_amd/csrc/linear.hip b/dis-pu_amd/csrc/linear.hip
--- a/dis-pu_amd/csrc/linear.hip
+++ b/dis-pu_amd/csrc/linear.hip
@@ -22,6 +22,10 @@
     const float* scale;
     const float* shift;
     const float* Mk; long ldm; int mcols;
+    const float* P3 = nullptr;
+    const float* W3 = nullptr;
+    long ldw3 = 0;
+    int c_lo = 0, c_hi = 0;
 };
 
 template <int BM, int BN, int BK, bool TRANSB, bool EDGE>
@@ -220,6 +224,14 @@
             for (int r = 0; r < 16; ++r) acc[i][j][r] = 0.f;
 
     const int fi = lane & 31, fk = lane >> 5;
+    constexpr bool E_XYZ = (EPI_T == 7);
+    float p3[3] = {0.f, 0.f, 0.f};
+    if constexpr (E_XYZ) {
+        int prow = m0 + wm * (TM * 32) + lane % (TM * 32);
+        if (EDGE && prow >= M) prow = M - 1;
+        const float* pp = a.P3 + (size_t)prow * 3;
+        p3[0] = pp[0]; p3[1] = pp[1]; p3[2] = pp[2];
+    }
     constexpr bool CI = !EDGE && !TRANSB && (TN == 4 || TN == 2);
     auto rdB = [&](const float* Bs, int krow, float (&b)[TN]) {
         if constexpr (CI && TN == 4) {
@@ -323,7 +335,7 @@
 #ifdef LIN_CLOCK
     if (blockIdx.x == 0 && blockIdx.y == 5 && threadIdx.x == 0) { lin_clock_ticks[0] = __builtin_readcyclecounter() - lc0; lin_clock_ticks[1] = ntile; lin_clock_ticks[2] = lc_wait; }
 #endif
-    constexpr int EPI = (EPI_T == 6) ? 0 : EPI_T;
+    constexpr int EPI = (EPI_T == 6 || EPI_T == 7) ? 0 : EPI_T;
     constexpr bool E_SCALE = (EPI == 1 || EPI == 4), E_R1 = (EPI >= 2), E_R2 = (EPI >= 3);
     float* __restrict__ Y = a.Y + (size_t)z * a.sy;
     const float lo = (a.act == 1) ? 0.f : -__builtin_inff();
@@ -335,6 +347,12 @@
     const long ldy = a.ldy, ldr1 = a.ldr1, ldr2 = a.ldr2, ldm = a.ldm;
     const unsigned offy = (unsigned)(4 * fk * ldy + fi), off1 = (unsigned)(4 * fk * ldr1 + fi), off2 = (unsigned)(4 * fk * ldr2 + fi);
     const unsigned offm = (unsigned)(4 * fk * ldm + fi);
+    const float* pts = lds + wave * 256;
+    if constexpr (E_XYZ) {
+        *reinterpret_cast<float4*>(lds + wave * 256 + (lane % (TM * 32)) * 4) = make_float4(p3[0], p3[1], p3[2], 0.f);
+        __builtin_amdgcn_fence(__ATOMIC_RELEASE, "wavefront");
+        __builtin_amdgcn_wave_barrier();
+    }
     if constexpr (CI) {
         typedef float vecT __attribute__((ext_vector_type(TN)));
         const int col0 = cbase + TN * fi;
@@ -346,6 +364,27 @@
         if (has_bias) bv = *reinterpret_cast<const vecT*>(a.bias + col0);
         if constexpr (E_SCALE) {
             if (a.scale) { sc = *reinterpret_cast<const vecT*>(a.scale + col0); sh = *reinterpret_cast<const vecT*>(a.shift + col0); }
+        }
+        if constexpr (E_XYZ) {
+            if (col0 >= a.c_lo && col0 < a.c_hi) {
+                const vecT w0 = *reinterpret_cast<const vecT*>(a.W3 + col0), w1 = *reinterpret_cast<const vecT*>(a.W3 + a.ldw3 + col0),
+                           w2 = *reinterpret_cast<const vecT*>(a.W3 + 2 * a.ldw3 + col0);
+#pragma unroll
+                for (int i = 0; i < TM; ++i) {
+#pragma unroll
+                    for (int r = 0; r < 16; ++r) {
+                        const int rw = i * 32 + (r & 3) + 8 * (r >> 2);
+                        const float4 pt = *reinterpret_cast<const float4*>(pts + (rw + 4 * fk) * 4);
+#pragma unroll
+                        for (int j = 0; j < TN; ++j) {
+                            float g = pt.x * w0[j];
+                            g = __builtin_fmaf(pt.y, w1[j], g);
+                            g = __builtin_fmaf(pt.z, w2[j], g);
+                            acc[i][j][r] = acc[i][j][r] + g;
+                        }
+                    }
+                }
+            }
         }
 #pragma unroll
         for (int i = 0; i < TM; ++i) {
@@ -416,6 +455,27 @@
         if constexpr (E_SCALE) {
             if (a.scale) { sc = a.scale[colc]; sh = a.shift[colc]; }
         }
+        if constexpr (E_XYZ) {
+            if (colu >= a.c_lo && colu < a.c_hi) {
+                const float w0 = a.W3[colc], w1 = a.W3[a.ldw3 + colc], w2 = a.W3[2 * a.ldw3 + colc];
+#pragma unroll
+                for (int i = 0; i < TM; ++i) {
+#pragma unroll
+                    for (int r = 0; r < 16; ++r) {
+                        const int rw = i * 32 + (r & 3) + 8 * (r >> 2);
+                        const int rowu = rbase + rw;
+                        const float4 pt = *reinterpret_cast<const float4*>(pts + (rw + 4 * fk) * 4);
+                        if (col_ok && (!EDGE || rowu + 4 * fk < M)) {
+                            float g = pt.x * w0;
+                            g = __builtin_fmaf(pt.y, w1, g);
+                            g = __builtin_fmaf(pt.z, w2, g);
+                            (Y + (size_t)rowu * ldy + colu)[offy] = (acc[i][j][r] + g) + bv;
+                        }
+                    }
+                }
+                continue;
+            }
+        }
 #pragma unroll
         for (int i = 0; i < TM; ++i) {
             float r1v[16], r2v[16], mkv[16];
@@ -538,13 +598,15 @@
                              (!a.scale || (al16(a.scale) && al16(a.shift))) &&
                              (!a.R1 || (((a.ldr1 & 3) == 0) && ((a.sr1 & 3) == 0) && al16(a.R1))) &&
                              (!a.R2 || (((a.ldr2 & 3) == 0) && ((a.sr2 & 3) == 0) && al16(a.R2))) &&
-                             (!a.Mk || (((a.ldm & 3) == 0) && al16(a.Mk) && a.mcols >= a.N));
+                             (!a.Mk || (((a.ldm & 3) == 0) && al16(a.Mk) && a.mcols >= a.N)) &&
+                             (!a.W3 || (((a.ldw3 & 3) == 0) && al16(a.W3)));
     const bool tiles_ok = aligned && out_aligned && (a.M % l.bm == 0) && (a.N % l.bn == 0);
     if (tiles_ok && !transb && (a.K % BK == 0)) { l.bk = BK; l.edge = 0; }
     else if (tiles_ok && transb && (a.K % bkr == 0)) { l.bk = bkr; l.edge = 0; }
     else { l.bk = bkr; l.edge = 1; }
-    if (!a.scale && !a.R1 && !a.R2 && !a.Mk)
-        l.epi = (l.bm == 128 && l.bn == 256 && l.bk == 16 && !transb && !l.edge && a.K >= 1024) ? 6 : 0;
+    if (a.W3) l.epi = 7;
+    else if (!a.scale && !a.R1 && !a.R2 && !a.Mk)
+        l.epi =(l.bm == 128 && l.bn == 256 && l.bk == 16 && !transb && !l.edge && a.K >= 1024) ? 6 : 0;
     else if (a.scale && !a.R1 && !a.R2 && !a.Mk) l.epi = 1;
     else l.epi = a.Mk ? 5 : 4;
     return l;
@@ -597,6 +659,9 @@
         case 6:
             if constexpr (BM == 128 && BN == 256 && BK == 16 && !TRANSB && !EDGE) return launch_epi<BM, BN, WM, WN, BK, TRANSB, EDGE, 6>(a, grid, s);
             break;
+        case 7:
+            if constexpr (!TRANSB) return launch_epi<BM, BN, WM, WN, BK, TRANSB, EDGE, 7>(a, grid, s);
+            break;
     }
     return (int)hipErrorInvalidValue;
 }
@@ -608,6 +673,28 @@
     if (!l.edge) return launch_one<BM, BN, WM, WN, BKR, true, false>(a, grid, l.epi, s);
     if (l.transb) return launch_one<BM, BN, WM, WN, BKR, true, true>(a, grid, l.epi, s);
     return launch_one<BM, BN, WM, WN, BKR, false, true>(a, grid, l.epi, s);
+}
+
+static int launch_tiled(const LinearArgs& a, int batch, const LinearLaunch& l, hipStream_t s) {
+    switch (l.bm * 1000 + l.bn) {
+        case 128256: return launch_linear<128, 256, 2, 2, 16>(a, batch, l, s);
+        case 128128: return launch_linear<128, 128, 2, 2, 16, 32>(a, batch, l, s);
+        case 64128: return launch_linear<64, 128, 2, 2, 16, 32>(a, batch, l, s);
+        case 128064: return launch_linear<128, 64, 2, 2, 16, 32>(a, batch, l, s);
+        default: return launch_linear<64, 64, 2, 2, 16, 32>(a, batch, l, s);
+    }
+}
+
+static void plan_write(int rc, const LinearPlan& p, int* plan) {
+    for (int i = 0; i < DISPU_LINEAR_PLAN_INTS; ++i) plan[i] = 0;
+    if (rc) return;
+    plan[0] = p.n;
+    for (int i = 0; i < p.n; ++i) {
+        const LinearLaunch& l = p.l[i];
+        int* o = plan + 1 + 10 * i;
+        o[0] = l.skinny ? 0 : 1; o[1] = l.n0; o[2] = l.n1; o[3] = l.bm; o[4] = l.bn; o[5] = l.bk; o[6] = l.transb; o[7] = l.edge;
+        o[8] = l.epi; o[9] = l.ng;
+    }
 }
 
 static int linear_impl(int batch, int M, int K, int N, const float* X, long ldx, long sx, const float* W, long ldw, long sw, int transb,
@@ -645,16 +732,8 @@
     LinearPlan p;
     const int rc = linear_decide(batch, M, K, N, X, ldx, sx, W, ldw, sw, transb, bias, scale, shift, act, Y, ldy, sy, R1, ldr1, sr1, R2,
                                  ldr2, sr2, Mk, ldm, Mk ? mcols : 0, p);
-    for (int i = 0; i < DISPU_LINEAR_PLAN_INTS; ++i) plan[i] = 0;
-    if (rc) return rc;
-    plan[0] = p.n;
-    for (int i = 0; i < p.n; ++i) {
-        const LinearLaunch& l = p.l[i];
-        int* o = plan + 1 + 10 * i;
-        o[0] = l.skinny ? 0 : 1; o[1] = l.n0; o[2] = l.n1; o[3] = l.bm; o[4] = l.bn; o[5] = l.bk; o[6] = l.transb; o[7] = l.edge;
-        o[8] = l.epi; o[9] = l.ng;
-    }
-    return 0;
+    plan_write(rc, p, plan);
+    return rc;
 }
 
 static int linear_impl(int batch, int M, int K, int N, const float* X, long ldx, long sx, const float* W, long ldw, long sw, int transb,
@@ -675,15 +754,40 @@
         } else {
             LinearArgs a{M, K, nn, X, ldx, sx, W, ldw, sw, bias, Y, ldy, sy, R1, ldr1, sr1, R2, ldr2, sr2, act, scale, shift,
                          (Mk && mcols > 0) ? Mk : nullptr, ldm, mcols};
-            switch (l.bm * 1000 + l.bn) {
-                case 128256: rc = launch_linear<128, 256, 2, 2, 16>(a, batch, l, s); break;
-                case 128128: rc = launch_linear<128, 128, 2, 2, 16, 32>(a, batch, l, s); break;
-                case 64128: rc = launch_linear<64, 128, 2, 2, 16, 32>(a, batch, l, s); break;
-                case 128064: rc = launch_linear<128, 64, 2, 2, 16, 32>(a, batch, l, s); break;
-                default: rc = launch_linear<64, 64, 2, 2, 16, 32>(a, batch, l, s); break;
-            }
+            rc = launch_tiled(a, batch, l, s);
         }
         if (rc) return rc;
     }
     return 0;
 }
+
+static int linear_xyz3_decide(int M, int K, int N, const float* X, long ldx, const float* W, long ldw, const float* bias, const float* Y,
+                              long ldy, const float* xyz, const float* W3, long ldw3, int c_lo, int c_hi, LinearArgs& a, LinearPlan& plan) {
+    plan = LinearPlan{};
+    if (M < 0 || K <= 0 || N <= 0 || !X || !W || !bias || !Y || !xyz || !W3 || ldw3 < N) return (int)hipErrorInvalidValue;
+    if (c_lo < 0 || c_hi < c_lo || c_hi > N || (c_lo % 64) != 0 || (c_hi % 64) != 0) return (int)hipErrorInvalidValue;
+    a = LinearArgs{M, K, N, X, ldx, 0, W, ldw, 0, bias, const_cast<float*>(Y), ldy, 0, nullptr, 0, 0, nullptr, 0, 0, 0, nullptr, nullptr,
+                   nullptr, 0, 0, xyz, W3, ldw3, c_lo, c_hi};
+    if (M == 0) return 0;
+    plan.l[plan.n++] = linear_decide_tiled(a, 1, false);
+    return 0;
+}
+
+DISPU_EXPORT int dispu_linear_xyz3(int M, int K, int N, const float* X, long ldx, const float* W, long ldw, const float* bias, float* Y,
+                                   long ldy, const float* xyz, const float* W3, long ldw3, int c_lo, int c_hi, void* stream) {
+    LinearArgs a;
+    LinearPlan plan;
+    const int rc = linear_xyz3_decide(M, K, N, X, ldx, W, ldw, bias, Y, ldy, xyz, W3, ldw3, c_lo, c_hi, a, plan);
+    if (rc || plan.n == 0) return rc;
+    return launch_tiled(a, 1, plan.l[0], (hipStream_t)stream);
+}
+
+DISPU_EXPORT int dispu_linear_xyz3_plan(int M, int K, int N, const float* X, long ldx, const float* W, long ldw, const float* bias,
+                                        const float* Y, long ldy, const float* xyz, const float* W3, long ldw3, int c_lo, int c_hi, int* plan) {
+    if (!plan) return (int)hipErrorInvalidValue;
+    LinearArgs a;
+    LinearPlan p;
+    const int rc = linear_xyz3_decide(M, K, N, X, ldx, W, ldw, bias, Y, ldy, xyz, W3, ldw3, c_lo, c_hi, a, p);
+    plan_write(rc, p, plan);
+    return rc;
+}
diff --git a/dis-pu_amd/csrc/ps_local.hip b/dis-pu_amd/csrc/ps_local.hip
--- a/dis-pu_amd/csrc/ps_local.hip
+++ b/dis-pu_amd/csrc/ps_local.hip
@@ -10,6 +10,7 @@
 typedef float f32x4 __attribute__((ext_vector_type(4)));
 typedef unsigned u32x4 __attribute__((ext_vector_type(4)));
 typedef unsigned u32x2 __attribute__((ext_vector_type(2)));
+typedef unsigned u32x3 __attribute__((ext_vector_type(3)));
 typedef __bf16 bf16x4 __attribute__((ext_vector_type(4)));
 
 constexpr int PL_BM = 128, PL_BN = 128, PL_BK = 32, PL_K = 128, PL_NT = 256;
@@ -184,7 +185,7 @@
 constexpr int PW_FLOATS = PW_WRES + 2 * PW_ASTG + 2 * 2048 + 2 * 1024 + 512;
 constexpr size_t PW_LDS_BYTES = (size_t)PW_FLOATS * sizeof(float);
 
-template <bool UNI, bool OUT16 = false>
+template <bool UNI, bool OUT16 = false, bool FORM = false>
 __global__ __launch_bounds__(512) void ps_local_ws_kernel(long npoints, int n_per_cloud, const int* __restrict__ idx,
                                                            const float* __restrict__ xyz, const float* __restrict__ Gm, int ldg,
                                                            const float* __restrict__ Am, const float* __restrict__ W1,
@@ -285,15 +286,39 @@
             }
         };
         float4 arow;
+        float4 wc0 = make_float4(0.f, 0.f, 0.f, 0.f), wc1 = wc0, wc2 = wc0;
+        if constexpr (FORM) {
+            wc0 = *reinterpret_cast<const float4*>(Am + 0 * PL_K + (ht & 31) * 4);
+            wc1 = *reinterpret_cast<const float4*>(Am + 1 * PL_K + (ht & 31) * 4);
+            wc2 = *reinterpret_cast<const float4*>(Am + 2 * PL_K + (ht & 31) * 4);
+        }
         auto load_arow = [&](int g) {
-            if constexpr (UNI) {
+            if constexpr (FORM) {
+                if constexpr (UNI) {
+                    const u32x3 r = __builtin_amdgcn_raw_buffer_load_b96(r_x, (ht >> 5) * 12, g * 96, 0);
+                    arow = make_float4(__uint_as_float(r[0]), __uint_as_float(r[1]), __uint_as_float(r[2]), 0.f);
+                } else {
+                    const float* p = xyz + (size_t)clampi(g * 8 + (ht >> 5)) * 3;
+                    arow = make_float4(p[0], p[1], p[2], 0.f);
+                }
+            } else if constexpr (UNI) {
                 arow = bload4(r_a, ht * 16, g * (8 * PL_K * 4));
             } else {
                 const int i = clampi(g * 8 + (ht >> 5));
                 arow = *reinterpret_cast<const float4*>(Am + (size_t)i * PL_K + (ht & 31) * 4);
             }
         };
-        auto store_arow = [&](float* ab) { *reinterpret_cast<float4*>(ab + (ht >> 5) * PL_K + (ht & 31) * 4) = arow; };
+        auto store_arow = [&](float* ab) {
+            float4 v = arow;
+            if constexpr (FORM) {
+                const f32x2 xx = {arow.x, arow.x}, yy = {arow.y, arow.y}, zz = {arow.z, arow.z};
+                f32x2 lo = xx * f32x2{wc0.x, wc0.y}, hi = xx * f32x2{wc0.z, wc0.w};
+                lo = __builtin_elementwise_fma(yy, f32x2{wc1.x, wc1.y}, lo); hi = __builtin_elementwise_fma(yy, f32x2{wc1.z, wc1.w}, hi);
+                lo = __builtin_elementwise_fma(zz, f32x2{wc2.x, wc2.y}, lo); hi = __builtin_elementwise_fma(zz, f32x2{wc2.z, wc2.w}, hi);
+                v = make_float4(lo.x, lo.y, hi.x, hi.y);
+            }
+            *reinterpret_cast<float4*>(ab + (ht >> 5) * PL_K + (ht & 31) * 4) = v;
+        };
         const int wt = ht & 15, wsn = (ht >> 4) & 15;
         const float ww0 = Ww[wt], ww1 = Ww[16 + wt], ww2 = Ww[32 + wt], wbw = bw[wt], wsc = scale[wt], wsh = shift[wt];
         int pj = 0, pi_ = 0;
@@ -550,7 +575,7 @@
 
 using namespace dispu;
 
-template <bool OUT16>
+template <bool OUT16, bool FORM = false>
 static int pw_launch(long npoints, int n_per_cloud, const int* idx, const float* xyz, const float* G, long ldg, const float* A, const float* W1,
                      const float* b1, const float* Ww, const float* bw, const float* scale, const float* shift,
                      std::conditional_t<OUT16, unsigned short, float>* out, hipStream_t stream) {
@@ -562,12 +587,13 @@
         const long ngroups = (np + 7) / 8;
         const unsigned grid = (unsigned)(ngroups < 256 ? ngroups : 256);
         const bool uni = (n_per_cloud % 8) == 0 && (np % 8) == 0 && np * ldg * 4 < 0x7fffffffL;
+        const float* Ap = FORM ? A : A + p0 * PL_K;
         if (uni)
-            hipLaunchKernelGGL((ps_local_ws_kernel<true, OUT16>), dim3(grid), dim3(512), PW_LDS_BYTES, stream, np, n_per_cloud, idx + p0 * 16,
-                               xyz + p0 * 3, G + p0 * ldg, (int)ldg, A + p0 * PL_K, W1, b1, Ww, bw, scale, shift, out + p0 * 2048);
+            hipLaunchKernelGGL((ps_local_ws_kernel<true, OUT16, FORM>), dim3(grid), dim3(512), PW_LDS_BYTES, stream, np, n_per_cloud, idx + p0 * 16,
+                               xyz + p0 * 3, G + p0 * ldg, (int)ldg, Ap, W1, b1, Ww, bw, scale, shift, out + p0 * 2048);
         else
-            hipLaunchKernelGGL((ps_local_ws_kernel<false, OUT16>), dim3(grid), dim3(512), PW_LDS_BYTES, stream, np, n_per_cloud, idx + p0 * 16,
-                               xyz + p0 * 3, G + p0 * ldg, (int)ldg, A + p0 * PL_K, W1, b1, Ww, bw, scale, shift, out + p0 * 2048);
+            hipLaunchKernelGGL((ps_local_ws_kernel<false, OUT16, FORM>), dim3(grid), dim3(512), PW_LDS_BYTES, stream, np, n_per_cloud, idx + p0 * 16,
+                               xyz + p0 * 3, G + p0 * ldg, (int)ldg, Ap, W1, b1, Ww, bw, scale, shift, out + p0 * 2048);
     }
     return 0;
 }
@@ -621,3 +647,36 @@
     if (rc) return rc;
     return (int)hipGetLastError();
 }
+
+template <bool OUT16>
+static int ps_local_xyz(long npoints, int n_per_cloud, int k, int c, const int* idx, const float* xyz, const float* G, long ldg, const float* W0,
+                        const float* W1, const float* b1, const float* Ww, const float* bw, const float* scale, const float* shift,
+                        std::conditional_t<OUT16, unsigned short, float>* out, void* stream) {
+    if (npoints < 0 || n_per_cloud <= 0 || k != 16 || c != 128 || ldg < 128 || (ldg & 3) || npoints * ldg > 0x7fffffffL) return (int)hipErrorInvalidValue;
+    if (!W0 || ((((uintptr_t)G) | ((uintptr_t)W0) | ((uintptr_t)W1) | ((uintptr_t)out)) & 15)) return (int)hipErrorInvalidValue;
+    if (npoints == 0) return 0;
+    static DevOnce attr;
+    if (attr.needed()) {
+        DISPU_TRY(hipFuncSetAttribute(reinterpret_cast<const void*>(ps_local_ws_kernel<false, OUT16, true>),
+                                      hipFuncAttributeMaxDynamicSharedMemorySize, (int)PW_LDS_BYTES));
+        DISPU_TRY(hipFuncSetAttribute(reinterpret_cast<const void*>(ps_local_ws_kernel<true, OUT16, true>),
+                                      hipFuncAttributeMaxDynamicSharedMemorySize, (int)PW_LDS_BYTES));
+        attr.done();
+    }
+    const int rc = pw_launch<OUT16, true>(npoints, n_per_cloud, idx, xyz, G, ldg, W0, W1, b1, Ww, bw, scale, shift, out, (hipStream_t)stream);
+    if (rc) return rc;
+    return (int)hipGetLastError();
+}
+
+DISPU_EXPORT int dispu_ps_local_xyz(long npoints, int n_per_cloud, int k, int c, const int* idx, const float* xyz, const float* G, long ldg,
+                                    const float* W0, const float* W1, const float* b1, const float* Ww, const float* bw, const float* scale,
+                                    const float* shift, float* out, void* stream) {
+    return ps_local_xyz<false>(npoints, n_per_cloud, k, c, idx, xyz, G, ldg, W0, W1, b1, Ww, bw, scale, shift, out, stream);
+}
+
+DISPU_EXPORT int dispu_ps_local_xyz_bf16(long npoints, int n_per_cloud, int k, int c, const int* idx, const float* xyz, const float* G,
+                                         long ldg, const float* W0, const float* W1, const float* b1, const float* Ww, const float* bw,
+                                         const float* scale, const float* shift, void* out, void* stream) {
+    return ps_local_xyz<true>(npoints, n_per_cloud, k, c, idx, xyz, G, ldg, W0, W1, b1, Ww, bw, scale, shift,
+                              reinterpret_cast<unsigned short*>(out), stream);
+}
diff --git a/dis-pu_amd/generator.py b/dis-pu_amd/generator.py
--- a/dis-pu_amd/generator.py
+++ b/dis-pu_amd/generator.py
@@ -117,7 +117,10 @@
         nlp = "refine/PointShuffle/PointShuffle/"
         self.w_up3 = torch.cat([self.P[nlp + "conv_kv/weights"], self.P[nlp + "conv_query/weights"], self.w_c0_feat], dim=1).contiguous()
         self.b_up3 = torch.cat([self.P[nlp + "conv_kv/biases"], self.P[nlp + "conv_query/biases"],
-                                torch.zeros(128, dtype=torch.float32, device=dev)]).contiguous()
+                                self.P["refine/PointShuffle/conv0/biases"]]).contiguous()
+        self.b_up3_pair = self.b_up3.clone()
+        self.b_up3_pair[192:] = 0.0
+        self.w_xyz3 = torch.cat([torch.zeros((3, 192), dtype=torch.float32, device=dev), w0[0:3] + w0[3:6]], dim=1).contiguous()
         wsk = self.P["refine/PointShuffle/skip/weights"]
         self.w_skip_pad = torch.cat([wsk, torch.zeros((10, wsk.shape[1]), dtype=torch.float32, device=dev)], dim=0).contiguous()
         if self.dtype == "bf16":
@@ -145,7 +148,7 @@
             feat=E(rn, 480), prep=E(rn, 48), prep_b=E(rn, 48), kidx=E(rn, k + 1, dtype=i32), h256=E(rn, 256),
             up256=E(rm, 256), up128=E(rm, 128), c256=E(rm, 256), c64=E(rm, 64), coarse=E(B, M, 3),
             psidx=E(rm, k, dtype=i32), up3=E(rm, 320), att=E(rm, 64), nl=E(rm, 256),
-            skipin=torch.zeros((rm, 144), dtype=f32, device=dev), skip=E(rm, 256), am=E(rm, 128),
+            skipin=torch.zeros((rm, 144), dtype=f32, device=dev), skip=E(rm, 256),
             fp=E(rm, 2048, dtype=torch.bfloat16 if self.dtype == "bf16" else f32), aft=E(rm, 256), agg=E(rm, 256),
             f256=E(rm, 256), f64=E(rm, 64), fine=E(B, M, 3))
         ws["kv"], ws["q"], ws["gm"] = ws["up3"][:, 0:128], ws["up3"][:, 128:192], ws["up3"][:, 192:320]
@@ -183,6 +186,15 @@
                                     None, 0, 0)
             name = linear_profile_name(plan, batch, M, K, N)
         self._call(name, _lib.lib().dispu_linear, batch, M, K, N, x, ldx, sx, w, ldw, sw, transb, b, act, y, ldy, sy, r1, ldr1, 0, r2, ldr2, 0, st)
+
+    def _linear_xyz3(self, st, ws, col, N, c_lo, c_hi):
+        up128, coarse, rm = ws["up128"], ws["coarse"], ws["up128"].shape[0]
+        args = (rm, 128, N, _lib.ptr(up128), 128, _off(self.w_up3, col), 320, _off(self.b_up3, col), _off(ws["up3"], col), 320,
+                _lib.ptr(coarse), _off(self.w_xyz3, col), 320, c_lo, c_hi)
+        name = "linear"
+        if self.profile is not None:
+            name = linear_profile_name(_lib.linear_xyz3_plan(*args), 1, rm, 128, N)
+        self._call(name, _lib.lib().dispu_linear_xyz3, *args, st)
 
     def __call__(self, inputs):
         return self.forward(inputs)
@@ -333,8 +345,12 @@
             aux.wait_event(ev_fork)
             sb = _lib.C.c_void_p(aux.cuda_stream)
         with (torch.cuda.stream(aux) if br else contextlib.nullcontext()):
-            self._linear(sb, ws["up128"], 128, self.w_up3, self.b_up3, 0, ws["up3"], 256)
-            self._linear(sb, ws["up128"], 128, self.w_up3, self.b_up3[256:], 0, ws["up3"], 64, woff=256, yoff=256)
+            if path.local == "pair":
+                self._linear(sb, ws["up128"], 128, self.w_up3, self.b_up3_pair, 0, ws["up3"], 256)
+                self._linear(sb, ws["up128"], 128, self.w_up3, self.b_up3_pair[256:], 0, ws["up3"], 64, woff=256, yoff=256)
+            else:
+                self._linear_xyz3(sb, ws, 0, 256, 192, 256)
+                self._linear_xyz3(sb, ws, 256, 64, 0, 64)
             if br:
                 ev_up3.record(aux)
             w_bp, b_bp = self._w("refine/PointShuffle/PointShuffle/conv_back_project")
@@ -367,15 +383,16 @@
     def _local(self, ws, path, B, N, st):
         L, ptr = _lib.lib(), _lib.ptr
         M, k, ps = N * self.up_ratio, K_NEIGH, "refine/PointShuffle/"
-        rm, coarse, psidx, gm, am = B * M, ws["coarse"], ws["psidx"], ws["gm"], ws["am"]
+        rm, coarse, psidx, gm = B * M, ws["coarse"], ws["psidx"], ws["gm"]
         w0, b0 = self._w(ps + "conv0")
-        self._call("ps_prep", L.dispu_ps_prep, rm, 128, ptr(coarse), ptr(w0), ptr(b0), ptr(gm), 320, ptr(am), 128, st)
         w1, b1 = self._w(ps + "conv1")
         wnet = [ptr(t) for t in self._w(ps + "weight_net/wconv0") + (self.bn_scale, self.bn_shift)]
         if path.local != "pair":
-            name, fn = ("ps_local_bf16", L.dispu_ps_local_bf16) if path.local == "bf16" else ("ps_local", L.dispu_ps_local)
-            self._call(name, fn, rm, M, k, 128, ptr(psidx), ptr(coarse), ptr(gm), 320, ptr(am), ptr(w1), ptr(b1), *wnet, ptr(ws["fp"]), st)
+            name, fn = ("ps_local_bf16", L.dispu_ps_local_xyz_bf16) if path.local == "bf16" else ("ps_local", L.dispu_ps_local_xyz)
+            self._call(name, fn, rm, M, k, 128, ptr(psidx), ptr(coarse), ptr(gm), 320, ptr(w0), ptr(w1), ptr(b1), *wnet, ptr(ws["fp"]), st)
             return
+        am = self._extra(ws, "am", (rm, 128))
+        self._call("ps_prep", L.dispu_ps_prep, rm, 128, ptr(coarse), ptr(w0), ptr(b0), ptr(gm), 320, ptr(am), 128, st)
         rows = rm * k
         flat = self._extra(self._ws, ("pair", B, N), (rows * 272,))
         x1, x2, wv = (t.view(rows, -1) for t in flat.split([rows * 128, rows * 128, rows * 16]))
diff --git a/include/dispu_hip.h b/include/dispu_hip.h
--- a/include/dispu_hip.h
+++ b/include/dispu_hip.h
@@ -124,6 +124,10 @@
                       int transb, const float* bias, const float* scale, const float* shift, int act, const float* Y, long ldy,
                       long sy, const float* R1, long ldr1, long sr1, const float* R2, long ldr2, long sr2, const float* Mk,
                       long ldm, int mcols, int* plan);
+int dispu_linear_xyz3(int M, int K, int N, const float* X, long ldx, const float* W, long ldw, const float* bias, float* Y, long ldy,
+                      const float* xyz, const float* W3, long ldw3, int c_lo, int c_hi, void* stream);
+int dispu_linear_xyz3_plan(int M, int K, int N, const float* X, long ldx, const float* W, long ldw, const float* bias, const float* Y,
+                           long ldy, const float* xyz, const float* W3, long ldw3, int c_lo, int c_hi, int* plan);
 int dispu_linear_small_k(long rows, int K, int N, const float* X, long ldx, const float* W, const float* bias, int act,
                          float* Y, long ldy, void* stream);
 int dispu_linear_small_n(long rows, int K, int N, const float* X, long ldx, const float* W, const float* bias, int mode,
@@ -156,6 +160,12 @@
 int dispu_ps_local_bf16(long npoints, int n_per_cloud, int k, int c, const int* idx, const float* xyz, const float* G, long ldg,
                         const float* A, const float* W1, const float* b1, const float* Ww, const float* bw, const float* scale,
                         const float* shift, void* out, void* stream);
+int dispu_ps_local_xyz(long npoints, int n_per_cloud, int k, int c, const int* idx, const float* xyz, const float* G, long ldg,
+                       const float* W0, const float* W1, const float* b1, const float* Ww, const float* bw, const float* scale,
+                       const float* shift, float* out, void* stream);
+int dispu_ps_local_xyz_bf16(long npoints, int n_per_cloud, int k, int c, const int* idx, const float* xyz, const float* G, long ldg,
+                            const float* W0, const float* W1, const float* b1, const float* Ww, const float* bw, const float* scale,
+                            const float* shift, void* out, void* stream);
 int dispu_attention(int b, int m, int nk, int d, const float* Q, long ldq, const float* K, long ldk, const float* V,
                     long ldv, float scale, float* O, long ldo, void* stream);
 int dispu_attention_project(int b, int m, int nk, int d, const float* Q, long ldq, const float* K, long ldk, const float* V,
```

Result: no change. 36.13 million points/s, median of 6 (+0.2%).
